# mfkiwl/hyteg

Hardware: AMD Instinct MI355X
Metric: DoF-updates/s, P1 Laplace apply() level 8 (higher is better)
Workload: dtype f64

## Files before the change

hyteg_amd/capi.py:

```python
from __future__ import annotations

import ctypes as C
from pathlib import Path

_PKG = Path(__file__).resolve().parent
_LIB_PATH = _PKG / "lib" / "libhyteg_hip.so"

REPLACE, ADD = 0, 1
MIN_LEVEL, MAX_LEVEL, MAX_SRCS = 2, 11, 4

_vp, _i, _d, _sz, _i64 = C.c_void_p, C.c_int, C.c_double, C.c_size_t, C.c_int64
_dp = C.POINTER(C.c_double)
SIGNATURES = {
    "hyteg_hip_version": (C.c_char_p, []),
    "hyteg_hip_last_error": (C.c_char_p, []),
    "hyteg_hip_device_count": (_i, [C.POINTER(_i)]),
    "hyteg_hip_set_device": (_i, [_i]),
    "hyteg_hip_device_name": (_i, [C.c_char_p, _sz]),
    "hyteg_hip_malloc": (_i, [C.POINTER(_vp), _sz]),
    "hyteg_hip_free": (_i, [_vp]),
    "hyteg_hip_memset_zero": (_i, [_vp, _sz, _vp]),
    "hyteg_hip_upload": (_i, [_vp, _vp, _sz, _vp]),
    "hyteg_hip_download": (_i, [_vp, _vp, _sz, _vp]),
    "hyteg_hip_copy": (_i, [_vp, _vp, _sz, _vp]),
    "hyteg_hip_calib_copy": (_i, [_vp, _vp, _i64, _i, _vp]),
    "hyteg_hip_p2_operator_table_closure_split": (_i, [_vp, _vp, _vp, _vp]),
    "hyteg_hip_p2_operator_table_face_edge_weights": (_i, [_vp, C.POINTER(_i), _vp]),
    "hyteg_hip_p2_sor_face_frames_bytes": (_sz, []),
    "hyteg_hip_p2_sor_face_frames": (_i, [_i, C.POINTER(_i), _vp, _vp]),
    "hyteg_hip_p2_sor_face_edgedofs_cells": (_i, [_i, C.POINTER(_vp), C.POINTER(_vp), _i, _vp, _d, C.POINTER(C.c_uint), _i, _vp]),
    "hyteg_hip_p2_sor_face_edgedofs_cell": (_i, [_vp, _vp, _i, C.POINTER(_i), _vp, _d, C.c_uint, _i, _vp]),
    "hyteg_hip_calib_copy_ring": (_i, [C.POINTER(_vp), C.POINTER(_vp), _i, _i64, _i, _i, _i, _vp, _vp, _vp]),
    "hyteg_hip_stream_create": (_i, [C.POINTER(_vp)]),
    "hyteg_hip_stream_destroy": (_i, [_vp]),
    "hyteg_hip_stream_synchronize": (_i, [_vp]),
    "hyteg_hip_stream_is_capturing": (_i, [_vp, C.POINTER(_i)]),
    "hyteg_hip_event_create": (_i, [C.POINTER(_vp)]),
    "hyteg_hip_event_create_timing": (_i, [C.POINTER(_vp)]),
    "hyteg_hip_event_elapsed_ms": (_i, [_vp, _vp, C.POINTER(C.c_float)]),
    "hyteg_hip_event_destroy": (_i, [_vp]),
    "hyteg_hip_event_record": (_i, [_vp, _vp]),
    "hyteg_hip_stream_wait_event": (_i, [_vp, _vp]),
    "hyteg_hip_comm_available": (_i, [C.c_char_p, _sz]),
    "hyteg_hip_comm_unique_id": (_i, [C.c_char_p]),
    "hyteg_hip_comm_create": (_i, [C.POINTER(_vp), _i, _i, C.c_char_p]),
    "hyteg_hip_comm_destroy": (_i, [_vp]),
    "hyteg_hip_comm_exchange": (_i, [_vp, _i, C.POINTER(_i), _vp, C.POINTER(_i), _vp, C.POINTER(_i), _vp]),
    "hyteg_hip_comm_allreduce_sum": (_i, [_vp, _vp, _i, _vp]),
    "hyteg_hip_p2p_arena_create": (_i, [C.c_size_t, C.POINTER(_vp), C.c_char_p, C.POINTER(_i)]),
    "hyteg_hip_p2p_arena_destroy": (_i, [_vp]),
    "hyteg_hip_p2p_arena_open": (_i, [C.c_char_p, C.POINTER(_vp)]),
    "hyteg_hip_p2p_arena_close": (_i, [_vp]),
    "hyteg_hip_p2p_pack": (_i, [_vp, _i, _vp, _vp, _vp, _i, C.c_ulonglong, _vp, _vp]),
    "hyteg_hip_p2p_wait": (_i, [_vp, _i, _i, C.c_ulonglong, _vp, C.c_uint, _vp]),
    "hyteg_hip_p1_apply_cell_boundary_p2p": (_i, [_vp, _vp, _i, _vp, C.c_uint, _i, _vp, _vp, _vp, _i, C.c_ulonglong, _vp, _vp]),
    "hyteg_hip_reduce_shared_after_p2p": (_i, [_vp, _vp, _vp, _vp, _i, _i, _i, _vp, _i, _i, C.c_ulonglong, _vp, C.c_uint, _vp]),
    "hyteg_hip_graph_begin_capture": (_i, [_vp]),
    "hyteg_hip_graph_end_capture": (_i, [_vp, C.POINTER(_vp)]),
    "hyteg_hip_graph_abort_capture": (_i, [_vp]),
    "hyteg_hip_graph_launch": (_i, [_vp, _vp]),
    "hyteg_hip_graph_destroy": (_i, [_vp]),
    "hyteg_hip_prepare_level": (_i, [_i]),
    "hyteg_hip_cell_width": (_i64, [_i]),
    "hyteg_hip_cell_size": (_i64, [_i]),
    "hyteg_hip_cell_inner_size": (_i64, [_i]),
    "hyteg_hip_cell_index": (_i64, [_i, _i, _i, _i]),
    "hyteg_hip_p1_apply_cell": (_i, [_vp, _vp, _i, _dp, _i, _vp]),
    "hyteg_hip_p1_apply_cell_steps": (_i, [C.POINTER(_vp), C.POINTER(_vp), _i, _i, _dp, _i, _vp]),
    "hyteg_hip_p1_apply_kernel_name": (_i, [_i, _i, C.c_char_p, _sz]),
    "hyteg_hip_p1_residual_jacobi_start_f32": (_i, [_vp, _vp, _vp, _vp, _i, _dp, _d, _vp]),
    "hyteg_hip_p1_jacobi_accumulate_f32": (_i, [_vp, _vp, _vp, _i, _dp, _d, _vp]),
    "hyteg_hip_set_apply_shape": (_i, [_i, _i, _i]),
    "hyteg_hip_p1_apply_cell_f32": (_i, [_vp, _vp, _i, _dp, _i, _vp]),
    "hyteg_hip_p1_jacobi_cell_f32": (_i, [_vp, _vp, _vp, _vp, _i, _dp, _d, _vp]),
    "hyteg_hip_convert_f64_to_f32": (_i, [_vp, _vp, _sz, _vp]),
    "hyteg_hip_convert_f32_to_f64": (_i, [_vp, _vp, _sz, _vp]),
    "hyteg_hip_axpy_f32_into_f64": (_i, [_vp, _vp, _d, _sz, _vp]),
    "hyteg_hip_p1_jacobi_cell": (_i, [_vp, _vp, _vp, _vp, _i, _dp, _d, _vp]),
    "hyteg_hip_p1_chebyshev_start_cell": (_i, [_vp, _vp, _vp, _vp, _i, _dp, _vp]),
    "hyteg_hip_p1_chebyshev_step_cell": (_i, [_vp, _vp, _vp, _vp, _i, _dp, _d, _d, _i, _vp]),
    "hyteg_hip_p1_sor_cell": (_i, [_vp, _vp, _i, _dp, _d, _i, _vp]),
    "hyteg_hip_p1_residual_cell": (_i, [_vp, _vp, _vp, _i, _dp, _vp]),
    "hyteg_hip_p1_sor_cell_sweeps": (_i, [_vp, _vp, _i, _dp, _d, _i, _i, _vp]),
    "hyteg_hip_set_sor_algorithm": (_i, [_i]),
    "hyteg_hip_p1_assign_cell": (_i, [_vp, _i, C.POINTER(_vp), _dp, _i, _vp]),
    "hyteg_hip_p1_add_cell": (_i, [_vp, _i, C.POINTER(_vp), _dp, _i, _vp]),
    "hyteg_hip_p1_mult_cell": (_i, [_vp, _i, C.POINTER(_vp), _i, _vp]),
    "hyteg_hip_dot_workspace_bytes": (_sz, []),
    "hyteg_hip_p1_dot_cell": (_i, [_vp, _vp, _i, _vp, _vp, _vp]),
    "hyteg_hip_p1_restrict_cell": (_i, [_vp, _vp, _i, _dp, _vp]),
    "hyteg_hip_p1_prolongate_cell": (_i, [_vp, _vp, _i, _dp, _i, _vp]),
    "hyteg_hip_p1_apply_cell_boundary": (_i, [_vp, _vp, _i, _dp, C.c_uint, _i, _vp]),
    "hyteg_hip_p1_vector_cell_masked": (_i, [_i, _vp, _i, C.POINTER(_vp), _dp, _i, C.c_uint, _vp]),
    "hyteg_hip_p1_set_cell_masked": (_i, [_vp, _d, _i, C.c_uint, _vp]),
    "hyteg_hip_p1_dot_cell_masked": (_i, [_vp, _vp, _i, C.c_uint, _vp, _vp, _vp]),
    "hyteg_hip_p1_restrict_cell_masked": (_i, [_vp, _vp, _i, _dp, C.c_uint, _vp]),
    "hyteg_hip_p1_prolongate_cell_masked": (_i, [_vp, _vp, _i, _dp, C.c_uint, _vp]),
    "hyteg_hip_p1_prolongate_cell_masked_update": (_i, [_vp, _vp, _i, _dp, C.c_uint, _i, _vp]),
    "hyteg_hip_sum_shared": (_i, [_vp, _vp, _vp, _vp, _i, _i, _vp]),
    "hyteg_hip_copy_shared": (_i, [_vp, _vp, _vp, _vp, _i, _i, _vp]),
    "hyteg_hip_p1_copy_face_to_cell": (_i, [_vp, _vp, _i, _i, _i, _i, _vp]),
    "hyteg_hip_p1_copy_cell_to_face": (_i, [_vp, _vp, _i, _i, _i, _i, _i, _vp]),
    "hyteg_hip_p1_vector_cells": (_i, [_i, _i, C.POINTER(_vp), _i, C.POINTER(_vp), _dp, _i, C.POINTER(C.c_uint), _vp]),
    "hyteg_hip_p1_dot_cells": (_i, [_i, C.POINTER(_vp), C.POINTER(_vp), _i, C.POINTER(C.c_uint), _vp, _vp, _vp]),
    "hyteg_hip_p1_apply_cells": (_i, [_i, C.POINTER(_vp), C.POINTER(_vp), _i, _vp, C.POINTER(C.c_uint), _i, _vp]),
    "hyteg_hip_p1_jacobi_cells": (_i, [_i, C.POINTER(_vp), C.POINTER(_vp), C.POINTER(_vp), C.POINTER(_vp), _i, _vp, _d,
                                        C.POINTER(C.c_uint), _i, _vp]),
    "hyteg_hip_p1_restrict_cells": (_i, [_i, C.POINTER(_vp), C.POINTER(_vp), _i, _vp, C.POINTER(C.c_uint), _vp]),
    "hyteg_hip_p1_prolongate_cells": (_i, [_i, C.POINTER(_vp), C.POINTER(_vp), _i, _vp, C.POINTER(C.c_uint), _i, _vp]),
    "hyteg_hip_p2_edge_array_size": (C.c_size_t, [_i]),
    "hyteg_hip_p2_operator_table_size": (C.c_size_t, []),
    "hyteg_hip_p2_build_operator_table": (_i, [_dp, _dp]),
    "hyteg_hip_p2_prolongate_cell": (_i, [_vp, _vp, _vp, _vp, _i, _i, C.c_uint, _vp]),
    "hyteg_hip_p2_restrict_cell": (_i, [_vp, _vp, _vp, _vp, _i, _dp, C.c_uint, _vp]),
    "hyteg_hip_p2_restrict_cells": (_i, [_i, C.POINTER(_vp), C.POINTER(_vp), C.POINTER(_vp), C.POINTER(_vp), _i, _vp, C.POINTER(C.c_uint), _vp]),
    "hyteg_hip_p2_prolongate_cells": (_i, [_i, C.POINTER(_vp), C.POINTER(_vp), C.POINTER(_vp), C.POINTER(_vp), _i, _i, C.POINTER(C.c_uint), _vp]),
    "hyteg_hip_p2_edge_vector_cell_masked": (_i, [_i, _vp, _i, C.POINTER(_vp), _dp, _i, C.c_uint, _vp]),
    "hyteg_hip_p2_edge_vector_cell_kinds": (_i, [_i, _vp, _i, C.POINTER(_vp), _dp, _i, C.c_uint, C.c_uint, _vp]),
    "hyteg_hip_p2_elementwise_apply_cells_kinds": (_i, [_i, C.POINTER(_vp), C.POINTER(_vp), C.POINTER(_vp), C.POINTER(_vp), _i, C.POINTER(_vp), _d, _i,
                                                   C.POINTER(C.c_uint), C.c_uint, _vp]),
    "hyteg_hip_p2_edge_dot_cells_masked": (_i, [_i, C.POINTER(_vp), C.POINTER(_vp), _i, C.POINTER(C.c_uint), _vp, _vp]),
    "hyteg_hip_p2_edge_vector_cells_kinds": (_i, [_i, _i, C.POINTER(_vp), _i, C.POINTER(_vp), _dp, _i, C.POINTER(C.c_uint), C.c_uint, _vp]),
    "hyteg_hip_p2_edge_dot_cell_masked": (_i, [_vp, _vp, _i, C.c_uint, _vp, _vp, _vp]),
    "hyteg_hip_p2_elementwise_apply_cell": (_i, [_vp, _vp, _vp, _vp, _i, _vp, _d, _i, C.c_uint, _vp]),
    "hyteg_hip_p2_elementwise_apply_cell_kinds": (_i, [_vp, _vp, _vp, _vp, _i, _vp, _d, _i, C.c_uint, C.c_uint, _vp]),
    "hyteg_hip_p2_set_class_rows_min_level": (_i, [_i]),
    "hyteg_hip_p1_vector_cells_dev": (_i, [_i, _i, C.POINTER(_vp), _i, C.POINTER(_vp), C.POINTER(_vp), _i, C.POINTER(C.c_uint), _vp]),
    "hyteg_hip_cg_scalars": (_i, [_vp, _i, _d, _d, _vp]),
    "hyteg_hip_p1_cg_small_max_entries": (_i, []),
    "hyteg_hip_p1_cg_small_cells": (_i, [_i, C.POINTER(_vp), C.POINTER(_vp), _i, _vp, C.POINTER(C.c_uint), C.POINTER(C.c_uint), C.POINTER(_vp),
                                         C.POINTER(_vp), C.POINTER(_vp), C.POINTER(_i), _i, _d, _d, _vp, _vp]),
    "hyteg_hip_p1_dot_cells_cg": (_i, [_i, C.POINTER(_vp), C.POINTER(_vp), _i, C.POINTER(C.c_uint), _vp, _i, _i, _d, _d, _vp, _vp]),
    "hyteg_hip_p1_sor_cells": (_i, [_i, C.POINTER(_vp), C.POINTER(_vp), _i, _vp, _d, _i, C.POINTER(C.c_uint), _vp]),
    "hyteg_hip_p1_sor_shell_cells": (_i, [_i, C.POINTER(_vp), C.POINTER(_vp), C.POINTER(_vp), _i, _vp, _d, C.POINTER(C.c_uint), _i, _vp]),
    "hyteg_hip_p1_sor_shell_cell": (_i, [_vp, _vp, _vp, _i, C.POINTER(_i), _dp, C.POINTER(_i), _dp, _dp, _d, C.c_uint, _i, _vp]),
    "hyteg_hip_p1_apply_face3d": (_i, [_vp, _vp, _i, _i, C.POINTER(_i), _dp, _i, _vp]),
    "hyteg_hip_p1_sor_face3d_workspace": (C.c_size_t, [_i]),
    "hyteg_hip_p1_sor_face3d": (_i, [_vp, _vp, _vp, _i, _i, C.POINTER(_i), _dp, C.c_double, _i, _vp]),
    "hyteg_hip_gather_entries": (_i, [_vp, _vp, _vp, _vp, _i, _vp]),
    "hyteg_hip_p2_constant_stencil_layout": (_i, [C.POINTER(_i), C.POINTER(_i)]),
    "hyteg_hip_p2_build_operator_table_from_stencils": (_i, [_dp, _dp, _dp]),
    "hyteg_hip_p2_apply_cell_edgedof_to_vertexdof": (_i, [_vp] * 7 + [_vp, _dp, _i, _i, _vp]),
    "hyteg_hip_p2_apply_cell_vertexdof_to_edgedof": (_i, [_vp] * 7 + [_vp, _i, _dp, _i, _vp]),
    "hyteg_hip_p2_apply_cell_edgedof_to_edgedof": (_i, [_vp] * 14 + [_dp, _i, _i, _vp]),
    "hyteg_hip_p1_elementwise_diffusion_apply_macro_3d": (_i, [_vp, _vp, _dp, _i64, _d, _vp]),
    "hyteg_hip_p1_elementwise_diffusion_apply_macro_3d_masked": (_i, [_vp, _vp, _dp, _i64, C.c_uint, _i, _vp]),
    "hyteg_hip_p1_elementwise_diffusion_apply_macro_3d_f32": (_i, [_vp, _vp, C.POINTER(C.c_float), _i64, C.c_float, _vp]),
    "hyteg_hip_p1_elementwise_diffusion_diagonal_macro_3d": (_i, [_vp, _dp, _i64, _d, _vp]),
    "hyteg_hip_p1_elementwise_diffusion_stencils": (_i, [_dp, _i64, _dp, _dp]),
    "hyteg_hip_p1_apply_cell_boundary_f32": (_i, [_vp, _vp, _i, _dp, C.c_uint, _i, _vp]),
    "hyteg_hip_p2_elementwise_diffusion_apply_macro_3d": (_i, [_vp, _vp, _vp, _vp, _dp, _i64, _d, _vp]),
    "hyteg_hip_p2_elementwise_diffusion_element_matrices": (_i, [_dp, _i64, _dp]),
}
MASK_INNER, MASK_SHELL, MASK_ALL = 1 << 14, 0x3FFF, 0x7FFF


class HytegHipError(RuntimeError):
    pass


def lib_path() -> Path:
    return _LIB_PATH


_lib = None


def lib() -> C.CDLL:
    global _lib
    if _lib is None:
        if not _LIB_PATH.exists():
            raise HytegHipError(
                f"{_LIB_PATH} not found: build it with `python -c 'import __graft_entry__ as g; g.build()'` "
                "(hipcc --offload-arch=gfx950).  hyteg_amd has no CPU fallback.")
        l = C.CDLL(str(_LIB_PATH))
# ... 95 lines not shown


def event_record(ev, stream=0) -> None:
    check(lib().hyteg_hip_event_record(ev, stream), "event_record")


def stream_wait_event(stream, ev) -> None:
    check(lib().hyteg_hip_stream_wait_event(stream, ev), "stream_wait_event")


def calib_copy(dst, src, n, nontemporal=True, stream=0) -> None:
    check(lib().hyteg_hip_calib_copy(dst, src, n, 1 if nontemporal else 0, stream), "calib_copy")


def calib_copy_ring(pairs, n, nontemporal=True, stream=0):
    m = len(pairs)
    d, s = (_vp * m)(*[p[0] for p in pairs]), (_vp * m)(*[p[1] for p in pairs])
    fn = lib().hyteg_hip_calib_copy_ring

    def call(first, count, ev_start=None, ev_stop=None):
        check(fn(d, s, m, n, 1 if nontemporal else 0, first, count, stream, ev_start, ev_stop), "calib_copy_ring")

    return call


def p1_residual_jacobi_start_f32(r_f32, e_f32, rhs, src, level, w, relax, stream=0):
    check(lib().hyteg_hip_p1_residual_jacobi_start_f32(r_f32, e_f32, rhs, src, level, _w15(w), float(relax), stream), "p1_residual_jacobi_start_f32")


def p1_jacobi_accumulate_f32(x, rhs_f32, e_f32, level, w, relax, stream=0):
    check(lib().hyteg_hip_p1_jacobi_accumulate_f32(x, rhs_f32, e_f32, level, _w15(w), float(relax), stream), "p1_jacobi_accumulate_f32")


def set_apply_shape(ny=0, lz=0, pfd=0) -> None:
    check(lib().hyteg_hip_set_apply_shape(ny, lz, pfd), "set_apply_shape")


def p1_apply_kernel_name(level, update=REPLACE) -> str:
    buf = C.create_string_buffer(256)
    check(lib().hyteg_hip_p1_apply_kernel_name(level, update, buf, 256), "p1_apply_kernel_name")
    return buf.value.decode()


def p2_prolongate_cell(fine_v, fine_e, coarse_v, coarse_e, coarse_level, update=REPLACE, mask=0x7FFF, stream=0):
    check(lib().hyteg_hip_p2_prolongate_cell(fine_v, fine_e, coarse_v, coarse_e, coarse_level, update, mask, stream), "p2_prolongate_cell")


def p2_restrict_cell(coarse_v, coarse_e, fine_v, fine_e, coarse_level, nnc, mask=0x7FFF, stream=0):
    a = (C.c_double * 14)(*[float(x) for x in nnc])
    check(lib().hyteg_hip_p2_restrict_cell(coarse_v, coarse_e, fine_v, fine_e, coarse_level, a, mask, stream), "p2_restrict_cell")


def p1_apply_cell_f32(dst, src, level, w, update=REPLACE, stream=0):
    check(lib().hyteg_hip_p1_apply_cell_f32(dst, src, level, _w15(w), update, stream), "p1_apply_cell_f32")


def p1_jacobi_cell_f32(dst, rhs, src, level, w, relax, invdiag=None, stream=0):
    check(lib().hyteg_hip_p1_jacobi_cell_f32(dst, rhs, src, invdiag, level, _w15(w), relax, stream), "p1_jacobi_cell_f32")


def convert_f64_to_f32(dst, src, n, stream=0):
    check(lib().hyteg_hip_convert_f64_to_f32(dst, src, n, stream), "convert_f64_to_f32")


def convert_f32_to_f64(dst, src, n, stream=0):
    check(lib().hyteg_hip_convert_f32_to_f64(dst, src, n, stream), "convert_f32_to_f64")


def axpy_f32_into_f64(y, x, alpha, n, stream=0):
    check(lib().hyteg_hip_axpy_f32_into_f64(y, x, alpha, n, stream), "axpy_f32_into_f64")


def p1_apply_cell(dst, src, level, w, update=REPLACE, stream=0):
    check(lib().hyteg_hip_p1_apply_cell(dst, src, level, _w15(w), update, stream), "p1_apply_cell")


def p1_apply_cell_steps(dsts, srcs, level, w, update=REPLACE, stream=0):
    if len(srcs) != len(dsts):
        raise ValueError("p1_apply_cell_steps: as many sources as destinations")
    d, s = (_vp * len(dsts))(*[int(p) for p in dsts]), (_vp * len(srcs))(*[int(p) for p in srcs])
    check(lib().hyteg_hip_p1_apply_cell_steps(d, s, len(dsts), level, _w15(w), update, stream), "p1_apply_cell_steps")


def p1_jacobi_cell(dst, rhs, src, level, w, relax, invdiag=None, stream=0):
    check(lib().hyteg_hip_p1_jacobi_cell(dst, rhs, src, invdiag, level, _w15(w), float(relax), stream),
          "p1_jacobi_cell")


def p1_chebyshev_start_cell(t_out, rhs, x, level, w, invdiag=None, stream=0):
    check(lib().hyteg_hip_p1_chebyshev_start_cell(t_out, rhs, x, invdiag, level, _w15(w), stream), "p1_chebyshev_start_cell")


def p1_chebyshev_step_cell(t_out, x, t_in, level, w, c_prev, c_cur, has_prev=True, invdiag=None, stream=0):
    check(lib().hyteg_hip_p1_chebyshev_step_cell(t_out, x, t_in, invdiag, level, _w15(w), float(c_prev), float(c_cur),
                                                 int(bool(has_prev)), stream), "p1_chebyshev_step_cell")


SOR_AUTO, SOR_PLANES, SOR_BLOCKS, SOR_DATAFLOW = 0, 1, 2, 3


def set_sor_algorithm(algorithm: int) -> None:
    check(lib().hyteg_hip_set_sor_algorithm(int(algorithm)), "set_sor_algorithm")


def p1_sor_cell(u, rhs, level, w, relax, backwards=False, stream=0):
    check(lib().hyteg_hip_p1_sor_cell(u, rhs, level, _w15(w), float(relax), int(backwards), stream), "p1_sor_cell")


def p1_residual_cell(dst, rhs, src, level, w, stream=0):
    check(lib().hyteg_hip_p1_residual_cell(dst, rhs, src, level, _w15(w), stream), "p1_residual_cell")


def p1_sor_cell_sweeps(u, rhs, level, w, relax, nsweeps, backwards=False, stream=0):
    check(lib().hyteg_hip_p1_sor_cell_sweeps(u, rhs, level, _w15(w), float(relax), int(backwards), int(nsweeps), stream), "p1_sor_cell_sweeps")


def p1_assign_cell(dst, scalars, srcs, level, stream=0):
    check(lib().hyteg_hip_p1_assign_cell(dst, len(srcs), _ptrs(srcs), _scal(scalars), level, stream),
          "p1_assign_cell")


def p1_add_cell(dst, scalars, srcs, level, stream=0):
    check(lib().hyteg_hip_p1_add_cell(dst, len(srcs), _ptrs(srcs), _scal(scalars), level, stream), "p1_add_cell")


def p1_mult_cell(dst, srcs, level, stream=0):
    check(lib().hyteg_hip_p1_mult_cell(dst, len(srcs), _ptrs(srcs), level, stream), "p1_mult_cell")


def dot_workspace_bytes(): return int(lib().hyteg_hip_dot_workspace_bytes())


def p1_dot_cell(a, b, level, result_dev, workspace_dev, stream=0):
    check(lib().hyteg_hip_p1_dot_cell(a, b, level, result_dev, workspace_dev, stream), "p1_dot_cell")


def p1_restrict_cell(coarse, fine, coarse_level, nnc, stream=0):
    check(lib().hyteg_hip_p1_restrict_cell(coarse, fine, coarse_level, _f14(nnc), stream), "p1_restrict_cell")


def p1_prolongate_cell(coarse, fine, coarse_level, nnc, update=REPLACE, stream=0):
    check(lib().hyteg_hip_p1_prolongate_cell(coarse, fine, coarse_level, _f14(nnc), update, stream),
          "p1_prolongate_cell")


def p1_apply_cell_boundary(dst, src, level, w_slots, mask=MASK_SHELL, update=REPLACE, stream=0):
    flat = [float(v) for row in w_slots for v in row]
    arr = (C.c_double * 210)(*flat)
    check(lib().hyteg_hip_p1_apply_cell_boundary(dst, src, level, arr, mask, update, stream), "p1_apply_cell_boundary")


def p1_vector_cell_masked(op, dst, scalars, srcs, level, mask, stream=0):
    sc = _scal(scalars) if scalars is not None else None
    check(lib().hyteg_hip_p1_vector_cell_masked(op, dst, len(srcs), _ptrs(srcs), sc, level, mask, stream),
          "p1_vector_cell_masked")


def p1_set_cell_masked(dst, value, level, mask, stream=0):
    check(lib().hyteg_hip_p1_set_cell_masked(dst, float(value), level, mask, stream), "p1_set_cell_masked")


def p1_dot_cell_masked(a, b, level, mask, result_dev, workspace_dev, stream=0):
    check(lib().hyteg_hip_p1_dot_cell_masked(a, b, level, mask, result_dev, workspace_dev, stream), "p1_dot_cell_masked")


def p1_restrict_cell_masked(coarse, fine, coarse_level, nnc, mask, stream=0):
    check(lib().hyteg_hip_p1_restrict_cell_masked(coarse, fine, coarse_level, _f14(nnc), mask, stream),
          "p1_restrict_cell_masked")


def p1_prolongate_cell_masked(coarse, fine, coarse_level, nnc, mask, stream=0):
    check(lib().hyteg_hip_p1_prolongate_cell_masked(coarse, fine, coarse_level, _f14(nnc), mask, stream),
          "p1_prolongate_cell_masked")


def p1_prolongate_cell_masked_update(coarse, fine, coarse_level, nnc, mask, update=REPLACE, stream=0):
    check(lib().hyteg_hip_p1_prolongate_cell_masked_update(coarse, fine, coarse_level, _f14(nnc), mask, update, stream),
          "p1_prolongate_cell_masked_update")


def sum_shared(bases, group_ptr, entry_buf, entry_off, ngroups, n_writable, stream=0):
    check(lib().hyteg_hip_sum_shared(bases, group_ptr, entry_buf, entry_off, ngroups, n_writable, stream), "sum_shared")


def gather_entries(out, bases, entry_buf, entry_off, n, stream=0):
    check(lib().hyteg_hip_gather_entries(out, bases, entry_buf, entry_off, n, stream), "gather_entries")


def p1_copy_face_to_cell(cell, face, level, v, stream=0):
    check(lib().hyteg_hip_p1_copy_face_to_cell(cell, face, level, int(v[0]), int(v[1]), int(v[2]), stream), "p1_copy_face_to_cell")


def p1_copy_cell_to_face(face, cell, level, v, neighbor, stream=0):
    check(lib().hyteg_hip_p1_copy_cell_to_face(face, cell, level, int(v[0]), int(v[1]), int(v[2]), int(neighbor), stream),
          "p1_copy_cell_to_face")


def _ptrs(ps):
    return (C.c_void_p * len(ps))(*[int(p) for p in ps])


def _masks(ms):
    return (C.c_uint * len(ms))(*[int(m) for m in ms])


def p1_vector_cells(op, dst, srcs, scalars, level, masks, stream=0):
    n = len(dst)
    flat = [p for f in srcs for p in f]
    sc = (C.c_double * max(1, len(scalars or [])))(*[float(v) for v in (scalars or [0.0])])
    check(lib().hyteg_hip_p1_vector_cells(op, n, _ptrs(dst), len(srcs), _ptrs(flat) if flat else None, sc if scalars is not None else None,
                                          level, _masks(masks), stream), "p1_vector_cells")


def p1_dot_cells(a, b, level, masks, result_dev, workspace_dev, stream=0):
    check(lib().hyteg_hip_p1_dot_cells(len(a), _ptrs(a), _ptrs(b), level, _masks(masks), result_dev, workspace_dev, stream), "p1_dot_cells")


(HYTEG_HIP_CG_PRSOLD, HYTEG_HIP_CG_PAP, HYTEG_HIP_CG_RR, HYTEG_HIP_CG_ALPHA, HYTEG_HIP_CG_NEG_ALPHA, HYTEG_HIP_CG_BETA, HYTEG_HIP_CG_RES_START,
 HYTEG_HIP_CG_DONE, HYTEG_HIP_CG_ITERATIONS, HYTEG_HIP_CG_ONE) = range(10)
HYTEG_HIP_CG_SLOTS = 16
HYTEG_HIP_MAX_BATCH = 80


def p1_vector_cells_dev(op, dst, srcs, scalar_ptrs, level, masks, stream=0):
    flat = [p for f in srcs for p in f]
    sp = (_vp * len(scalar_ptrs))(*[None if p is None else int(p) for p in scalar_ptrs]) if scalar_ptrs is not None else None
    check(lib().hyteg_hip_p1_vector_cells_dev(op, len(dst), _ptrs(dst), len(srcs), _ptrs(flat) if flat else None, sp, level, _masks(masks), stream),
          "p1_vector_cells_dev")


def p1_dot_cells_cg(a, b, level, masks, s_dev, slot, phase, rel_tol, abs_tol, workspace_dev, stream=0):
    check(lib().hyteg_hip_p1_dot_cells_cg(len(a), _ptrs(a), _ptrs(b), level, _masks(masks), s_dev, slot, phase, float(rel_tol), float(abs_tol),
# ... 286 lines not shown
```

hyteg_amd/csrc/exp/apply_trace.hip:

```cpp
#include <algorithm>
#include <cmath>
#include <cstdlib>
#include <cstring>
#include <random>
#include <vector>

#include <hip/hip_runtime.h>

#ifdef ZM_DO_TRACE
__device__ unsigned long long* g_trace;
#define ZM_TRACE( slot )                                                                                              \
   do                                                                                                                 \
   {                                                                                                                  \
      if ( ( slot ) == 3 )                                                                                            \
         asm volatile( "s_waitcnt vmcnt(0)" ::: "memory" );                                                           \
      const unsigned long long _t = __builtin_amdgcn_s_memrealtime();                                                 \
      if ( ( threadIdx.x & 63 ) == 0 )                                                                                \
      {                                                                                                               \
         unsigned long long* _p = g_trace + ( (size_t) blockIdx.x * kZMarchWavesPerBlock + ( threadIdx.x >> 6 ) ) * 8; \
         _p[slot]               = _t;                                                                                 \
         if ( ( slot ) == 0 )                                                                                         \
         {                                                                                                            \
            _p[6] = __builtin_amdgcn_s_getreg( 20 | ( 0 << 6 ) | ( 31 << 11 ) );                          \
            _p[7] = __builtin_amdgcn_s_getreg( 4 | ( 0 << 6 ) | ( 31 << 11 ) );                            \
         }                                                                                                            \
      }                                                                                                               \
   } while ( 0 )
#endif

#include "../kernels_apply_zmarch.hpp"
#include "kernels_apply_zloop.hpp"

using namespace hyteg_hip;

template < int NY, int LZ, int PFD >
__global__ __launch_bounds__( 64 * kZMarchWavesPerBlock ) void zmarch_trace_kernel( const ZMarchArgs A )
{
   zmarch_body< APPLY_REPLACE, NY, LZ, PFD, double >( A, A.tasks, A.ntasks, A.xcd_chunk, A.src, A.dst );
}

#define CK( e )                                                                                \
   do                                                                                          \
   {                                                                                           \
      hipError_t _e = ( e );                                                                   \
      if ( _e != hipSuccess )                                                                  \
      {                                                                                        \
         fprintf( stderr, "%s:%d %s: %s\n", __FILE__, __LINE__, #e, hipGetErrorString( _e ) ); \
         exit( 1 );                                                                            \
      }                                                                                        \
   } while ( 0 )

__global__ __launch_bounds__( 64 ) void apply_rows_naive( double* dst, const double* src, int N, Stencil15 st )
{
   const int z = 1 + blockIdx.y, y = 1 + blockIdx.x;
   const int W = N - z, R = W - y;
   if ( y > W - 3 )
      return;
   const int     S0 = tri( W ), Sm = tri( W + 1 );
   const int     base = slice_start( N, z ) + row_start( W, y );
   const double* w    = st.w;
   for ( int x = 1 + threadIdx.x; x <= R - 2; x += 64 )
   {
      const int i = base + x;
      double    acc;
      acc    = w[6] * src[i - 1];
      acc    = fma( w[3], src[i - Sm + W + 1], acc );
      acc    = fma( w[10], src[i + R], acc );
      acc    = fma( w[5], src[i - R], acc );
      acc    = fma( w[12], src[i + S0 - W + 1], acc );
      acc    = fma( w[1], src[i - Sm + y + 1], acc );
      acc    = fma( w[8], src[i + 1], acc );
      acc    = fma( w[13], src[i + S0 - y - 1], acc );
      acc    = fma( w[2], src[i - Sm + W], acc );
      acc    = fma( w[9], src[i + R - 1], acc );
      acc    = fma( w[4], src[i - R - 1], acc );
      acc    = fma( w[11], src[i + S0 - W], acc );
      acc    = fma( w[0], src[i - Sm + y], acc );
      acc    = fma( w[7], src[i], acc );
      acc    = fma( w[14], src[i + S0 - y], acc );
      dst[i] = acc;
   }
}

template < typename T >
static T pct( std::vector< T > v, double p )
{
   std::sort( v.begin(), v.end() );
   return v[std::min( v.size() - 1, (size_t) ( p * ( v.size() - 1 ) + 0.5 ) )];
}

int main( int argc, char** argv )
{
   const int     level = argc > 1 ? atoi( argv[1] ) : 8;
   const int     reps  = argc > 2 ? atoi( argv[2] ) : 300;
   const int     nbuf  = argc > 3 ? atoi( argv[3] ) : 9;
   const int     N     = ( 1 << level ) + 1;
   const int     total = (int) tet64( N );
   const int64_t inner = hyteg_hip_cell_inner_size( level );
   printf( "level %d  N %d  entries %d  inner %lld  buffers %d pairs (%.1f MB total)\n", level, N, total, (long long) inner,
           nbuf, nbuf * 2.0 * total * 8 / 1e6 );

   std::vector< double >                    h( total );
   std::mt19937_64                          gen( 42 );
   std::uniform_real_distribution< double > U( 0, 1 );
   for ( auto& v : h )
      v = U( gen );
   Stencil15 st;
   for ( int k = 0; k < 15; ++k )
      st.w[k] = U( gen ) - 0.5;
   std::vector< double* > src( nbuf ), dst( nbuf );
   for ( int b = 0; b < nbuf; ++b )
   {
      CK( hipMalloc( &src[b], (size_t) total * 8 + 16 ) );
      CK( hipMalloc( &dst[b], (size_t) total * 8 + 16 ) );
      CK( hipMemcpy( src[b], h.data(), (size_t) total * 8, hipMemcpyHostToDevice ) );
      CK( hipMemset( dst[b], 0, (size_t) total * 8 ) );
   }
   double* refout;
   CK( hipMalloc( &refout, (size_t) total * 8 ) );
   CK( hipMemset( refout, 0, (size_t) total * 8 ) );
   hipLaunchKernelGGL( apply_rows_naive, dim3( N, N ), dim3( 64 ), 0, 0, refout, src[0], N, st );
// ... 142 lines not shown
```

hyteg_amd/csrc/exp/p1_apply_rank.hip:

```cpp
#include <cstdlib>

#include "../kernels_apply_zmarch.hpp"
#include "../p2p_device.hpp"
#include "../shell.hpp"

using namespace hyteg_hip;

namespace {

constexpr int kBrickNY = 4;
inline int   brick_lz( int level ) { return level >= 8 ? 8 : 4; }
constexpr int kRankThreads = 64 * kZMarchWavesPerBlock;

struct RankArgs
{
   shell::Slots14x15           S;
   unsigned                    mask;
   int                         update;
   int                         brickBlocks, shellBlocks;
   const hyteg_hip_p2p_peer_t* peers;
   int                         npeers;
   double* const*              bases;
   const int*                  entry_buf;
   const int*                  entry_off;
   int                         n;
   unsigned long long          seq;
   unsigned*                   counters;
   unsigned*                   status;
   unsigned long long          timeout_ticks;
   int                         dbg;
};

template < int MODE, int LZ >
__global__ __launch_bounds__( kRankThreads ) void p1_apply_rank_kernel( const BrickTask* tasks, int ntasks, int xcd_chunk, const ZMarchArgs A,
                                                                        const RankArgs R )
{
   const int b = blockIdx.x;
   if ( b < R.brickBlocks )
   {
      zmarch_body< MODE, kBrickNY, LZ, 2, double >( A, tasks, ntasks, xcd_chunk, A.src, A.dst );
      return;
   }
   double*       dst = static_cast< double* >( A.dst );
   const double* src = static_cast< const double* >( A.src );
   if ( b < R.brickBlocks + R.shellBlocks )
   {
      const int q = ( b - R.brickBlocks ) * kRankThreads + (int) threadIdx.x;
      int       x, y, z, slot;
      if ( !( R.dbg & 4 ) && shell::shell_point( A.N, q, x, y, z, slot ) && ( ( R.mask >> slot ) & 1u ) )
      {
         const double acc = shell::share( R.S, src, A.N, x, y, z, slot );
         const int    i   = cell_index( A.N, x, y, z );
         if ( R.dbg & 2 )
            dst[i] = acc;
         else
            __hip_atomic_store( dst + i, R.update == HYTEG_HIP_ADD ? acc + dst[i] : acc, __ATOMIC_RELAXED, __HIP_MEMORY_SCOPE_AGENT );
      }
      p2p::stores_acknowledged();
      __syncthreads();
      if ( threadIdx.x == 0 )
         __hip_atomic_fetch_add( R.counters + 1, 1u, __ATOMIC_RELAXED, __HIP_MEMORY_SCOPE_AGENT );
      return;
   }
   if ( threadIdx.x == 0 && !( R.dbg & 1 ) )
   {
      const unsigned long long t0 = wall_clock64();
      while ( __hip_atomic_load( R.counters + 1, __ATOMIC_RELAXED, __HIP_MEMORY_SCOPE_AGENT ) < (unsigned) R.shellBlocks )
      {
         if ( wall_clock64() - t0 > R.timeout_ticks )
         {
            __hip_atomic_store( R.status, 0x40000000u, __ATOMIC_RELAXED, __HIP_MEMORY_SCOPE_SYSTEM );
            break;
         }
         __builtin_amdgcn_s_sleep( 4 );
      }
   }
   __syncthreads();
   const int first = R.brickBlocks + R.shellBlocks;
   const int k     = ( b - first ) * kRankThreads + (int) threadIdx.x;
   if ( k < R.n && !( R.dbg & 8 ) )
      p2p::send_value( R.peers, R.npeers, k, R.seq,
                       __hip_atomic_load( R.bases[R.entry_buf[k]] + R.entry_off[k], __ATOMIC_RELAXED, __HIP_MEMORY_SCOPE_AGENT ) );
   p2p::stores_acknowledged();
   __syncthreads();
   if ( threadIdx.x == 0 )
   {
      const unsigned done = __hip_atomic_fetch_add( R.counters, 1u, __ATOMIC_RELAXED, __HIP_MEMORY_SCOPE_AGENT );
      if ( done == gridDim.x - first - 1 )
      {
         __hip_atomic_store( R.counters, 0u, __ATOMIC_RELAXED, __HIP_MEMORY_SCOPE_AGENT );
         __hip_atomic_store( R.counters + 1, 0u, __ATOMIC_RELAXED, __HIP_MEMORY_SCOPE_AGENT );
         p2p::publish( R.peers, R.npeers, R.seq );
      }
   }
}

template < int MODE, int LZ >
int launch_rank( double* dst, const double* src, int level, const double* w, RankArgs& R, hipStream_t stream )
{
   BrickTable bt;
   int        rc = get_bricks( level, kBrickNY, LZ, &bt );
   if ( rc != HYTEG_HIP_OK )
      return rc;
   ZMarchArgs A{};
   A.dst    = dst;
   A.src    = src;
   A.tasks  = bt.dev;
   A.ntasks = bt.count;
   A.N      = ( 1 << level ) + 1;
   A.bytes  = (unsigned) ( tet64( A.N ) * (int64_t) sizeof( double ) );
   for ( int k = 0; k < 15; ++k )
      A.st.w[k] = w[k];
   int nblocks   = ( bt.count + kZMarchWavesPerBlock - 1 ) / kZMarchWavesPerBlock;
   nblocks       = ( nblocks + 7 ) & ~7;
   if ( R.dbg & 16 )
      nblocks = 0;
   A.xcd_chunk   = nblocks / 8;
   R.brickBlocks = nblocks;
   R.shellBlocks = ( 4 * tri( A.N ) + kRankThreads - 1 ) / kRankThreads;
   const int packBlocks = R.n > 0 ? ( R.n + kRankThreads - 1 ) / kRankThreads : 1;
   hipLaunchKernelGGL( ( p1_apply_rank_kernel< MODE, LZ > ), dim3( nblocks + R.shellBlocks + packBlocks ), dim3( kRankThreads ), 0, stream, A.tasks,
                       A.ntasks, A.xcd_chunk, A, R );
   HH_CHECK_HIP( hipGetLastError() );
// ... 48 lines not shown
```

hyteg_amd/csrc/kernels_apply_zmarch.hpp:

```cpp
#pragma once

#include <algorithm>
#include <utility>
#include <vector>

#include "common.hpp"

namespace hyteg_hip {

constexpr int kBrickMaxSlices = 10;
struct BrickTask
{
   int i0;
   int W0;
   int y0;
   int xb;
   int nz;
   int pad;
   int base[kBrickMaxSlices];
};
static_assert( sizeof( BrickTask ) == 64, "BrickTask must be 64 bytes (one s_load_dwordx16)" );

struct ZMarchArgs
{
// ... 2 lines not shown
   const void*      rhs;
   const void*      invdiag;
   void*            dst2;
   double*          xacc;
   const BrickTask* tasks;
   int              ntasks;
   unsigned         bytes;
   int              xcd_chunk;
   int              N;
   double           relax;
   Stencil15        st;
   double           relax2;
   int              flag;
};

#ifndef HYTEG_ZM_WAVES_PER_BLOCK
#define HYTEG_ZM_WAVES_PER_BLOCK 4
#endif
constexpr int kZMarchWavesPerBlock = HYTEG_ZM_WAVES_PER_BLOCK;

#ifndef ZM_TRACE
#define ZM_TRACE( slot )
#endif

typedef int zm_v2i_t __attribute__( ( ext_vector_type( 2 ) ) );

template < typename T, int AUX = 0 >
__device__ inline T zm_load2( __amdgpu_buffer_rsrc_t r, int voff, int soff )
{
   if constexpr ( sizeof( T ) == 8 )
   {
      zm_v2i_t v = __builtin_amdgcn_raw_buffer_load_b64( r, voff, soff, AUX );
      return *reinterpret_cast< T* >( &v );
   }
   else
   {
      int v = __builtin_amdgcn_raw_buffer_load_b32( r, voff, soff, AUX );
      return *reinterpret_cast< T* >( &v );
   }
}
template < typename T, int AUX = 0 >
__device__ inline void zm_store2( __amdgpu_buffer_rsrc_t r, int voff, int soff, T d )
{
   if constexpr ( sizeof( T ) == 8 )
      __builtin_amdgcn_raw_buffer_store_b64( *reinterpret_cast< zm_v2i_t* >( &d ), r, voff, soff, AUX );
   else
      __builtin_amdgcn_raw_buffer_store_b32( *reinterpret_cast< int* >( &d ), r, voff, soff, AUX );
}
__device__ inline double zm_lane_minus_1( double v )
{
   int lo = __double2loint( v ), hi = __double2hiint( v );
   lo     = __builtin_amdgcn_mov_dpp( lo, 0x138, 0xf, 0xf, true );
   hi     = __builtin_amdgcn_mov_dpp( hi, 0x138, 0xf, 0xf, true );
   return __hiloint2double( hi, lo );
}
__device__ inline double zm_lane_plus_1( double v )
{
   int lo = __double2loint( v ), hi = __double2hiint( v );
   lo     = __builtin_amdgcn_mov_dpp( lo, 0x130, 0xf, 0xf, true );
   hi     = __builtin_amdgcn_mov_dpp( hi, 0x130, 0xf, 0xf, true );
   return __hiloint2double( hi, lo );
}
__device__ inline float zm_lane_minus_1( float v )
{
   return __int_as_float( __builtin_amdgcn_mov_dpp( __float_as_int( v ), 0x138, 0xf, 0xf, true ) );
}
__device__ inline float zm_lane_plus_1( float v )
{
   return __int_as_float( __builtin_amdgcn_mov_dpp( __float_as_int( v ), 0x130, 0xf, 0xf, true ) );
}

__host__ __device__ inline void zm_fill_bases( BrickTask& t, int LZ )
{
   int base = t.i0, Wq = t.W0;
   for ( int q = 0; q < kBrickMaxSlices; ++q )
   {
      t.base[q] = q < LZ + 2 ? base : 0;
      base += tri( Wq ) - ( t.y0 - 1 );
      Wq -= 1;
   }
}

template < int MODE, int NY, int LZ, int PFD, typename T >
__device__ inline void zmarch_body( const ZMarchArgs& A, const BrickTask* tasks, int ntasks, int xcd_chunk, const void* srcp, void* dstp )
{
   static_assert( LZ + 2 <= kBrickMaxSlices, "the table carries the slice bases of bricks of up to kBrickMaxSlices - 2 slices" );
   constexpr int SZ = (int) sizeof( T );
   ZM_TRACE( 0 );
   int b = blockIdx.x;
   if ( xcd_chunk > 0 )
      b = ( blockIdx.x & 7 ) * xcd_chunk + ( blockIdx.x >> 3 );
   const int task = __builtin_amdgcn_readfirstlane( b * kZMarchWavesPerBlock + ( threadIdx.x >> 6 ) );
   if ( task >= ntasks )
      return;
   const BrickTask t = tasks[task];
   const int lane = threadIdx.x & 63;
   ZM_TRACE( 1 );

   constexpr int kStAux = 2;
   const __amdgpu_buffer_rsrc_t rs = __builtin_amdgcn_make_buffer_rsrc( const_cast< void* >( srcp ), 0, A.bytes, 0x00020000 );
   const __amdgpu_buffer_rsrc_t rd = __builtin_amdgcn_make_buffer_rsrc( dstp, 0, MODE == APPLY_RESIDUAL_F32OUT ? A.bytes / 2 : A.bytes, 0x00020000 );
   constexpr bool kHasRhs = MODE == APPLY_JACOBI || MODE == APPLY_RESIDUAL || MODE == APPLY_RESIDUAL_F32OUT || MODE == APPLY_JACOBI_ACCUM ||
                            MODE == APPLY_CHEB_START;
   constexpr bool kHasInv = MODE == APPLY_JACOBI || MODE == APPLY_CHEB_START || MODE == APPLY_CHEB_STEP;
   static_assert( MODE != APPLY_CHEB_STEP || SZ == 8, "the Chebyshev step updates a double iterate" );
   const __amdgpu_buffer_rsrc_t rr = __builtin_amdgcn_make_buffer_rsrc( const_cast< void* >( kHasRhs ? A.rhs : srcp ), 0, A.bytes, 0x00020000 );
   const __amdgpu_buffer_rsrc_t rd2 =
       __builtin_amdgcn_make_buffer_rsrc( MODE == APPLY_RESIDUAL_F32OUT ? A.dst2 : dstp, 0, MODE == APPLY_RESIDUAL_F32OUT ? A.bytes / 2 : A.bytes, 0x00020000 );
   const __amdgpu_buffer_rsrc_t rx = __builtin_amdgcn_make_buffer_rsrc(
       ( MODE == APPLY_JACOBI_ACCUM || MODE == APPLY_CHEB_STEP ) ? (void*) A.xacc : dstp, 0, MODE == APPLY_JACOBI_ACCUM ? A.bytes * 2 : A.bytes, 0x00020000 );
   const __amdgpu_buffer_rsrc_t ri = __builtin_amdgcn_make_buffer_rsrc(
       const_cast< void* >( ( kHasInv && A.invdiag ) ? A.invdiag : srcp ), 0, A.bytes, 0x00020000 );

   const int lane_off = lane * SZ;
   const int ym       = t.y0 - 1;

   T S[LZ + 2][NY + 2];

   auto load_slice = [&]( auto qc, int base_q, int W_q ) {
      constexpr int q  = decltype( qc )::value;
      int           ix = base_q;
#pragma unroll
      for ( int r = 0; r < NY + 2; ++r )
      {
         const bool need = ( q == 0 ) ? ( r >= 1 ) : ( q == LZ + 1 ? ( r <= NY ) : true );
         if ( need )
         {
            const int last8 = ( W_q - ( ym + r ) - 1 - t.xb ) * SZ;
            S[q][r]         = zm_load2< T >( rs, min( lane_off, last8 ), ix * SZ );
         }
         ix += W_q - ( ym + r );
      }
   };

   int baseq[LZ + 2], Wqs[LZ + 2];
#pragma unroll
   for ( int q = 0; q < LZ + 2; ++q )
   {
      baseq[q] = t.base[q];
      Wqs[q]   = t.W0 - q;
   }
   [&]< int... Is >( std::integer_sequence< int, Is... > ) {
      ( load_slice( std::integral_constant< int, Is >{}, baseq[Is], Wqs[Is] ), ... );
   }
   ( std::make_integer_sequence < int, ( 2 + PFD <= LZ + 2 ? 2 + PFD : LZ + 2 ) > {} );
   ZM_TRACE( 2 );

   T w[15];
#pragma unroll
   for ( int i = 0; i < 15; ++i )
      w[i] = (T) A.st.w[i];
   const T invc  = (T) ( 1.0 / A.st.w[7] );
   const T relax = (T) A.relax;

   constexpr int kExAux = MODE == APPLY_ADD ? 2 : 0;
   T          EX0[LZ][NY], EX1[LZ][NY];
   double     EXD[LZ][NY];
   const bool hasInv = kHasInv && A.invdiag != nullptr;
   auto       load_extra = [&]( auto sc ) {
      constexpr int s = decltype( sc )::value;
      constexpr int q = s + 1;
      if constexpr ( MODE != APPLY_REPLACE )
      {
         const int W  = Wqs[q];
         int       ie = baseq[q] + ( W - ym );
#pragma unroll
         for ( int j = 0; j < NY; ++j )
         {
            const int last8 = ( W - ( t.y0 + j ) - 1 - t.xb ) * SZ;
            const int vo    = min( lane_off, last8 );
            if constexpr ( MODE == APPLY_CHEB_STEP )
               EXD[s][j] = zm_load2< double, 0 >( rx, vo, ie * 8 );
            else
               EX0[s][j] = MODE == APPLY_ADD ? zm_load2< T, kExAux >( rd, vo, ie * SZ ) : zm_load2< T, kExAux >( rr, vo, ie * SZ );
            if constexpr ( MODE == APPLY_JACOBI_ACCUM )
               EXD[s][j] = zm_load2< double, 2 >( rx, min( lane * 8, last8 * 2 ), ie * 8 );
            if constexpr ( kHasInv )
            {
               T v = invc;
               if ( hasInv )
                  v = zm_load2< T >( ri, vo, ie * SZ );
               EX1[s][j] = v;
            }
            ie += W - ( t.y0 + j );
         }
      }
   };
   if constexpr ( MODE != APPLY_REPLACE )
   {
      [&]< int... Is >( std::integer_sequence< int, Is... > ) { ( load_extra( std::integral_constant< int, Is >{} ), ... ); }
      ( std::make_integer_sequence < int, ( PFD < LZ ? PFD : LZ ) > {} );
   }

   auto step = [&]( auto sc ) {
      constexpr int s = decltype( sc )::value;
      constexpr int q = s + 1;
      if constexpr ( q + 1 + PFD <= LZ + 1 )
         load_slice( std::integral_constant< int, q + 1 + PFD >{}, baseq[q + 1 + PFD], Wqs[q + 1 + PFD] );
      if constexpr ( s + PFD < LZ )
         load_extra( std::integral_constant< int, s + PFD >{} );

      const int W  = Wqs[q];
      int       io = baseq[q] + ( W - ym );
      if constexpr ( s == 0 )
         ZM_TRACE( 3 );
#pragma unroll
      for ( int j = 0; j < NY; ++j )
      {
         const T am = S[q][j], a0 = S[q][j + 1], ap = S[q][j + 2];
         const T um = S[q + 1][j], u0 = S[q + 1][j + 1];
         const T d0 = S[q - 1][j + 1], dp = S[q - 1][j + 2];
         T pe = w[8] * a0;
         pe        = fma( w[5], am, pe );
         pe        = fma( w[12], um, pe );
         pe        = fma( w[1], d0, pe );
         T pw = w[6] * a0;
         pw        = fma( w[13], u0, pw );
         pw        = fma( w[2], dp, pw );
         pw        = fma( w[9], ap, pw );
         T acc = zm_lane_plus_1( pe ) + zm_lane_minus_1( pw );
         acc        = fma( w[3], dp, acc );
         acc        = fma( w[10], ap, acc );
         acc        = fma( w[4], am, acc );
         acc        = fma( w[11], um, acc );
         acc        = fma( w[0], d0, acc );
         acc        = fma( w[7], a0, acc );
         acc        = fma( w[14], u0, acc );

         const int R = W - ( t.y0 + j );
         T         out;
         if ( MODE == APPLY_REPLACE )
            out = acc;
         else if ( MODE == APPLY_ADD )
            out = acc + EX0[s][j];
         else if ( MODE == APPLY_RESIDUAL || MODE == APPLY_RESIDUAL_F32OUT )
            out = EX0[s][j] - acc;
         else if ( MODE == APPLY_JACOBI_ACCUM )
            out = a0 + relax * ( invc * ( EX0[s][j] - acc ) );
         else if ( MODE == APPLY_CHEB_START )
            out = EX1[s][j] * ( EX0[s][j] - acc );
         else if ( MODE == APPLY_CHEB_STEP )
            out = EX1[s][j] * acc;
         else
            out = a0 + relax * ( EX1[s][j] * ( EX0[s][j] - acc ) );
         const int      cnt = s < t.nz ? min( 62, R - 2 - t.xb ) : 0;
         const unsigned lm1 = (unsigned) ( lane - 1 );
         const bool     on  = lm1 < (unsigned) max( cnt, 0 );
         if constexpr ( MODE == APPLY_RESIDUAL_F32OUT )
         {
            const float rf = (float) out;
            zm_store2< float, 0 >( rd, on ? lane * 4 : -8, io * 4, rf );
            zm_store2< float, 0 >( rd2, on ? lane * 4 : -8, io * 4, (float) relax * ( (float) invc * rf ) );
         }
         else if constexpr ( MODE == APPLY_JACOBI_ACCUM )
            zm_store2< double, kStAux >( rx, on ? lane * 8 : -8, io * 8, EXD[s][j] + (double) out );
         else if constexpr ( MODE == APPLY_CHEB_STEP )
         {
            double xn = EXD[s][j];
            if ( A.flag )
               xn = xn + (double) A.relax2 * (double) a0;
            xn = xn + (double) relax * (double) out;
            zm_store2< T, kStAux >( rd, on ? lane_off : -8, io * SZ, out );
            zm_store2< double, kStAux >( rx, on ? lane * 8 : -8, io * 8, xn );
         }
         else
            zm_store2< T, kStAux >( rd, on ? lane_off : -8, io * SZ, out );
         io += R;
      }
   };

   [&]< int... Is >( std::integer_sequence< int, Is... > ) { ( step( std::integral_constant< int, Is >{} ), ... ); }
   ( std::make_integer_sequence< int, LZ >{} );
   ZM_TRACE( 4 );
}

template < int MODE, int NY, int LZ, int PFD, typename T >
__global__ __launch_bounds__( 64 * kZMarchWavesPerBlock ) void p1_apply_zmarch_preload_kernel( const BrickTask* tasks, int ntasks, int xcd_chunk,
                                                                                              const ZMarchArgs A )
{
   zmarch_body< MODE, NY, LZ, PFD, T >( A, tasks, ntasks, xcd_chunk, A.src, A.dst );
}

constexpr int kZMarchMaxSteps = 16;
struct ZMarchStepPtrs
{
   const void* srcs[kZMarchMaxSteps];
   void*       dsts[kZMarchMaxSteps];
};

template < int MODE, int NY, int LZ, int PFD, typename T >
__global__ __launch_bounds__( 64 * kZMarchWavesPerBlock ) void p1_apply_zmarch_steps_kernel( const BrickTask* tasks, int ntasks, int xcd_chunk,
                                                                                            const ZMarchArgs A, const ZMarchStepPtrs P )
{
   static_assert( MODE == APPLY_REPLACE || MODE == APPLY_ADD, "a steps launch has one source and one destination per step" );
   const unsigned step = blockIdx.y < (unsigned) kZMarchMaxSteps ? blockIdx.y : 0u;
   zmarch_body< MODE, NY, LZ, PFD, T >( A, tasks, ntasks, xcd_chunk, P.srcs[step], P.dsts[step] );
}

inline void build_brick_tasks( int level, int NY, int LZ, std::vector< BrickTask >& out )
{
   const int N = ( 1 << level ) + 1;
   out.clear();
   for ( int z0 = 1; z0 <= N - 4; z0 += LZ )
   {
      const int W = N - z0;
      for ( int y0 = 1; y0 <= W - 3; y0 += NY )
      {
         const int xmax = W - y0 - 2;
         for ( int x0 = 1; x0 <= xmax; x0 += 62 )
         {
            BrickTask t{};
            t.xb = x0 - 1;
            t.y0 = y0;
            t.W0 = W + 1;
            t.i0 = slice_start( N, z0 - 1 ) + row_start( W + 1, y0 - 1 ) + t.xb;
            t.nz = std::min( LZ, N - 4 - z0 + 1 );
            zm_fill_bases( t, LZ );
            out.push_back( t );
         }
      }
   }
}

}
```

hyteg_amd/csrc/p1_apply.hip:

```cpp
#include <cstdlib>
#include <string>
#include <type_traits>

#include "kernels_apply.hpp"
#include "kernels_apply_zmarch.hpp"

using namespace hyteg_hip;

namespace {

constexpr int kTile = 1024;

struct BrickShape
{
   int  ny, lz, pfd;
   bool operator==( const BrickShape& o ) const { return ny == o.ny && lz == o.lz && pfd == o.pfd; }
};
BrickShape g_shape_override{ 0, 0, 0 };

inline BrickShape default_shape( int mode, int level, bool f32 )
{
   if ( level <= 7 )
      return ( mode == APPLY_REPLACE || f32 ) ? BrickShape{ 2, 4, 1 } : BrickShape{ 4, 4, 1 };
   if ( level == 8 )
// ... 39 lines not shown
int zmarch_common_args( ZMarchArgs& A, int& nblocks, int NY, int LZ, int level, const double* w )
{
   nblocks = 0;
   BrickTable bt;
   int        rc = get_bricks( level, NY, LZ, &bt );
   if ( rc != HYTEG_HIP_OK || bt.count == 0 )
      return rc;
   A.tasks  = bt.dev;
   A.ntasks = bt.count;
   A.N      = ( 1 << level ) + 1;
   A.bytes  = (unsigned) ( tet64( A.N ) * (int64_t) sizeof( T ) );
   for ( int k = 0; k < 15; ++k )
      A.st.w[k] = w[k];
   nblocks     = ( bt.count + kZMarchWavesPerBlock - 1 ) / kZMarchWavesPerBlock;
   nblocks     = ( nblocks + 7 ) & ~7;
   A.xcd_chunk = nblocks / 8;
   static const bool xcdSlabs = env_flag( "HYTEG_HIP_APPLY_XCD_SLABS", true );
   if ( !xcdSlabs )
      A.xcd_chunk = 0;
   return HYTEG_HIP_OK;
}

template < int MODE, int NY, int LZ, int PFD, typename T >
int launch_zmarch_shape( void* dst, const T* src, const T* rhs, const T* invdiag, int level, const double* w, double relax, hipStream_t stream,
                         void* extra, double relax2, int flag )
{
   ZMarchArgs A{};
   int        nblocks = 0;
   const int  rc      = zmarch_common_args< T >( A, nblocks, NY, LZ, level, w );
   if ( rc != HYTEG_HIP_OK || nblocks == 0 )
      return rc;
   A.dst     = dst;
   A.src     = src;
   A.rhs     = rhs;
   A.invdiag = invdiag;
   A.dst2    = extra;
   A.xacc    = static_cast< double* >( extra );
   A.relax   = relax;
   A.relax2  = relax2;
   A.flag    = flag;
   hipLaunchKernelGGL( ( p1_apply_zmarch_preload_kernel< MODE, NY, LZ, PFD, T > ), dim3( nblocks ), dim3( 64 * kZMarchWavesPerBlock ), 0, stream, A.tasks,
                       A.ntasks, A.xcd_chunk, A );
   HH_CHECK_HIP( hipGetLastError() );
   return HYTEG_HIP_OK;
}

inline unsigned steps_lds_request( int level )
{
   static const int fromEnv = [] {
      const char* v = getenv( "HYTEG_HIP_APPLY_STEPS_WG_PER_CU" );
      return v ? atoi( v ) : -1;
   }();
   const int m = fromEnv >= 0 ? fromEnv : ( level == 8 ? 2 : 0 );
   return ( m >= 1 && m <= 6 ) ? (unsigned) ( ( 160 * 1024 / m ) & ~4095 ) : 0u;
}

template < int MODE, int NY, int LZ, int PFD >
int launch_zmarch_steps_shape( void* const* dsts, const void* const* srcs, int nsteps, int level, const double* w, hipStream_t stream )
{
   static_assert( MODE == APPLY_REPLACE || MODE == APPLY_ADD, "steps launch: Replace and Add" );
   ZMarchArgs A{};
   int        nblocks = 0;
   const int  rc      = zmarch_common_args< double >( A, nblocks, NY, LZ, level, w );
   if ( rc != HYTEG_HIP_OK || nblocks == 0 )
      return rc;
   ZMarchStepPtrs P{};
   for ( int k = 0; k < kZMarchMaxSteps; ++k )
   {
      P.srcs[k] = srcs[k < nsteps ? k : 0];
      P.dsts[k] = dsts[k < nsteps ? k : 0];
   }
   A.src = P.srcs[0];
   A.dst = P.dsts[0];
   auto           kern = p1_apply_zmarch_steps_kernel< MODE, NY, LZ, PFD, double >;
   const unsigned lds  = steps_lds_request( level );
   if ( lds > 0 )
   {
      static const hipError_t attr = hipFuncSetAttribute( reinterpret_cast< const void* >( kern ), hipFuncAttributeMaxDynamicSharedMemorySize, (int) lds );
      HH_CHECK_HIP( attr );
   }
   hipLaunchKernelGGL( kern, dim3( nblocks, nsteps ), dim3( 64 * kZMarchWavesPerBlock ), lds, stream, A.tasks, A.ntasks, A.xcd_chunk, A, P );
   HH_CHECK_HIP( hipGetLastError() );
   return HYTEG_HIP_OK;
}

template < int MODE, typename T = double >
int launch_zmarch( void* dst, const T* src, const T* rhs, const T* invdiag, int level, const double* w, double relax, hipStream_t stream,
                   void* extra = nullptr, double relax2 = 0.0, int flag = 0 )
{
   const int shapeMode = MODE == APPLY_RESIDUAL_F32OUT ? APPLY_RESIDUAL :
                                                         ( ( MODE == APPLY_JACOBI_ACCUM || MODE == APPLY_CHEB_START || MODE == APPLY_CHEB_STEP ) ? APPLY_JACOBI : MODE );
   int        rc       = HYTEG_HIP_OK;
   const bool compiled = with_compiled_shape( current_shape( shapeMode, level, !std::is_same< T, double >::value ), [&]( auto ny, auto lz, auto pfd ) {
      rc = launch_zmarch_shape< MODE, decltype( ny )::value, decltype( lz )::value, decltype( pfd )::value, T >( dst, src, rhs, invdiag, level, w, relax, stream,
                                                                                                                 extra, relax2, flag );
   } );
   return compiled ? rc : fail( HYTEG_HIP_EINVAL, "apply: brick shape not compiled in" );
}

template < int MODE >
int launch_zmarch_steps( void* const* dsts, const void* const* srcs, int nsteps, int level, const double* w, hipStream_t stream )
{
   int        rc       = HYTEG_HIP_OK;
   const bool compiled = with_compiled_shape( current_shape( MODE, level, false ), [&]( auto ny, auto lz, auto pfd ) {
      rc = launch_zmarch_steps_shape< MODE, decltype( ny )::value, decltype( lz )::value, decltype( pfd )::value >( dsts, srcs, nsteps, level, w, stream );
   } );
   return compiled ? rc : fail( HYTEG_HIP_EINVAL, "apply steps: brick shape not compiled in" );
}

inline bool level_runs_zmarch( int level )
{
   static const bool forceTiled = env_flag( "HYTEG_HIP_APPLY_LDS_TILED", false );
   return !forceTiled && tet64( ( 1 << level ) + 1 ) * 8 < ( (int64_t) 1 << 31 );
}

template < int MODE >
int launch_apply( double* dst, const double* src, const double* rhs, const double* invdiag, int level, const double* w,
                  double relax, hipStream_t stream )
{
   if ( level_runs_zmarch( level ) )
      return launch_zmarch< MODE >( dst, src, rhs, invdiag, level, w, relax, stream );

   TileTable tt;
   int       rc = get_tiles( level, TILES_INNER, kTile, &tt );
   if ( rc != HYTEG_HIP_OK )
      return rc;
   if ( tt.count == 0 )
      return HYTEG_HIP_OK;

   ApplyArgs A;
   A.dst     = dst;
   A.src     = src;
   A.rhs     = rhs;
   A.invdiag = invdiag;
   A.tiles   = tt.dev;
   A.ntiles  = tt.count;
   A.N       = ( 1 << level ) + 1;
   A.total   = (int) tet64( A.N );
   A.relax   = relax;
   for ( int k = 0; k < 15; ++k )
      A.st.w[k] = w[k];
   const int nblocks = ( tt.count + 7 ) & ~7;
   A.xcd_chunk       = nblocks / 8;

   const size_t lds_bytes = (size_t) apply_lds_doubles( kTile, A.N ) * sizeof( double );
   const bool   vec       = ( reinterpret_cast< uintptr_t >( src ) & 15 ) == 0;
   auto         kern      = vec ? p1_apply_tiled_kernel< MODE, true > : p1_apply_tiled_kernel< MODE, false >;
   if ( lds_bytes > 48 * 1024 )
      HH_CHECK_HIP( hipFuncSetAttribute( reinterpret_cast< const void* >( kern ),
                                         hipFuncAttributeMaxDynamicSharedMemorySize,
                                         (int) lds_bytes ) );
   hipLaunchKernelGGL( kern, dim3( nblocks ), dim3( kApplyThreads ), lds_bytes, stream, A );
   HH_CHECK_HIP( hipGetLastError() );
   return HYTEG_HIP_OK;
}

}

extern "C" {

HYTEG_HIP_API int hyteg_hip_p1_apply_cell( double*            dst,
                                           const double*      src,
                                           int                level,
                                           const double*      w,
                                           int                update,
                                           hyteg_hip_stream_t stream )
{
   HH_REQUIRE( dst && src && w, "p1_apply_cell: null pointer" );
   HH_REQUIRE( level_ok( level ), "p1_apply_cell: level out of range [2,11]" );
   HH_REQUIRE( dst != src, "p1_apply_cell: src and dst must not alias" );
   HH_REQUIRE( update == HYTEG_HIP_REPLACE || update == HYTEG_HIP_ADD, "p1_apply_cell: bad update type" );
   if ( update == HYTEG_HIP_REPLACE )
      return launch_apply< APPLY_REPLACE >( dst, src, nullptr, nullptr, level, w, 0.0, as_stream( stream ) );
   return launch_apply< APPLY_ADD >( dst, src, nullptr, nullptr, level, w, 0.0, as_stream( stream ) );
}

HYTEG_HIP_API int hyteg_hip_p1_apply_cell_steps( void* const*       dsts,
                                                 const void* const* srcs,
                                                 int                nsteps,
                                                 int                level,
                                                 const double*      w,
                                                 int                update,
                                                 hyteg_hip_stream_t stream )
{
   HH_REQUIRE( dsts && srcs && w, "p1_apply_cell_steps: null pointer" );
   HH_REQUIRE( nsteps >= 1 && nsteps <= kZMarchMaxSteps, "p1_apply_cell_steps: nsteps out of range [1,16]" );
   HH_REQUIRE( level_ok( level ), "p1_apply_cell_steps: level out of range [2,11]" );
   HH_REQUIRE( update == HYTEG_HIP_REPLACE || update == HYTEG_HIP_ADD, "p1_apply_cell_steps: bad update type" );
   for ( int i = 0; i < nsteps; ++i )
   {
      HH_REQUIRE( dsts[i] && srcs[i], "p1_apply_cell_steps: null array" );
      for ( int j = 0; j < nsteps; ++j )
         HH_REQUIRE( dsts[i] != srcs[j] && ( i == j || dsts[i] != dsts[j] ),
                     "p1_apply_cell_steps: an array written by one step must not be read or written by another (nor be the step's own source)" );
   }
   if ( nsteps == 1 )
      return hyteg_hip_p1_apply_cell( static_cast< double* >( dsts[0] ), static_cast< const double* >( srcs[0] ), level, w, update, stream );
   if ( !level_runs_zmarch( level ) )
      return fail( HYTEG_HIP_ENOTSUP, "p1_apply_cell_steps: this level does not run the z-march kernel" );
   if ( update == HYTEG_HIP_REPLACE )
      return launch_zmarch_steps< APPLY_REPLACE >( dsts, srcs, nsteps, level, w, as_stream( stream ) );
   return launch_zmarch_steps< APPLY_ADD >( dsts, srcs, nsteps, level, w, as_stream( stream ) );
}

HYTEG_HIP_API int hyteg_hip_p1_apply_cell_f32( float* dst, const float* src, int level, const double* w, int update, hyteg_hip_stream_t stream )
{
   HH_REQUIRE( dst && src && w, "p1_apply_cell_f32: null pointer" );
   HH_REQUIRE( level >= HYTEG_HIP_MIN_LEVEL && level <= 10, "p1_apply_cell_f32: level out of range [2,10]" );
   HH_REQUIRE( dst != src, "p1_apply_cell_f32: src and dst must not alias" );
   HH_REQUIRE( update == HYTEG_HIP_REPLACE || update == HYTEG_HIP_ADD, "p1_apply_cell_f32: bad update type" );
   if ( update == HYTEG_HIP_REPLACE )
      return launch_zmarch< APPLY_REPLACE, float >( dst, src, nullptr, nullptr, level, w, 0.0, as_stream( stream ) );
   return launch_zmarch< APPLY_ADD, float >( dst, src, nullptr, nullptr, level, w, 0.0, as_stream( stream ) );
}

HYTEG_HIP_API int hyteg_hip_p1_jacobi_cell_f32( float*             dst,
                                                const float*       rhs,
                                                const float*       src,
                                                const float*       invdiag,
                                                int                level,
                                                const double*      w,
                                                double             relax,
                                                hyteg_hip_stream_t stream )
{
   HH_REQUIRE( dst && rhs && src && w, "p1_jacobi_cell_f32: null pointer" );
   HH_REQUIRE( level >= HYTEG_HIP_MIN_LEVEL && level <= 10, "p1_jacobi_cell_f32: level out of range [2,10]" );
   HH_REQUIRE( dst != src, "p1_jacobi_cell_f32: src and dst must not alias" );
   HH_REQUIRE( w[7] != 0.0, "p1_jacobi_cell_f32: zero centre weight" );
   return launch_zmarch< APPLY_JACOBI, float >( dst, src, rhs, invdiag, level, w, relax, as_stream( stream ) );
}

HYTEG_HIP_API int hyteg_hip_p1_residual_cell( double*            dst,
                                              const double*      rhs,
                                              const double*      src,
                                              int                level,
                                              const double*      w,
                                              hyteg_hip_stream_t stream )
{
   HH_REQUIRE( dst && rhs && src && w, "p1_residual_cell: null pointer" );
   HH_REQUIRE( level >= HYTEG_HIP_MIN_LEVEL && level <= 10, "p1_residual_cell: level out of range [2,10]" );
   HH_REQUIRE( dst != src, "p1_residual_cell: src and dst must not alias" );
   return launch_zmarch< APPLY_RESIDUAL >( dst, src, rhs, (const double*) nullptr, level, w, 0.0, as_stream( stream ) );
}

HYTEG_HIP_API int hyteg_hip_p1_residual_jacobi_start_f32( float*             r_f32,
                                                          float*             e_f32,
                                                          const double*      rhs,
                                                          const double*      src,
                                                          int                level,
                                                          const double*      w,
                                                          double             relax,
                                                          hyteg_hip_stream_t stream )
{
   HH_REQUIRE( r_f32 && e_f32 && rhs && src && w, "p1_residual_jacobi_start_f32: null pointer" );
   HH_REQUIRE( level >= HYTEG_HIP_MIN_LEVEL && level <= 10, "p1_residual_jacobi_start_f32: level out of range [2,10]" );
   HH_REQUIRE( r_f32 != e_f32, "p1_residual_jacobi_start_f32: the two outputs must differ" );
   HH_REQUIRE( w[7] != 0.0, "p1_residual_jacobi_start_f32: zero centre weight" );
   return launch_zmarch< APPLY_RESIDUAL_F32OUT >( r_f32, src, rhs, (const double*) nullptr, level, w, relax, as_stream( stream ), e_f32 );
}

HYTEG_HIP_API int hyteg_hip_p1_jacobi_accumulate_f32( double*            x,
                                                      const float*       rhs_f32,
                                                      const float*       e_f32,
                                                      int                level,
                                                      const double*      w,
                                                      double             relax,
                                                      hyteg_hip_stream_t stream )
{
   HH_REQUIRE( x && rhs_f32 && e_f32 && w, "p1_jacobi_accumulate_f32: null pointer" );
   HH_REQUIRE( level >= HYTEG_HIP_MIN_LEVEL && level <= 10, "p1_jacobi_accumulate_f32: level out of range [2,10]" );
   HH_REQUIRE( w[7] != 0.0, "p1_jacobi_accumulate_f32: zero centre weight" );
   return launch_zmarch< APPLY_JACOBI_ACCUM, float >( nullptr, e_f32, rhs_f32, (const float*) nullptr, level, w, relax, as_stream( stream ), x );
}

HYTEG_HIP_API int hyteg_hip_p1_chebyshev_start_cell( double*            t_out,
                                                     const double*      rhs,
                                                     const double*      x,
                                                     const double*      invdiag,
                                                     int                level,
                                                     const double*      w,
                                                     hyteg_hip_stream_t stream )
{
   HH_REQUIRE( t_out && rhs && x && w, "p1_chebyshev_start_cell: null pointer" );
   HH_REQUIRE( level_ok( level ), "p1_chebyshev_start_cell: level out of range [2,11]" );
   HH_REQUIRE( t_out != x && t_out != rhs && t_out != invdiag, "p1_chebyshev_start_cell: t_out must not alias x, rhs or invdiag" );
   HH_REQUIRE( w[7] != 0.0, "p1_chebyshev_start_cell: zero centre weight" );
   if ( level_runs_zmarch( level ) )
// ... 110 lines not shown
```

hyteg_amd/csrc/p1_boundary.hip:

```cpp
#include "p2p_device.hpp"
#include "shell.hpp"

using namespace hyteg_hip;

namespace {

constexpr int kThreads = 256;

using namespace hyteg_hip::shell;

template < typename T >
__global__ __launch_bounds__( kThreads ) void p1_apply_shell_kernel( T* __restrict__ dst,
                                                                      const T* __restrict__ src,
                                                                      int              N,
                                                                      unsigned         mask,
                                                                      int              update,
                                                                      const Slots14x15 S )
{
   const int q = blockIdx.x * kThreads + threadIdx.x;
   int       x, y, z, slot;
   if ( !shell_point( N, q, x, y, z, slot ) || !( ( mask >> slot ) & 1u ) )
      return;
   const T   acc = share< T >( S, src, N, x, y, z, slot );
   const int i   = cell_index( N, x, y, z );
   dst[i]        = update == HYTEG_HIP_ADD ? acc + dst[i] : acc;
}

__global__ __launch_bounds__( kThreads ) void p1_apply_shell_send_kernel( double* __restrict__ dst,
                                                                           const double* __restrict__ src,
                                                                           int              N,
                                                                           unsigned         mask,
                                                                           int              update,
                                                                           const Slots14x15 S,
                                                                           const int* __restrict__ send_first,
                                                                           const int* __restrict__ send_list,
                                                                           const hyteg_hip_p2p_peer_t* __restrict__ peers,
                                                                           int                npeers,
                                                                           unsigned long long seq,
                                                                           unsigned*          counter )
{
   const int q = blockIdx.x * kThreads + threadIdx.x;
   int       x, y, z, slot;
   if ( shell_point( N, q, x, y, z, slot ) && ( ( mask >> slot ) & 1u ) )
   {
      const double acc = share( S, src, N, x, y, z, slot );
      const int    i   = cell_index( N, x, y, z );
      const double val = update == HYTEG_HIP_ADD ? acc + dst[i] : acc;
      dst[i]           = val;
      for ( int j = send_first[q]; j < send_first[q + 1]; ++j )
         p2p::send_value( peers, npeers, send_list[j], seq, val );
   }
   p2p::stores_acknowledged();
   __syncthreads();
   if ( threadIdx.x == 0 )
   {
      const unsigned done = __hip_atomic_fetch_add( counter, 1u, __ATOMIC_RELAXED, __HIP_MEMORY_SCOPE_AGENT );
      if ( done == gridDim.x - 1 )
      {
         __hip_atomic_store( counter, 0u, __ATOMIC_RELAXED, __HIP_MEMORY_SCOPE_AGENT );
         p2p::publish( peers, npeers, seq );
      }
   }
}

struct VecArgsM
{
   double*       dst;
   const double* src[HYTEG_HIP_MAX_SRCS];
   double        c[HYTEG_HIP_MAX_SRCS];
   int           N;
   int           nsrc;
   unsigned      mask;
   int           op;
};

__global__ __launch_bounds__( kThreads ) void p1_vector_shell_kernel( const VecArgsM A )
{
   const int q = blockIdx.x * kThreads + threadIdx.x;
   int       x, y, z, slot;
   if ( !shell_point( A.N, q, x, y, z, slot ) || !( ( A.mask >> slot ) & 1u ) )
      return;
   const int i = cell_index( A.N, x, y, z );
   double    tmp;
   if ( A.op == 3 )
      tmp = A.c[0];
   else if ( A.op == 2 )
   {
      tmp = A.src[0][i];
      for ( int k = 1; k < A.nsrc; ++k )
         tmp *= A.src[k][i];
   }
   else
   {
      tmp = A.c[0] * A.src[0][i];
      for ( int k = 1; k < A.nsrc; ++k )
         tmp += A.c[k] * A.src[k][i];
      if ( A.op == 1 )
         tmp = A.dst[i] + tmp;
   }
   A.dst[i] = tmp;
}

constexpr int kFlatPerThread = 4;
__global__ __launch_bounds__( kThreads ) void p1_vector_flat_kernel( const VecArgsM A, int n )
{
   const int base = blockIdx.x * ( kThreads * kFlatPerThread ) + threadIdx.x;
   double    v[kFlatPerThread][HYTEG_HIP_MAX_SRCS + 1];
#pragma unroll
// ... 234 lines not shown
   const int Wf = dir == 0 ? N : N - 1;
   const int r  = blockIdx.x * kThreads + threadIdx.x;
   if ( r >= tri( Wf ) )
      return;
   const int y = row_of( Wf, r ), x = r - row_start( Wf, y );
   int       cx, cy, cz;
   face_to_cell( N - 1, m, x, y, dir, cx, cy, cz );
   const int ci = cell_index( N, cx, cy, cz );
   if ( dir == 0 )
      dst[ci] = src[r];
   else
      dst[ghost_offset + r] = src[ci];
}

__global__ __launch_bounds__( kThreads ) void p1_apply_face3d_kernel( const FaceApplyArgs A )
{
   const int N = A.N, n = N - 1;
   const int r = blockIdx.x * kThreads + threadIdx.x;
   if ( r >= tri( N ) )
      return;
   const int y = row_of( N, r ), x = r - row_start( N, y );
   if ( x < 1 || y < 1 || x + y > n - 1 )
      return;
   double tmp = 0.0;
   for ( int k = 0; k < A.ncells; ++k )
   {
      const FaceMap& m = A.map[k];
      int            cx, cy, cz;
      face_to_cell( n, m, x, y, 0, cx, cy, cz );
#pragma unroll
      for ( int s = 0; s < 15; ++s )
      {
         const int lx = cx + kStencilOffs[s][0], ly = cy + kStencilOffs[s][1], lz = cz + kStencilOffs[s][2];
         if ( lx < 0 || ly < 0 || lz < 0 || lx + ly + lz > n )
            continue;
         const int bary[4] = { n - lx - ly - lz, lx, ly, lz };
         const int fx = bary[m.v[1]], fy = bary[m.v[2]], fz = bary[m.v3];
         if ( fz > 1 )
            continue;
         const int idx = fz == 0 ? row_start( N, fy ) + fx : tri( N ) + k * tri( N - 1 ) + row_start( N - 1, fy ) + fx;
         tmp           = fma( A.w[k][s], A.src[idx], tmp );
      }
   }
   A.dst[r] = A.update == HYTEG_HIP_ADD ? A.dst[r] + tmp : tmp;
}

inline bool vmap_ok( int v0, int v1, int v2 )
{
   return v0 >= 0 && v0 < 4 && v1 >= 0 && v1 < 4 && v2 >= 0 && v2 < 4 && v0 != v1 && v0 != v2 && v1 != v2;
}

inline int  shell_blocks( int N ) { return ( 4 * tri( N ) + kThreads - 1 ) / kThreads; }

}

namespace hyteg_hip {
int launch_vec_inner( int op, double* dst, int nsrc, const double* const* srcs, const double* scalars, int level, hipStream_t stream );
int launch_dot_inner_partial( const double* a, const double* b, int level, double* partial, int* nblocks, hipStream_t stream );
}

extern "C" {

HYTEG_HIP_API int hyteg_hip_p1_apply_cell_boundary( double*            dst,
                                                    const double*      src,
                                                    int                level,
                                                    const double*      w_slots,
                                                    unsigned           mask,
                                                    int                update,
                                                    hyteg_hip_stream_t stream )
{
   HH_REQUIRE( dst && src && w_slots, "p1_apply_cell_boundary: null pointer" );
   HH_REQUIRE( any_level_ok( level ), "p1_apply_cell_boundary: level out of range [0,11]" );
   HH_REQUIRE( dst != src, "p1_apply_cell_boundary: src and dst must not alias" );
   HH_REQUIRE( update == HYTEG_HIP_REPLACE || update == HYTEG_HIP_ADD, "p1_apply_cell_boundary: bad update type" );
   if ( ( mask & HYTEG_HIP_MASK_SHELL ) == 0 )
      return HYTEG_HIP_OK;
   Slots14x15 S;
   for ( int s = 0; s < 14; ++s )
      for ( int k = 0; k < 15; ++k )
         S.w[s][k] = w_slots[15 * s + k];
   const int N = ( 1 << level ) + 1;
   hipLaunchKernelGGL( p1_apply_shell_kernel< double >, dim3( shell_blocks( N ) ), dim3( kThreads ), 0, as_stream( stream ), dst, src, N,
                       mask & HYTEG_HIP_MASK_SHELL, update, S );
   HH_CHECK_HIP( hipGetLastError() );
   return HYTEG_HIP_OK;
}

HYTEG_HIP_API int hyteg_hip_p1_apply_cell_boundary_f32( float*             dst,
                                                        const float*       src,
                                                        int                level,
                                                        const double*      w_slots,
                                                        unsigned           mask,
                                                        int                update,
                                                        hyteg_hip_stream_t stream )
{
   HH_REQUIRE( dst && src && w_slots, "p1_apply_cell_boundary_f32: null pointer" );
   HH_REQUIRE( any_level_ok( level ), "p1_apply_cell_boundary_f32: level out of range [0,11]" );
   HH_REQUIRE( dst != src, "p1_apply_cell_boundary_f32: src and dst must not alias" );
   HH_REQUIRE( update == HYTEG_HIP_REPLACE || update == HYTEG_HIP_ADD, "p1_apply_cell_boundary_f32: bad update type" );
   if ( ( mask & HYTEG_HIP_MASK_SHELL ) == 0 )
      return HYTEG_HIP_OK;
   Slots14x15 S;
   for ( int s = 0; s < 14; ++s )
      for ( int k = 0; k < 15; ++k )
         S.w[s][k] = w_slots[15 * s + k];
   const int N = ( 1 << level ) + 1;
   hipLaunchKernelGGL( p1_apply_shell_kernel< float >, dim3( shell_blocks( N ) ), dim3( kThreads ), 0, as_stream( stream ), dst, src, N,
                       mask & HYTEG_HIP_MASK_SHELL, update, S );
   HH_CHECK_HIP( hipGetLastError() );
   return HYTEG_HIP_OK;
}

HYTEG_HIP_API int hyteg_hip_p1_apply_cell_boundary_p2p( double*                     dst,
                                                        const double*               src,
                                                        int                         level,
                                                        const double*               w_slots,
                                                        unsigned                    mask,
                                                        int                         update,
                                                        const int*                  send_first,
                                                        const int*                  send_list,
                                                        const hyteg_hip_p2p_peer_t* peers,
                                                        int                         npeers,
                                                        unsigned long long          seq,
                                                        unsigned*                   counter,
                                                        hyteg_hip_stream_t          stream )
{
   HH_REQUIRE( dst && src && w_slots, "p1_apply_cell_boundary_p2p: null pointer" );
   HH_REQUIRE( any_level_ok( level ), "p1_apply_cell_boundary_p2p: level out of range [0,11]" );
   HH_REQUIRE( dst != src, "p1_apply_cell_boundary_p2p: src and dst must not alias" );
   HH_REQUIRE( update == HYTEG_HIP_REPLACE || update == HYTEG_HIP_ADD, "p1_apply_cell_boundary_p2p: bad update type" );
   HH_REQUIRE( send_first && send_list && peers && npeers > 0 && counter && seq > 0, "p1_apply_cell_boundary_p2p: bad exchange arguments" );
   Slots14x15 S;
   for ( int s = 0; s < 14; ++s )
      for ( int k = 0; k < 15; ++k )
         S.w[s][k] = w_slots[15 * s + k];
   const int N = ( 1 << level ) + 1;
   hipLaunchKernelGGL( p1_apply_shell_send_kernel, dim3( shell_blocks( N ) ), dim3( kThreads ), 0, as_stream( stream ), dst, src, N,
                       mask & HYTEG_HIP_MASK_SHELL, update, S, send_first, send_list, peers, npeers, seq, counter );
   HH_CHECK_HIP( hipGetLastError() );
   return HYTEG_HIP_OK;
}

HYTEG_HIP_API int hyteg_hip_p1_vector_cell_masked( int                  op,
                                                   double*              dst,
                                                   int                  nsrc,
                                                   const double* const* srcs,
                                                   const double*        scalars,
                                                   int                  level,
                                                   unsigned             mask,
                                                   hyteg_hip_stream_t   stream )
{
   HH_REQUIRE( dst && srcs, "p1_vector_cell_masked: null pointer" );
   HH_REQUIRE( op >= 0 && op <= 2, "p1_vector_cell_masked: op must be 0 (assign), 1 (add) or 2 (mult)" );
   HH_REQUIRE( any_level_ok( level ), "p1_vector_cell_masked: level out of range [0,11]" );
   HH_REQUIRE( nsrc >= 1 && nsrc <= HYTEG_HIP_MAX_SRCS, "p1_vector_cell_masked: nsrc must be 1..HYTEG_HIP_MAX_SRCS" );
   HH_REQUIRE( op == 2 || scalars != nullptr, "p1_vector_cell_masked: null scalars" );
   for ( int k = 0; k < nsrc; ++k )
      HH_REQUIRE( srcs[k] != nullptr, "p1_vector_cell_masked: null source pointer" );
   if ( ( mask & HYTEG_HIP_MASK_ALL ) == HYTEG_HIP_MASK_ALL && level <= 10 )
   {
      VecArgsM A{};
      A.dst = dst;
      for ( int k = 0; k < nsrc; ++k )
      {
         A.src[k] = srcs[k];
         A.c[k]   = scalars ? scalars[k] : 1.0;
// ... 266 lines not shown
```

hyteg_amd/host.py:

```python
from __future__ import annotations

import ctypes as C
from pathlib import Path

import numpy as np

_PKG = Path(__file__).resolve().parent
_LIB_PATH = _PKG / "lib" / "libhyteg_host.so"

Inner, DirichletBoundary, NeumannBoundary, FreeslipBoundary, All, Boundary = 1, 2, 4, 8, 15, 14
Replace, Add = 0, 1
JACOBI, GAUSS_SEIDEL, SOR, JACOBI_FP32 = 0, 1, 2, 3
CHEBYSHEV = 4

_vp, _i, _d, _u = C.c_void_p, C.c_int, C.c_double, C.c_uint
_ip, _dp = C.POINTER(C.c_int), C.POINTER(C.c_double)
EXCHANGE_CB = C.CFUNCTYPE(_i, _vp, _i, _i)
ALLREDUCE_CB = C.CFUNCTYPE(_i, _vp, _dp, _i)

SIGNATURES = {
    "hyteg_host_last_error": (C.c_char_p, []),
    "hyteg_host_storage_from_gmsh": (_i, [C.c_char_p, _i, _i, C.POINTER(_vp)]),
    "hyteg_host_storage_from_arrays": (_i, [_i, _dp, _i, _ip, _i, _i, C.POINTER(_vp)]),
    "hyteg_host_storage_destroy": (_i, [_vp]),
    "hyteg_host_storage_counts": (_i, [_vp, _ip]),
    "hyteg_host_storage_local_cell": (_i, [_vp, _i, _ip, _dp, _dp]),
    "hyteg_host_storage_mask": (_i, [_vp, _i, _i, _i, C.POINTER(_u)]),
    "hyteg_host_storage_set_boundary_type": (_i, [_vp, _i]),
    "hyteg_host_storage_set_stream": (_i, [_vp, _vp]),
    "hyteg_host_storage_set_batch_max_level": (_i, [_vp, _i]),
    "hyteg_host_storage_set_apply_lanes": (_i, [_vp, _i]),
    "hyteg_host_storage_set_apply_cell_lanes_min": (_i, [_vp, _i]),
    "hyteg_host_storage_lanes_seen": (_i, [_vp, C.POINTER(C.c_uint)]),
    "hyteg_host_storage_set_apply_steps": (_i, [_vp, _i]),
    "hyteg_host_storage_steps_launches": (_i, [_vp, C.POINTER(_u)]),
    "hyteg_host_apply_steps_plan": (_i, [_i, C.POINTER(C.c_ulonglong), C.POINTER(C.c_ulonglong), _i, _i, _i, _i, _ip, _ip]),
    "hyteg_host_lane_plan": (_i, [_i, _i, _ip, C.POINTER(C.c_ulonglong), _ip, C.POINTER(C.c_ulonglong), _ip, C.POINTER(_u)]),
    "hyteg_host_storage_set_hooks": (_i, [_vp, EXCHANGE_CB, EXCHANGE_CB, ALLREDUCE_CB, _vp]),
    "hyteg_host_storage_use_rccl": (_i, [_vp, C.c_char_p]),
    "hyteg_host_storage_use_p2p": (_i, [_vp, C.c_size_t, C.c_char_p, C.POINTER(C.c_int)]),
    "hyteg_host_storage_p2p_open": (_i, [_vp, C.c_char_p]),
    "hyteg_host_storage_p2p_layout": (_i, [_vp, _i, _i, C.POINTER(C.c_longlong)]),
    "hyteg_host_storage_p2p_connect": (_i, [_vp, _i, _i, C.POINTER(C.c_longlong)]),
    "hyteg_host_storage_drop_p2p": (_i, [_vp]),
    "hyteg_host_storage_check_transport": (_i, [_vp]),
    "hyteg_host_storage_transport_name": (_i, [_vp, C.c_char_p, _i]),
    "hyteg_host_storage_allreduce_sum": (_i, [_vp, _dp, _i]),
    "hyteg_host_storage_enable_timing": (_i, [_vp, _i, _i]),
    "hyteg_host_storage_timing_json": (_i, [_vp, C.c_char_p, C.c_size_t, C.POINTER(C.c_size_t)]),
    "hyteg_host_storage_timing_reset": (_i, [_vp]),
    "hyteg_host_plan_sizes": (_i, [_vp, _i, _i, _ip]),
    "hyteg_host_plan_export": (_i, [_vp, _i, _i, _ip, _ip, _ip, _ip, _ip, _ip, _ip, _ip]),
    "hyteg_host_plan_register_buffers": (_i, [_vp, _i, _i, _vp, _vp]),
    "hyteg_host_function_create": (_i, [_vp, C.c_char_p, _i, _i, C.POINTER(_vp)]),
    "hyteg_host_function_destroy": (_i, [_vp]),
    "hyteg_host_function_cell_pointer": (_i, [_vp, _i, _i, C.POINTER(_vp)]),
    "hyteg_host_function_upload_cell": (_i, [_vp, _i, _i, _dp]),
    "hyteg_host_function_download_cell": (_i, [_vp, _i, _i, _dp]),
    "hyteg_host_function_interpolate_constant": (_i, [_vp, _d, _i, _i]),
    "hyteg_host_function_assign": (_i, [_vp, _i, _dp, C.POINTER(_vp), _i, _i]),
    "hyteg_host_function_add": (_i, [_vp, _i, _dp, C.POINTER(_vp), _i, _i]),
    "hyteg_host_function_mult_elementwise": (_i, [_vp, _i, C.POINTER(_vp), _i, _i]),
    "hyteg_host_function_dot": (_i, [_vp, _vp, _i, _i, _i, _dp]),
    "hyteg_host_function_sum_shared": (_i, [_vp, _i, _i]),
    "hyteg_host_function_sync_shared": (_i, [_vp, _i, _i]),
    "hyteg_host_function_set_all_inner": (_i, [_vp, _i]),
    "hyteg_host_th_function_create": (_i, [_vp, C.c_char_p, _i, _i, C.POINTER(_vp)]),
    "hyteg_host_th_function_destroy": (_i, [_vp]),
    "hyteg_host_th_function_velocity": (_i, [_vp, _i, C.POINTER(_vp)]),
    "hyteg_host_th_function_pressure": (_i, [_vp, C.POINTER(_vp)]),
    "hyteg_host_th_function_assign": (_i, [_vp, _i, _dp, C.POINTER(_vp), _i, _i]),
    "hyteg_host_th_function_interpolate_constant": (_i, [_vp, _d, _i, _i]),
    "hyteg_host_th_function_dot": (_i, [_vp, _vp, _i, _i, C.POINTER(_d)]),
    "hyteg_host_th_operator_create": (_i, [_vp, _i, _i, C.POINTER(_vp)]),
    "hyteg_host_th_operator_destroy": (_i, [_vp]),
    "hyteg_host_th_operator_apply": (_i, [_vp, _vp, _vp, _i, _i]),
    "hyteg_host_th_operator_apply_block": (_i, [_vp, _i, _vp, _vp, _i, _i]),
    "hyteg_host_th_gmg_create": (_i, [_vp, _i, _i, _d, _i, _i, _i, _i, _d, C.POINTER(_vp)]),
    "hyteg_host_th_minres_create": (_i, [_vp, _i, _i, _i, _d, C.POINTER(_vp)]),
    "hyteg_host_th_solver_solve": (_i, [_vp, _vp, _vp, _vp, _i]),
    "hyteg_host_th_solver_destroy": (_i, [_vp]),
    "hyteg_host_th_project_pressure_mean": (_i, [_vp, _i]),
    "hyteg_host_th_form_element_matrix": (_i, [_i, _i, _dp, _dp]),
    "hyteg_host_stokes_function_create": (_i, [_vp, C.c_char_p, _i, _i, C.POINTER(_vp)]),
    "hyteg_host_stokes_function_destroy": (_i, [_vp]),
    "hyteg_host_stokes_function_component": (_i, [_vp, _i, C.POINTER(_vp)]),
    "hyteg_host_stokes_function_assign": (_i, [_vp, _i, _dp, C.POINTER(_vp), _i, _i]),
    "hyteg_host_stokes_function_dot": (_i, [_vp, _vp, _i, _i, _dp]),
    "hyteg_host_project_mean": (_i, [_vp, _i]),
    "hyteg_host_stokes_operator_create": (_i, [_vp, _i, _i, C.POINTER(_vp)]),
    "hyteg_host_stokes_operator_destroy": (_i, [_vp]),
    "hyteg_host_stokes_operator_apply": (_i, [_vp, _vp, _vp, _i, _i]),
    "hyteg_host_stokes_uzawa_create": (_i, [_vp, _i, _i, _d, _i, _i, _d, C.POINTER(_vp)]),
    "hyteg_host_stokes_gmg_create": (_i, [_vp, _vp, _i, _i, _i, _i, _i, _i, C.POINTER(_vp)]),
    "hyteg_host_stokes_gmg_create_with_coarse": (_i, [_vp, _vp, _i, _i, _i, _i, _i, _i, _i, _i, _d, C.POINTER(_vp)]),
    "hyteg_host_stokes_minres_create": (_i, [_vp, _i, _i, _i, _d, _i, _i, C.POINTER(_vp)]),
    "hyteg_host_stokes_minres_iterations": (_i, [_vp, C.POINTER(_i)]),
    "hyteg_host_solver_create_minres": (_i, [_vp, _i, _i, _i, _d, _i, C.POINTER(_vp)]),
    "hyteg_host_stokes_solver_solve": (_i, [_vp, _vp, _vp, _vp, _i]),
    "hyteg_host_stokes_solver_destroy": (_i, [_vp]),
    "hyteg_host_operator_create": (_i, [_vp, _i, _i, _i, C.POINTER(_vp)]),
    "hyteg_host_operator_destroy": (_i, [_vp]),
    "hyteg_host_operator_stencils": (_i, [_vp, _i, _i, _dp, _dp]),
    "hyteg_host_operator_apply": (_i, [_vp, _vp, _vp, _i, _i, _i]),
    "hyteg_host_operator_apply_cycle": (_i, [_vp, _i, C.POINTER(_vp), C.POINTER(_vp), _i, _i, _i, _i, _i]),
    "hyteg_host_operator_apply_cycle_timed": (_i, [_vp, _i, C.POINTER(_vp), C.POINTER(_vp), _i, _i, _i, _i, _i, _vp, _vp]),
    "hyteg_host_operator_smooth_jac": (_i, [_vp, _vp, _vp, _vp, _d, _i, _i]),
    "hyteg_host_operator_smooth_sor": (_i, [_vp, _vp, _vp, _d, _i, _i, _i]),
    "hyteg_host_operator_smooth_sor_many": (_i, [_vp, _i, C.POINTER(_vp), C.POINTER(_vp), _d, _i, _i, _i]),
    "hyteg_host_operator_compute_inverse_diagonal": (_i, [_vp]),
    "hyteg_host_operator_inverse_diagonal": (_i, [_vp, C.POINTER(_vp)]),
    "hyteg_host_elementwise_create": (_i, [_vp, _i, _i, C.POINTER(_vp)]),
    "hyteg_host_elementwise_destroy": (_i, [_vp]),
    "hyteg_host_elementwise_apply": (_i, [_vp, _vp, _vp, _i, _i, _i]),
    "hyteg_host_elementwise_compute_inverse_diagonal": (_i, [_vp]),
    "hyteg_host_elementwise_inverse_diagonal": (_i, [_vp, C.POINTER(_vp)]),
    "hyteg_host_elementwise_smooth_jac": (_i, [_vp, _vp, _vp, _vp, _d, _i, _i]),
    "hyteg_host_restrict": (_i, [_vp, _i, _i]),
# ... 93 lines not shown
    _ck(lib().hyteg_host_chebyshev_coefficients(int(order), float(lower), float(upper), out.ctypes.data_as(_dp)), "chebyshev_coefficients")
    return out


def estimate_radius(op, level: int, max_iter: int, x, tmp) -> float:
    r = _d()
    fn = lib().hyteg_host_p2_chebyshev_estimate_radius if isinstance(op, P2ElementwiseLaplaceOperator) else lib().hyteg_host_chebyshev_estimate_radius
    _ck(fn(op.h, int(level), int(max_iter), x.h, tmp.h, C.byref(r)), "chebyshev_estimate_radius")
    return r.value


def cell_size(level: int) -> int:
    n = (1 << level) + 1
    return n * (n + 1) * (n + 2) // 6


class Storage:

    def __init__(self, handle):
        self.h = handle
        self._hooks = None
        self.stream = 0
        c = (C.c_int * 6)()
        _ck(lib().hyteg_host_storage_counts(self.h, c), "storage_counts")
        self.n_cells, self.n_faces, self.n_edges, self.n_vertices, self.n_local_cells, self.n_ranks = list(c)

    @classmethod
    def from_gmsh(cls, path, rank=0, nranks=1):
        h = _vp()
        _ck(lib().hyteg_host_storage_from_gmsh(str(path).encode(), rank, nranks, C.byref(h)), "storage_from_gmsh")
        return cls(h)

    @classmethod
    def from_arrays(cls, vertices, cells, rank=0, nranks=1):
        v = np.ascontiguousarray(vertices, dtype=np.float64).reshape(-1, 3)
        c = np.ascontiguousarray(cells, dtype=np.int32).reshape(-1, 4)
        h = _vp()
        _ck(lib().hyteg_host_storage_from_arrays(len(v), v.ctypes.data_as(_dp), len(c), c.ctypes.data_as(_ip), rank, nranks,
                                                 C.byref(h)), "storage_from_arrays")
        return cls(h)

    @classmethod
    def single_tet(cls, coords):
        return cls.from_arrays(coords, [[0, 1, 2, 3]])

    def local_cell(self, i):
        gid = C.c_int()
        co = np.empty(12)
        nnc = np.empty(14)
        _ck(lib().hyteg_host_storage_local_cell(self.h, i, C.byref(gid), co.ctypes.data_as(_dp), nnc.ctypes.data_as(_dp)),
            "storage_local_cell")
        return gid.value, co.reshape(4, 3), nnc

    def mask(self, i, flag, owned=False):
        m = _u()
        _ck(lib().hyteg_host_storage_mask(self.h, i, flag, int(owned), C.byref(m)), "storage_mask")
        return m.value

    def set_boundary_type(self, t):
        _ck(lib().hyteg_host_storage_set_boundary_type(self.h, t), "set_boundary_type")

    def set_batch_max_level(self, level):
        _ck(lib().hyteg_host_storage_set_batch_max_level(self.h, level), "set_batch_max_level")

    def set_apply_steps(self, steps):
        _ck(lib().hyteg_host_storage_set_apply_steps(self.h, steps), "set_apply_steps")

    def set_apply_lanes(self, lanes):
        _ck(lib().hyteg_host_storage_set_apply_lanes(self.h, lanes), "set_apply_lanes")

    def set_apply_cell_lanes_min(self, cells):
        _ck(lib().hyteg_host_storage_set_apply_cell_lanes_min(self.h, cells), "set_apply_cell_lanes_min")

    def lanes_seen(self):
        m = C.c_uint()
        _ck(lib().hyteg_host_storage_lanes_seen(self.h, C.byref(m)), "lanes_seen")
        return m.value

    def steps_launches(self):
        n = C.c_uint()
        _ck(lib().hyteg_host_storage_steps_launches(self.h, C.byref(n)), "steps_launches")
        return n.value

    def set_stream(self, stream):
        _ck(lib().hyteg_host_storage_set_stream(self.h, stream), "set_stream")
        self.stream = int(stream) if stream else 0

    def set_hooks(self, exchange_begin, exchange_end, allreduce_sum):

        def guard(fn):
            def call(user, *args):
                global _hook_exception
                try:
                    fn(*args)
                    return 0
                except BaseException as e:
                    _hook_exception = e
                    return 1
            return call

        exb, exe, ar = EXCHANGE_CB(guard(exchange_begin)), EXCHANGE_CB(guard(exchange_end)), ALLREDUCE_CB(guard(allreduce_sum))
        self._hooks = (exb, exe, ar)
        _ck(lib().hyteg_host_storage_set_hooks(self.h, exb, exe, ar, None), "set_hooks")

    def use_rccl(self, unique_id: bytes):
        if len(unique_id) != 128:
            raise ValueError("use_rccl: the unique id has 128 bytes")
        _ck(lib().hyteg_host_storage_use_rccl(self.h, bytes(unique_id)), "storage_use_rccl")

    def use_p2p(self, arena_bytes: int):
        buf = C.create_string_buffer(64)
        kind = C.c_int(0)
        _ck(lib().hyteg_host_storage_use_p2p(self.h, int(arena_bytes), buf, C.byref(kind)), "storage_use_p2p")
        return buf.raw, kind.value

    def p2p_open(self, handles):
        blob = b"".join(bytes(h) for h in handles)
        _ck(lib().hyteg_host_storage_p2p_open(self.h, blob), "storage_p2p_open")

    def p2p_layout(self, level: int, key: int, npeers: int):
        o = np.zeros((max(npeers, 1), 3), dtype=np.int64)
        _ck(lib().hyteg_host_storage_p2p_layout(self.h, level, key, o.ctypes.data_as(C.POINTER(C.c_longlong))), "storage_p2p_layout")
        return o[:npeers]

    def p2p_connect(self, level: int, key: int, offsets):
        o = np.ascontiguousarray(offsets, dtype=np.int64).reshape(-1, 3)
        o = o if len(o) else np.zeros((1, 3), dtype=np.int64)
        _ck(lib().hyteg_host_storage_p2p_connect(self.h, level, key, o.ctypes.data_as(C.POINTER(C.c_longlong))), "storage_p2p_connect")

    def drop_p2p(self):
        _ck(lib().hyteg_host_storage_drop_p2p(self.h), "storage_drop_p2p")

    def check_transport(self):
        _ck(lib().hyteg_host_storage_check_transport(self.h), "storage_check_transport")

    def allreduce_sum(self, values):
        a = np.ascontiguousarray(values, dtype=np.float64).copy()
        _ck(lib().hyteg_host_storage_allreduce_sum(self.h, a.ctypes.data_as(_dp), len(a)), "storage_allreduce_sum")
        return a

    def enable_timing(self, on=True, synchronize=False):
        _ck(lib().hyteg_host_storage_enable_timing(self.h, int(on), int(synchronize)), "storage_enable_timing")

    def timing_json(self) -> str:
        need = C.c_size_t()
        _ck(lib().hyteg_host_storage_timing_json(self.h, None, 0, C.byref(need)), "storage_timing_json")
        buf = C.create_string_buffer(need.value)
        _ck(lib().hyteg_host_storage_timing_json(self.h, buf, need.value, None), "storage_timing_json")
        return buf.value.decode()

    def timing_reset(self):
        _ck(lib().hyteg_host_storage_timing_reset(self.h), "storage_timing_reset")

    @property
    def transport(self) -> str:
        buf = C.create_string_buffer(32)
        _ck(lib().hyteg_host_storage_transport_name(self.h, buf, 32), "storage_transport_name")
        return buf.value.decode()

    def plan(self, level, key):
        cls = key
        s = (C.c_int * 5)()
        _ck(lib().hyteg_host_plan_sizes(self.h, level, cls, s), "plan_sizes")
        ng, ne, npeer, ts, tr = list(s)
        a = lambda n: np.zeros(max(n, 1), dtype=np.int32)
        gp, eb, eo, peers, sc, rc, sb, so = a(ng + 1), a(ne), a(ne), a(npeer), a(npeer), a(npeer), a(ts), a(ts)
# ... 611 lines not shown
```

hyteg_amd/host/hyteg_host_capi.cpp:

```cpp
#include "hyteg_host.hpp"

#include <variant>

#include "../../include/hyteg_host.h"

using namespace hyteg;

namespace {
thread_local std::string g_err;

struct StorageH
{
   std::shared_ptr< PrimitiveStorage > p;
};
struct FunctionH
{
   std::shared_ptr< P1Function< double > > p;
};
struct OperatorH
{
   std::variant< std::shared_ptr< P1ConstantLaplaceOperator >, std::shared_ptr< P1ConstantMassOperator >, std::shared_ptr< P1DivxOperator >,
                 std::shared_ptr< P1DivyOperator >, std::shared_ptr< P1DivzOperator >, std::shared_ptr< P1DivTxOperator >,
                 std::shared_ptr< P1DivTyOperator >, std::shared_ptr< P1DivTzOperator >, std::shared_ptr< P1PSPGOperator > >
             op;
// ... 198 lines not shown
   if ( nRadii == 1 )
      sm->setupCoefficients( (uint_t) order, radii[0], upper, lower );
   else
      sm->setupCoefficients( (uint_t) order, std::vector< double >( radii, radii + nRadii ), upper, lower );
   return sm;
}
}

extern "C" {

HYTEG_HOST_API const char* hyteg_host_last_error( void ) { return g_err.c_str(); }

HYTEG_HOST_API int hyteg_host_storage_from_gmsh( const char* path, int rank, int nranks, hh_storage_t* out )
{
   return guarded( [&] { *out = new StorageH{ std::make_shared< PrimitiveStorage >( MeshInfo::fromGmshFile( path ), rank, nranks ) }; } );
}
HYTEG_HOST_API int hyteg_host_storage_from_arrays( int nv, const double* xyz, int nc, const int* cells, int rank, int nranks, hh_storage_t* out )
{
   return guarded( [&] { *out = new StorageH{ std::make_shared< PrimitiveStorage >( MeshInfo::fromArrays( nv, xyz, nc, cells ), rank, nranks ) }; } );
}
HYTEG_HOST_API int hyteg_host_storage_destroy( hh_storage_t s )
{
   return guarded( [&] { delete static_cast< StorageH* >( s ); } );
}
HYTEG_HOST_API int hyteg_host_storage_counts( hh_storage_t s, int* c )
{
   return guarded( [&] {
      auto& st = S( s );
      c[0]     = (int) st.getCells().size();
      c[1]     = (int) st.getFaces().size();
      c[2]     = (int) st.getEdges().size();
      c[3]     = (int) st.getVertices().size();
      c[4]     = (int) st.getNumberOfLocalCells();
      c[5]     = st.numRanks();
   } );
}
HYTEG_HOST_API int hyteg_host_storage_local_cell( hh_storage_t s, int li, int* gid, double* coords12, double* nnc14 )
{
   return guarded( [&] {
      const MacroCell& c = S( s ).getLocalCell( (uint_t) li );
      if ( gid )
         *gid = c.id;
      if ( coords12 )
         for ( int v = 0; v < 4; ++v )
            for ( int r = 0; r < 3; ++r )
               coords12[3 * v + r] = c.coords[v][r];
      if ( nnc14 )
      {
         auto n = S( s ).numNeighborCells( c );
         std::copy( n.begin(), n.end(), nnc14 );
      }
   } );
}
HYTEG_HOST_API int hyteg_host_storage_mask( hh_storage_t s, int li, int flag, int owned, unsigned* mask )
{
   return guarded( [&] {
      const MacroCell& c = S( s ).getLocalCell( (uint_t) li );
      *mask              = owned ? S( s ).ownedMaskFor( c, DoFType( flag ) ) : S( s ).maskFor( c, DoFType( flag ) );
   } );
}
HYTEG_HOST_API int hyteg_host_storage_set_boundary_type( hh_storage_t s, int t )
{
   return guarded( [&] { S( s ).setBoundaryType( DoFType( t ) ); } );
}
HYTEG_HOST_API int hyteg_host_storage_set_stream( hh_storage_t s, void* stream )
{
   return guarded( [&] { S( s ).setStream( stream ); } );
}
HYTEG_HOST_API int hyteg_host_storage_set_batch_max_level( hh_storage_t s, int level )
{
   return guarded( [&] { S( s ).setBatchMaxLevel( level ); } );
}
HYTEG_HOST_API int hyteg_host_storage_set_apply_lanes( hh_storage_t s, int lanes )
{
   return guarded( [&] { S( s ).setApplyLanes( lanes ); } );
}
HYTEG_HOST_API int hyteg_host_storage_set_apply_steps( hh_storage_t s, int steps )
{
   return guarded( [&] { S( s ).setApplySteps( steps ); } );
}
HYTEG_HOST_API int hyteg_host_storage_steps_launches( hh_storage_t s, unsigned* count )
{
   return guarded( [&] { *count = S( s ).stepsLaunchesSeen(); } );
}
HYTEG_HOST_API int hyteg_host_storage_set_apply_cell_lanes_min( hh_storage_t s, int cells )
{
   return guarded( [&] { S( s ).setApplyCellLanesMin( cells ); } );
}
HYTEG_HOST_API int hyteg_host_storage_lanes_seen( hh_storage_t s, unsigned* mask )
{
   return guarded( [&] { *mask = S( s ).lanesSeen(); } );
}
HYTEG_HOST_API int hyteg_host_lane_plan( int lanes, int nsteps, const int* read_ptr, const unsigned long long* read_ids, const int* write_ptr,
                                         const unsigned long long* write_ids, int* lane_out, unsigned* waits_out )
{
   return guarded( [&] {
      if ( nsteps < 0 || ( nsteps > 0 && ( !read_ptr || !write_ptr || !lane_out || !waits_out ) ) )
         throw std::runtime_error( "lane_plan: null argument" );
      LanePlanner                 planner( lanes );
      std::vector< const void* > r, w;
      for ( int k = 0; k < nsteps; ++k )
      {
         r.clear(), w.clear();
         for ( int i = read_ptr[k]; i < read_ptr[k + 1]; ++i )
            r.push_back( reinterpret_cast< const void* >( (uintptr_t) read_ids[i] ) );
         for ( int i = write_ptr[k]; i < write_ptr[k + 1]; ++i )
            w.push_back( reinterpret_cast< const void* >( (uintptr_t) write_ids[i] ) );
         const auto p = planner.place( r.data(), (int) r.size(), w.data(), (int) w.size() );
         lane_out[k] = p.lane, waits_out[k] = p.waits;
      }
   } );
}
HYTEG_HOST_API int hyteg_host_apply_steps_plan( int npairs, const unsigned long long* src_ids, const unsigned long long* dst_ids, int first, int steps,
                                                int max_group, int lanes, int* sizes_out, int* ngroups_out )
{
   return guarded( [&] {
      if ( npairs < 1 || steps < 0 || first < 0 || !src_ids || !dst_ids || !ngroups_out || ( steps > 0 && !sizes_out ) )
         throw std::runtime_error( "apply_steps_plan: bad argument" );
      std::vector< const void* > u( (size_t) steps ), d( (size_t) steps );
      for ( int k = 0; k < steps; ++k )
      {
         const int j   = (int) ( ( (long long) first + k ) % npairs );
         u[(size_t) k] = reinterpret_cast< const void* >( (uintptr_t) src_ids[j] );
         d[(size_t) k] = reinterpret_cast< const void* >( (uintptr_t) dst_ids[j] );
      }
      const std::vector< int > sizes = planApplySteps( u.data(), d.data(), steps, max_group, lanes );
      std::copy( sizes.begin(), sizes.end(), sizes_out );
      *ngroups_out = (int) sizes.size();
   } );
}
HYTEG_HOST_API int hyteg_host_storage_use_rccl( hh_storage_t s, const unsigned char* unique_id )
{
   return guarded( [&] {
      if ( !unique_id )
         throw std::runtime_error( "storage_use_rccl: null unique id" );
      S( s ).useRccl( unique_id );
   } );
}
HYTEG_HOST_API int hyteg_host_storage_use_p2p( hh_storage_t s, size_t arena_bytes, unsigned char* handle, int* arena_kind )
{
   return guarded( [&] {
      if ( !handle )
         throw std::runtime_error( "storage_use_p2p: null handle buffer" );
      P2PTransport& T = S( s ).useP2P( arena_bytes );
      std::copy( T.handle().begin(), T.handle().end(), handle );
      if ( arena_kind )
         *arena_kind = T.arenaKind();
   } );
}
HYTEG_HOST_API int hyteg_host_storage_p2p_open( hh_storage_t s, const unsigned char* handles )
{
   return guarded( [&] {
      if ( !handles )
         throw std::runtime_error( "storage_p2p_open: null handles" );
      S( s ).p2p().openPeers( handles );
   } );
}
HYTEG_HOST_API int hyteg_host_storage_p2p_layout( hh_storage_t s, int level, int key, long long* offsets )
{
   return guarded( [&] {
      const auto& plan = S( s ).devicePlan( level, key & 1, key >> 1 );
      const auto  o    = S( s ).p2p().layoutPlan( plan, level, key );
      if ( !o.empty() && !offsets )
         throw std::runtime_error( "storage_p2p_layout: null offsets" );
      std::copy( o.begin(), o.end(), offsets );
   } );
// ... 821 lines not shown
```

hyteg_amd/host/p1operator.hpp:

```cpp
#pragma once

#include "forms.hpp"
#include "p1function.hpp"

namespace hyteg {

template < class Form >
class P1ConstantOperator
{
 public:
   using srcType = P1Function< double >;
   using dstType = P1Function< double >;
   using FunctionList = std::vector< std::reference_wrapper< const P1Function< double > > >;

   P1ConstantOperator( const std::shared_ptr< PrimitiveStorage >& storage, uint_t minLevel, uint_t maxLevel )
   : storage_( storage )
   , minLevel_( minLevel )
   , maxLevel_( maxLevel )
   {
      for ( uint_t l = minLevel; l <= maxLevel; ++l )
      {
         std::vector< stencil::CellStencils > perCell;
         for ( const auto& cell : storage->getCells() )
            perCell.push_back( stencil::assemble< Form >( cell, l ) );
         stencils_[l] = perCell;
         sorTables_[l] = buildSorTables( perCell );
         if ( l >= HYTEG_HIP_MIN_LEVEL )
            hipCheck( hyteg_hip_prepare_level( (int) l ), "P1ConstantOperator: prepare_level" );
      }
   }

   std::shared_ptr< PrimitiveStorage > getStorage() const { return storage_; }
   uint64_t                            uid() const { return uid_; }
   uint_t                              getMinLevel() const { return minLevel_; }
   uint_t                              getMaxLevel() const { return maxLevel_; }
   const stencil::CellStencils&        getCellStencils( int globalCellID, uint_t level ) const { return stencils_.at( level ).at( globalCellID ); }

   void apply( const P1Function< double >& src, const P1Function< double >& dst, uint_t level, DoFType flagIn, UpdateType updateType = Replace ) const
   {
      ScopedTimer timerOp( storage_->getTimingTree(), "Operator P1Function to P1Function" ), timerApply( storage_->getTimingTree(), "Apply" );
      const DoFType flag = dst.effectiveFlag( flagIn );
      if ( &src == &dst )
         throw std::runtime_error( "P1ConstantOperator::apply: src and dst must differ (P1Operator.hpp:198)" );
      if ( storage_->lanesOpen() )
      {
         if ( pureInterior( level, flag ) )
         {
            storage_->forLocalCells( [&]( uint_t c, const MacroCell& cell ) {
               if ( !( storage_->maskFor( cell, flag ) & HYTEG_HIP_MASK_INNER ) )
                  return;
               double*            d    = dst.getCellPointer( c, level );
               const double*      u    = src.getCellPointer( c, level );
               const void*        r[1] = { u };
               const void*        w[1] = { d };
               hyteg_hip_stream_t lane = storage_->laneFor( r, 1, w, 1 );
               hipCheck( hyteg_hip_p1_apply_cell( d, u, (int) level, getCellStencils( cell.id, level ).inner, hipUpdate( updateType ), lane ),
                         "apply: cell" );
            } );
            return;
         }
         storage_->joinLanes();
      }
      if ( storage_->useBatch( level ) )
      {
         applyBatched( src, dst, level, flag, updateType );
         return;
      }
      std::unique_ptr< P1Function< double > > tmp;
      if ( updateType == Add && hasSharedPoints( level, flag ) )
         tmp = P1Function< double >::zeroedScratch( "apply_tmp", storage_, level );
      const P1Function< double >& shellDst    = tmp ? *tmp : dst;
      const int                   shellUpdate = hipUpdate( tmp ? Replace : updateType );
      const bool                  sideChain = storage_->sideChainUsable( (int) level, flag, 0 );
      PrimitiveStorage::SideChain chain( *storage_, sideChain );
      PrimitiveStorage::LaneScope cellLanes( *storage_, !sideChain && storage_->applyCellLanesMin() > 0 && storage_->getNumberOfLocalCells() >= storage_->applyCellLanesMin() &&
                                                            level >= HYTEG_HIP_MIN_LEVEL );
      PrimitiveStorage::ShareSend send;
      const bool bySharesKernel = shellDst.beginSumSharedCopiesByShares( level, flag, send );
      storage_->forLocalCells( [&]( uint_t c, const MacroCell& cell ) {
         const auto& S = getCellStencils( cell.id, level );
         if ( bySharesKernel )
         {
            hipCheck( hyteg_hip_p1_apply_cell_boundary_p2p( shellDst.getCellPointer( c, level ), src.getCellPointer( c, level ), (int) level,
                                                            &S.slots[0][0], storage_->maskFor( cell, flag ), shellUpdate, send.first, send.list,
                                                            send.a.peers, send.a.npeers, send.a.seq, send.a.counter, storage_->stream() ),
                      "apply: boundary + send" );
            return;
         }
         hipCheck( hyteg_hip_p1_apply_cell_boundary( shellDst.getCellPointer( c, level ), src.getCellPointer( c, level ), (int) level,
                                                     &S.slots[0][0], storage_->maskFor( cell, flag ), shellUpdate, storage_->stream() ),
                   "apply: boundary" );
      } );
      if ( !bySharesKernel )
         shellDst.beginSumSharedCopies( level, flag );
      chain.toMain();
      storage_->forLocalCells( [&]( uint_t c, const MacroCell& cell ) {
         const unsigned mask = storage_->maskFor( cell, flag );
         if ( ( mask & HYTEG_HIP_MASK_INNER ) && level >= HYTEG_HIP_MIN_LEVEL )
            hipCheck( hyteg_hip_p1_apply_cell( dst.getCellPointer( c, level ), src.getCellPointer( c, level ), (int) level,
                                               getCellStencils( cell.id, level ).inner, hipUpdate( updateType ),
                                               cellLanes.active() ? storage_->laneStream( (int) c + 1 ) : storage_->stream() ),
                      "apply: cell" );
      } );
      cellLanes.join();
      chain.toSide();
      shellDst.endSumSharedCopies( level, flag );
      chain.join();
      if ( tmp )
         dst.addOnShell( *tmp, level, flag );
   }

   void applyRun( const std::vector< const P1Function< double >* >& srcs, const std::vector< const P1Function< double >* >& dsts, uint_t level,
                  DoFType flagIn, UpdateType updateType = Replace ) const
   {
      const int n       = (int) srcs.size();
      const int G       = storage_->applySteps();
      storage_->resetStepsLaunches();
      bool      grouped = G > 1 && n > 1 && level <= 8 && storage_->getNumberOfLocalCells() == 1 && storage_->applyStepsUsable();
      for ( int k = 0; k < n && grouped; ++k )
      {
         const DoFType flag = dsts[k]->effectiveFlag( flagIn );
         grouped            = srcs[k] != dsts[k] && pureInterior( level, flag );
         storage_->forLocalCells( [&]( uint_t, const MacroCell& cell ) { grouped = grouped && ( storage_->maskFor( cell, flag ) & HYTEG_HIP_MASK_INNER ); } );
      }
      if ( !grouped )
      {
         for ( int k = 0; k < n; ++k )
            apply( *srcs[k], *dsts[k], level, flagIn, updateType );
         return;
      }
      std::vector< const void* > u( (size_t) n );
      std::vector< void* >       d( (size_t) n );
      const double*              stencil = nullptr;
      storage_->forLocalCells( [&]( uint_t c, const MacroCell& cell ) {
         stencil = getCellStencils( cell.id, level ).inner;
         for ( int k = 0; k < n; ++k )
         {
            u[(size_t) k] = srcs[k]->getCellPointer( c, level );
            d[(size_t) k] = dsts[k]->getCellPointer( c, level );
         }
      } );
      const int upd = hipUpdate( updateType );
      int       k   = 0;
      for ( const int g : planApplySteps( u.data(), d.data(), n, G, storage_->lanesOpen() ? storage_->applyLanes() : 1 ) )
      {
         const void* const* r = u.data() + k;
         void* const*       w = d.data() + k;
         hyteg_hip_stream_t s = storage_->lanesOpen() ? storage_->laneFor( r, g, w, g ) : storage_->stream();
         int                rc = g > 1 ? hyteg_hip_p1_apply_cell_steps( w, r, g, (int) level, stencil, upd, s ) : HYTEG_HIP_ENOTSUP;
         if ( g > 1 && rc == HYTEG_HIP_OK )
            storage_->countStepsLaunch();
         if ( rc == HYTEG_HIP_ENOTSUP )
         {
            rc = HYTEG_HIP_OK;
            for ( int i = 0; i < g && rc == HYTEG_HIP_OK; ++i )
               rc = hyteg_hip_p1_apply_cell( static_cast< double* >( w[i] ), static_cast< const double* >( r[i] ), (int) level, stencil, upd, s );
         }
         hipCheck( rc, "applyRun: cell" );
         k += g;
      }
   }

   void residual( const P1Function< double >& x, const P1Function< double >& b, const P1Function< double >& r, uint_t level, DoFType flagIn ) const
   {
      const DoFType flag = r.effectiveFlag( flagIn );
      if ( !pureInterior( level, flag ) || level > 10 || &x == &r )
      {
         apply( x, r, level, flagIn );
         r.assign( { 1.0, -1.0 }, { b, r }, level, flagIn );
         return;
      }
      ScopedTimer timerOp( storage_->getTimingTree(), "Operator P1Function to P1Function" ), timerApply( storage_->getTimingTree(), "Apply" );
      storage_->forLocalCells( [&]( uint_t c, const MacroCell& cell ) {
         if ( storage_->maskFor( cell, flag ) & HYTEG_HIP_MASK_INNER )
            hipCheck( hyteg_hip_p1_residual_cell( r.getCellPointer( c, level ), b.getCellPointer( c, level ), x.getCellPointer( c, level ),
                                                  (int) level, getCellStencils( cell.id, level ).inner, storage_->stream() ),
                      "residual: cell" );
      } );
   }

   void smooth_jac( const P1Function< double >& dst, const P1Function< double >& rhs, const P1Function< double >& src, double relax,
                    uint_t level, DoFType flagIn ) const
   {
      ScopedTimer timerOp( storage_->getTimingTree(), "Operator P1Function to P1Function" ), timerJac( storage_->getTimingTree(), "smooth_jac" );
      const DoFType flag = dst.effectiveFlag( flagIn );
      if ( &src == &dst )
// ... 346 lines not shown
            if ( c.v[q] == g )
               return q;
         throw std::runtime_error( "slotOf: primitive is not part of the cell" );
      };
      if ( p.v.size() == 1 )
         return 10 + local( p.v[0] );
      if ( p.v.size() == 2 )
      {
         int a = local( p.v[0] ), b = local( p.v[1] );
         if ( a > b )
            std::swap( a, b );
         for ( int e = 0; e < 6; ++e )
            if ( kCellEdgeVerts[e][0] == a && kCellEdgeVerts[e][1] == b )
               return e;
      }
      int l[3] = { local( p.v[0] ), local( p.v[1] ), local( p.v[2] ) };
      std::sort( l, l + 3 );
      for ( int f = 0; f < 4; ++f )
         if ( kCellFaceVerts[f][0] == l[0] && kCellFaceVerts[f][1] == l[1] && kCellFaceVerts[f][2] == l[2] )
            return 6 + f;
      throw std::runtime_error( "slotOf: not found" );
   }

 private:
   void applyBatched( const P1Function< double >& src, const P1Function< double >& dst, uint_t level, DoFType flag, UpdateType updateType ) const
   {
      const bool sharedAdd = updateType == Add && hasSharedPoints( level, flag );
      auto       run       = [&]( const P1Function< double >& out, unsigned keep, int update ) {
         const auto masks = storage_->masksFor( flag, false, keep );
         storage_->forCellChunks( [&]( int first, int count ) {
            const auto d = out.cellPointers( level, first, count ), u = src.cellPointers( level, first, count );
            hipCheck( hyteg_hip_p1_apply_cells( count, d.data(), u.data(), (int) level, stencilTable( level ) + (size_t) first * 225,
                                                masks.data() + first, update, storage_->stream() ),
                      "apply (batched)" );
         } );
      };
      if ( !sharedAdd )
      {
         run( dst, HYTEG_HIP_MASK_ALL, hipUpdate( updateType ) );
         dst.sumSharedCopies( level, flag );
         return;
      }
      const auto tmp = P1Function< double >::zeroedScratch( "apply_tmp", storage_, level );
      run( dst, HYTEG_HIP_MASK_INNER, HYTEG_HIP_ADD );
      run( *tmp, HYTEG_HIP_MASK_SHELL, HYTEG_HIP_REPLACE );
      tmp->sumSharedCopies( level, flag );
      const auto masks = storage_->masksFor( flag, false, HYTEG_HIP_MASK_SHELL );
      storage_->forCellChunks( [&]( int first, int count ) {
         const auto   d = dst.cellPointers( level, first, count ), t = tmp->cellPointers( level, first, count );
         const double one = 1.0;
         hipCheck( hyteg_hip_p1_vector_cells( 1, count, d.data(), 1, t.data(), &one, (int) level, masks.data() + first, storage_->stream() ),
                   "apply: add shell (batched)" );
      } );
   }
 public:
   bool canCgSolveSmall( uint_t level ) const
   {
      const size_t n = storage_->getNumberOfLocalCells();
      return storage_->numRanks() == 1 && n >= 1 && n <= HYTEG_HIP_MAX_BATCH &&
             (int64_t) n * layout::cellSize( (int) level ) <= hyteg_hip_p1_cg_small_max_entries();
   }
   void cgSolveSmall( const P1Function< double >& x, const P1Function< double >& b, uint_t level, DoFType flagIn, uint_t maxIter, double relTol,
                      double absTol, double* infoDev ) const
   {
      const DoFType flag = x.effectiveFlag( flagIn );
      const int  count = (int) storage_->getNumberOfLocalCells();
      const auto masks = storage_->masksFor( flag ), owned = storage_->masksFor( flag, true );
      const auto xs = x.cellPointers( level, 0, count ), bs = b.cellPointers( level, 0, count );
      const int* gp[2] = { nullptr, nullptr }, *ec[2] = { nullptr, nullptr }, *eo[2] = { nullptr, nullptr };
      int        ng[2] = { 0, 0 };
      for ( int cls = 0; cls < 2; ++cls )
      {
         if ( !testFlag( storage_->boundaryTypeOf( cls == 1 ), flag ) || storage_->exchangePlan( (int) level, cls ).ngroups() == 0 )
            continue;
         const auto& plan = storage_->devicePlan( (int) level, cls );
         gp[cls] = plan.dGroupPtr, ec[cls] = plan.dEntryBuf, eo[cls] = plan.dEntryOff, ng[cls] = plan.ngroups();
      }
      hipCheck( hyteg_hip_p1_cg_small_cells( count, xs.data(), bs.data(), (int) level, stencilTable( level ), masks.data(), owned.data(), gp, ec,
                                             eo, ng, (int) maxIter, relTol, absTol, infoDev, storage_->stream() ),
                "cgSolveSmall" );
   }

 private:
   template < typename T, typename Build >
   const T* deviceTable( std::map< std::pair< uint_t, uint_t >, const T* >& cache, uint_t level, uint_t nf, Build&& hostTable ) const
   {
      const auto key = std::make_pair( level, nf );
      const auto it  = cache.find( key );
      if ( it != cache.end() )
         return it->second;
      const std::vector< T > once = hostTable();
      std::vector< T >       h;
      for ( uint_t k = 0; k < nf; ++k )
         h.insert( h.end(), once.begin(), once.end() );
      return cache[key] = static_cast< const T* >( storage_->uploadBytes( h.data(), h.size() * sizeof( T ) ) );
   }
   const double* stencilTable( uint_t level, uint_t nf = 1 ) const
   {
      return deviceTable( stencilTables_, level, nf, [&] { return stencilTableHost( level ); } );
   }
   const double* restTable( uint_t level, uint_t nf = 1 ) const
   {
      return deviceTable( restTables_, level, nf, [&] { return restTableHost( level ); } );
   }
   const hyteg_hip_sor_shell_tables* shellTable( uint_t level, uint_t nf = 1 ) const
   {
      return deviceTable( shellTables_, level, nf, [&] { return shellTableHost( level ); } );
   }
   std::vector< double > stencilTableHost( uint_t level ) const
   {
      std::vector< double > h;
      for ( int id : storage_->getLocalCellIDs() )
      {
         const auto& S = getCellStencils( id, level );
         h.insert( h.end(), &S.slots[0][0], &S.slots[0][0] + 14 * 15 );
         h.insert( h.end(), S.inner, S.inner + 15 );
      }
      return h;
   }
   std::vector< double > restTableHost( uint_t level ) const
   {
      std::vector< double > h;
      for ( int id : storage_->getLocalCellIDs() )
      {
         const auto& T = sorTables_.at( level ).at( id );
         h.insert( h.end(), &T.rest[0][0], &T.rest[0][0] + 14 * 15 );
         h.insert( h.end(), 15, 0.0 );
      }
      return h;
   }
   std::vector< hyteg_hip_sor_shell_tables > shellTableHost( uint_t level ) const
   {
      std::vector< hyteg_hip_sor_shell_tables > h;
      for ( int id : storage_->getLocalCellIDs() )
      {
         const auto&                T = sorTables_.at( level ).at( id );
         hyteg_hip_sor_shell_tables r{};
         std::memcpy( r.edge_verts, T.edgeVerts, sizeof( r.edge_verts ) );
         std::memcpy( r.face_verts, T.faceVerts, sizeof( r.face_verts ) );
         std::memcpy( r.edge_w, T.edgeW, sizeof( r.edge_w ) );
         std::memcpy( r.face_w, T.faceW, sizeof( r.face_w ) );
         std::memcpy( r.vertex_w, T.vertexW, sizeof( r.vertex_w ) );
         h.push_back( r );
      }
      return h;
   }
   std::vector< stencil::CellSorTables > buildSorTables( const std::vector< stencil::CellStencils >& S ) const
   {
      using namespace stencil;
      const auto&                   cells = storage_->getCells();
      std::vector< CellSorTables >  T( cells.size() );
      std::vector< std::array< double, 3 > > edgeTot( storage_->getEdges().size(), std::array< double, 3 >{} );
      std::vector< std::array< double, 7 > > faceTot( storage_->getFaces().size(), std::array< double, 7 >{} );
      std::vector< double >                  vertTot( storage_->getVertices().size(), 0.0 );
      for ( const auto& c : cells )
      {
         CellSorTables& t = T[c.id];
         for ( int s = 0; s < 14; ++s )
            for ( int k = 0; k < 15; ++k )
               t.rest[s][k] = k == C ? 0.0 : S[c.id].slots[s][k];
         for ( int k = 0; k < 4; ++k )
            vertTot[c.v[k]] += S[c.id].slots[10 + k][C];
         for ( int e = 0; e < 6; ++e )
         {
            int lo = kCellEdgeVerts[e][0], hi = kCellEdgeVerts[e][1];
            if ( c.v[lo] > c.v[hi] )
               std::swap( lo, hi );
            const int kp = offsetIndex( kUnit[hi][0] - kUnit[lo][0], kUnit[hi][1] - kUnit[lo][1], kUnit[hi][2] - kUnit[lo][2] );
            const int km = offsetIndex( kUnit[lo][0] - kUnit[hi][0], kUnit[lo][1] - kUnit[hi][1], kUnit[lo][2] - kUnit[hi][2] );
            t.edgeVerts[e][0] = lo, t.edgeVerts[e][1] = hi;
            auto& tot = edgeTot[c.edges[e]];
            tot[0] += S[c.id].slots[e][C], tot[1] += S[c.id].slots[e][km], tot[2] += S[c.id].slots[e][kp];
            t.rest[e][km] = t.rest[e][kp] = 0.0;
         }
         for ( int f = 0; f < 4; ++f )
         {
            int l[3] = { kCellFaceVerts[f][0], kCellFaceVerts[f][1], kCellFaceVerts[f][2] };
            std::sort( l, l + 3, [&]( int a, int b ) { return c.v[a] < c.v[b]; } );
            auto& tot = faceTot[c.faces[f]];
            tot[0] += S[c.id].slots[6 + f][C];
            for ( int d = 0; d < 6; ++d )
            {
               int o[3];
               for ( int r = 0; r < 3; ++r )
                  o[r] = kFaceDirs[d][0] * ( kUnit[l[1]][r] - kUnit[l[0]][r] ) + kFaceDirs[d][1] * ( kUnit[l[2]][r] - kUnit[l[0]][r] );
               const int k = offsetIndex( o[0], o[1], o[2] );
               tot[1 + d] += S[c.id].slots[6 + f][k];
               t.rest[6 + f][k] = 0.0;
            }
            for ( int r = 0; r < 3; ++r )
               t.faceVerts[f][r] = l[r];
         }
      }
      for ( const auto& c : cells )
      {
         CellSorTables& t = T[c.id];
         for ( int k = 0; k < 4; ++k )
            t.vertexW[k] = vertTot[c.v[k]];
         for ( int e = 0; e < 6; ++e )
            for ( int k = 0; k < 3; ++k )
               t.edgeW[e][k] = edgeTot[c.edges[e]][k];
         for ( int f = 0; f < 4; ++f )
            for ( int k = 0; k < 7; ++k )
               t.faceW[f][k] = faceTot[c.faces[f]][k];
      }
      return T;
   }
   bool pureInterior( uint_t level, DoFType flag ) const
   {
      return storage_->numRanks() == 1 && !storage_->useBatch( level ) && level >= HYTEG_HIP_MIN_LEVEL && !storage_->anyShellSelected( flag );
   }
   bool hasSharedPoints( uint_t level, DoFType flag ) const
   {
      for ( int cls = 0; cls < 2; ++cls )
         if ( testFlag( storage_->boundaryTypeOf( cls == 1 ), flag ) && storage_->exchangePlan( (int) level, cls ).ngroups() > 0 )
            return true;
      return false;
   }

   std::shared_ptr< PrimitiveStorage >                        storage_;
   uint_t                                                     minLevel_, maxLevel_;
   uint64_t                                                   uid_ = nextUid();
   std::map< uint_t, std::vector< stencil::CellStencils > >   stencils_;
   std::map< uint_t, std::vector< stencil::CellSorTables > >  sorTables_;
   mutable std::map< std::pair< uint_t, uint_t >, std::unique_ptr< P1Function< double > > > sorRest_;
   mutable std::map< std::pair< uint_t, uint_t >, const double* >                         stencilTables_, restTables_;
   mutable std::map< std::pair< uint_t, uint_t >, const hyteg_hip_sor_shell_tables* >     shellTables_;
   std::shared_ptr< P1Function< double > >                    inverseDiagonalValues_;
};

using P1ConstantLaplaceOperator = P1ConstantOperator< forms::P1LaplaceForm >;
using P1ConstantMassOperator    = P1ConstantOperator< forms::P1MassForm >;

}
```

hyteg_amd/host/storage.hpp:

```cpp
#pragma once

#include "comm.hpp"
#include "lanes.hpp"
#include "mesh.hpp"
#include "timing.hpp"

namespace hyteg {

struct MacroCell
{
   int                      id;
   std::array< int, 4 >     v;
   std::array< Point3D, 4 > coords;
   std::array< int, 6 >     edges;
   std::array< int, 4 >     faces;
   int                      rank;
   int                      localIndex;
};
struct MacroPrimitive
{
   std::vector< int > v;
   std::vector< int > cells;
   bool               onBoundary = false;
   uint_t             getNumNeighborCells() const { return cells.size(); }
// ... 233 lines not shown
   }
   double* uploadTable( const std::vector< double >& h ) const
   {
      return static_cast< double* >( uploadBytes( h.data(), h.size() * sizeof( double ) ) );
   }
   template < typename F >
   void forCellChunks( F&& fn ) const
   {
      const int n = (int) localCells_.size();
      for ( int first = 0; first < n; first += HYTEG_HIP_MAX_BATCH )
         fn( first, std::min( HYTEG_HIP_MAX_BATCH, n - first ) );
   }

   void              setStream( hyteg_hip_stream_t s )
   {
      joinLanes();
      stream_ = s;
      if ( timingTree_ )
         timingTree_->setStream( s );
   }
   void enableTiming( bool on, bool synchronize = false )
   {
      if ( !on )
      {
         timingTree_.reset();
         return;
      }
      if ( !timingTree_ )
         timingTree_ = std::make_shared< TimingTree >();
      timingTree_->setSynchronize( synchronize, stream_ );
   }
   TimingTree* getTimingTree() const { return timingTree_.get(); }
   hyteg_hip_stream_t stream() const
   {
      if ( laneUsed_ )
         joinLanes();
      return stream_;
   }

   void setApplyLanes( int lanes )
   {
      if ( lanes < 0 || lanes > LanePlanner::kMaxLanes )
         throw std::runtime_error( "setApplyLanes: 0 (default) to " + std::to_string( LanePlanner::kMaxLanes ) + " lanes" );
      if ( laneDepth_ > 0 )
         throw std::runtime_error( "setApplyLanes: a lane scope is open" );
      laneCount_ = lanes == 0 ? -1 : lanes;
   }
   int applyLanes() const
   {
      if ( laneCount_ < 0 )
      {
         static const int fromEnv = [] {
            const char* e = std::getenv( "HYTEG_AMD_APPLY_LANES" );
            const int   n = e ? std::atoi( e ) : 2;
            return std::min( std::max( n, 1 ), (int) LanePlanner::kMaxLanes );
         }();
         laneCount_ = fromEnv;
      }
      return laneCount_;
   }
   static constexpr int kMaxApplySteps = 16, kDefaultApplySteps = 16;
   void                 setApplySteps( int steps )
   {
      if ( steps < 0 || steps > kMaxApplySteps )
         throw std::runtime_error( "setApplySteps: 0 (default) to " + std::to_string( kMaxApplySteps ) + " steps per launch" );
      applySteps_ = steps == 0 ? -1 : steps;
   }
   int applySteps() const
   {
      if ( applySteps_ < 0 )
      {
         static const int fromEnv = [] {
            const char* e = std::getenv( "HYTEG_AMD_APPLY_STEPS" );
            const int   n = e ? std::atoi( e ) : kDefaultApplySteps;
            return std::min( std::max( n, 1 ), kMaxApplySteps );
         }();
         applySteps_ = fromEnv;
      }
      return applySteps_;
   }
   unsigned stepsLaunchesSeen() const { return stepsLaunches_; }
   void     resetStepsLaunches() const { stepsLaunches_ = 0; }
   void     countStepsLaunch() const { ++stepsLaunches_; }
   bool applyStepsUsable() const
   {
      if ( nranks_ != 1 || mainStream_ || timingTree_ )
         return false;
      if ( lanesOpen() )
         return true;
      int capturing = 0;
      return hyteg_hip_stream_is_capturing( stream_, &capturing ) == HYTEG_HIP_OK && !capturing;
   }
   void   setApplyCellLanesMin( int cells ) { cellLanesMin_ = cells < 0 ? -1 : cells; }
   uint_t applyCellLanesMin() const
   {
      if ( cellLanesMin_ < 0 )
      {
         static const int fromEnv = [] {
            const char* e = std::getenv( "HYTEG_AMD_APPLY_CELL_LANES_MIN" );
            return e ? std::max( 0, std::atoi( e ) ) : 24;
         }();
         cellLanesMin_ = fromEnv;
      }
      return (uint_t) cellLanesMin_;
   }
   unsigned lanesSeen() const { return lanesSeen_; }
   bool lanesOpen() const { return laneDepth_ > 0 && lanesOn_; }
   hyteg_hip_stream_t laneFor( const void* const* reads, int nReads, const void* const* writes, int nWrites ) const
   {
      if ( laneManual_ )
         joinLanes();
      const LanePlanner::Placement p = planner_.place( reads, nReads, writes, nWrites );
      hyteg_hip_stream_t           s = useLane( p.lane );
      lanesSeen_ |= 1u << p.lane;
      for ( int j = 0; j < planner_.lanes(); ++j )
         if ( p.waits & ( 1u << j ) )
         {
            hipCheck( hyteg_hip_event_record( laneEvents_[j], j == 0 ? stream_ : laneStreams_[j] ), "lanes: record" );
            hipCheck( hyteg_hip_stream_wait_event( s, laneEvents_[j] ), "lanes: wait" );
         }
      return s;
   }
   hyteg_hip_stream_t laneStream( int lane ) const
   {
      laneManual_ = true;
      lane %= planner_.lanes();
      lanesSeen_ |= 1u << lane;
      return useLane( lane );
   }
   void joinLanes() const
   {
      const unsigned used = laneUsed_;
      laneUsed_ = 0, laneManual_ = false;
      planner_.reset();
      for ( int l = 1; l < LanePlanner::kMaxLanes; ++l )
         if ( used & ( 1u << l ) )
         {
            hipCheck( hyteg_hip_event_record( laneEvents_[l], laneStreams_[l] ), "lanes: record" );
            hipCheck( hyteg_hip_stream_wait_event( stream_, laneEvents_[l] ), "lanes: wait" );
         }
   }
   class LaneScope
   {
    public:
      explicit LaneScope( const PrimitiveStorage& st, bool want = true )
      : st_( st )
      {
         if ( st_.laneDepth_ == 0 )
         {
            st_.lanesSeen_ = 0;
            st_.lanesOn_   = want && st_.nranks_ == 1 && st_.applyLanes() > 1 && !st_.mainStream_ && !st_.timingTree_;
            if ( st_.lanesOn_ )
            {
               int capturing = 0;
               if ( hyteg_hip_stream_is_capturing( st_.stream_, &capturing ) != HYTEG_HIP_OK || capturing )
                  st_.lanesOn_ = false;
            }
            if ( st_.lanesOn_ && st_.planner_.lanes() != st_.applyLanes() )
               st_.planner_.setLanes( st_.applyLanes() );
            st_.planner_.reset();
         }
         ++st_.laneDepth_;
         use_ = want && st_.lanesOn_;
      }
      bool active() const { return use_; }
      int  lanes() const { return use_ ? st_.planner_.lanes() : 1; }
// ... 549 lines not shown

      std::vector< int > recvCursor( P.peers.size(), 0 );
      P.groupPtr.push_back( 0 );
      forAllPrimitives( [&]( const MacroPrimitive& p ) {
         bool local;
         if ( !involves( p, local ) || !local )
            return;
         pointsOf( p, [&]( const int* w, const int* wb ) {
            for ( int c : p.cells )
            {
               const MacroCell& cell = cells_[c];
               if ( cell.rank == rank_ )
               {
                  const int off = dofKind == 1 ? (int) edgeIndexInCell( cell, p, w, wb, level ) : (int) indexInCell( cell, p, w, N );
                  P.entryBuf.push_back( cell.localIndex );
                  P.entryOff.push_back( off );
                  std::set< int > dests;
                  for ( int c2 : p.cells )
                     if ( cells_[c2].rank != rank_ )
                        dests.insert( cells_[c2].rank );
                  for ( int d : dests )
                  {
                     sendBufPer[peerSlot[d]].push_back( cell.localIndex );
                     sendOffPer[peerSlot[d]].push_back( off );
                  }
               }
               else
               {
                  const int s = peerSlot[cell.rank];
                  P.entryBuf.push_back( nLocal + s );
                  P.entryOff.push_back( recvCursor[s]++ );
               }
            }
            P.groupPtr.push_back( (int) P.entryBuf.size() );
         } );
      } );
      for ( uint_t s = 0; s < P.peers.size(); ++s )
      {
         P.recvCount[s] = recvCursor[s];
         P.sendCount[s] = (int) sendBufPer[s].size();
         P.sendBuf.insert( P.sendBuf.end(), sendBufPer[s].begin(), sendBufPer[s].end() );
         P.sendOff.insert( P.sendOff.end(), sendOffPer[s].begin(), sendOffPer[s].end() );
      }
      return P;
   }

   int                                                     rank_, nranks_;
   std::vector< MacroCell >                                cells_;
   std::vector< MacroPrimitive >                           faces_, edges_, vertices_;
   std::vector< int >                                      localCells_;
   DoFType                                                 boundaryType_ = DirichletBoundary;
   mutable hyteg_hip_stream_t                              stream_       = nullptr;
   mutable hyteg_hip_stream_t                              sideStream_ = nullptr, mainStream_ = nullptr;
   mutable hyteg_hip_event_t                               forked_ = nullptr, joined_ = nullptr;
   mutable int                                             sideEnabled_ = -1;
   hyteg_hip_stream_t useLane( int lane ) const
   {
      if ( lane == 0 )
         return stream_;
      if ( !laneStreams_[lane] )
      {
         hipCheck( hyteg_hip_stream_create( &laneStreams_[lane] ), "lanes: stream_create" );
         hipCheck( hyteg_hip_event_create( &laneEvents_[lane] ), "lanes: event_create" );
      }
      if ( !laneEvents_[0] )
      {
         hipCheck( hyteg_hip_event_create( &laneEvents_[0] ), "lanes: event_create" );
         hipCheck( hyteg_hip_event_create( &laneFork_ ), "lanes: event_create" );
      }
      if ( !( laneUsed_ & ( 1u << lane ) ) )
      {
         if ( !laneUsed_ )
            hipCheck( hyteg_hip_event_record( laneFork_, stream_ ), "lanes: fork" );
         hipCheck( hyteg_hip_stream_wait_event( laneStreams_[lane], laneFork_ ), "lanes: fork wait" );
         laneUsed_ |= 1u << lane;
      }
      return laneStreams_[lane];
   }
   mutable LanePlanner                                     planner_;
   mutable hyteg_hip_stream_t                              laneStreams_[LanePlanner::kMaxLanes] = {};
   mutable hyteg_hip_event_t                               laneEvents_[LanePlanner::kMaxLanes]  = {}, laneFork_ = nullptr;
   mutable int                                             laneCount_ = -1, laneDepth_ = 0, applySteps_ = -1;
   mutable int                                             cellLanesMin_ = -1;
   mutable unsigned                                        laneUsed_  = 0, lanesSeen_ = 0, stepsLaunches_ = 0;
   mutable bool                                            lanesOn_ = false, laneManual_ = false;
   std::shared_ptr< Transport >                            transport_;
   std::shared_ptr< TimingTree >                           timingTree_;
   mutable void *                                          dotResult_ = nullptr, *dotWorkspace_ = nullptr;
   mutable std::map< size_t, std::vector< double* > >      scratchFree_;
   mutable std::vector< void* >                            scratchAll_;
   mutable std::map< std::vector< double* >, double** >    pointerTables_;
   mutable std::map< std::pair< int, int >, ShareSendTable > shareSendTables_;
   mutable double*                                         nncInv_        = nullptr;
   mutable int                                             batchMaxLevel_ = -2;
   static constexpr int                                    kBatchSingleMaxLevelDefault = -1;
   mutable int                                             batchSingleMaxLevel_        = kBatchSingleMaxLevelDefault;
   mutable std::map< std::pair< int, int >, ExchangePlan > plans_;
};

}
```

include/hyteg_hip.h:

```cpp
#ifndef HYTEG_HIP_H
#define HYTEG_HIP_H

#include <stddef.h>
#include <stdint.h>

#ifdef __cplusplus
extern "C" {
#endif

#if defined( HYTEG_HIP_BUILDING )
#define HYTEG_HIP_API __attribute__( ( visibility( "default" ) ) )
#else
#define HYTEG_HIP_API
#endif

enum
{
   HYTEG_HIP_OK      = 0,
   HYTEG_HIP_EINVAL  = 1,
   HYTEG_HIP_ELAUNCH = 2,
   HYTEG_HIP_ENOMEM  = 3,
   HYTEG_HIP_ENODEV  = 4,
   HYTEG_HIP_ENOTSUP = 5
};

enum
{
   HYTEG_HIP_REPLACE = 0,
   HYTEG_HIP_ADD     = 1
};

#define HYTEG_HIP_MIN_LEVEL 2
#define HYTEG_HIP_MAX_LEVEL 11
#define HYTEG_HIP_MAX_SRCS 4

typedef void* hyteg_hip_stream_t;

HYTEG_HIP_API const char* hyteg_hip_version( void );
HYTEG_HIP_API const char* hyteg_hip_last_error( void );
HYTEG_HIP_API int         hyteg_hip_device_count( int* count );
HYTEG_HIP_API int         hyteg_hip_set_device( int device );
HYTEG_HIP_API int hyteg_hip_device_name( char* buf, size_t buflen );

HYTEG_HIP_API int hyteg_hip_malloc( void** dev_ptr, size_t bytes );
HYTEG_HIP_API int hyteg_hip_free( void* dev_ptr );
HYTEG_HIP_API int hyteg_hip_memset_zero( void* dev_ptr, size_t bytes, hyteg_hip_stream_t stream );
HYTEG_HIP_API int hyteg_hip_upload( void* dev_dst, const void* host_src, size_t bytes, hyteg_hip_stream_t stream );
HYTEG_HIP_API int hyteg_hip_download( void* host_dst, const void* dev_src, size_t bytes, hyteg_hip_stream_t stream );
HYTEG_HIP_API int hyteg_hip_copy( void* dev_dst, const void* dev_src, size_t bytes, hyteg_hip_stream_t stream );
HYTEG_HIP_API int hyteg_hip_calib_copy( double* dst, const double* src, int64_t n, int nontemporal, hyteg_hip_stream_t stream );
typedef void* hyteg_hip_event_t;
HYTEG_HIP_API int hyteg_hip_calib_copy_ring( double* const* dsts, const double* const* srcs, int npairs, int64_t n, int nontemporal, int first,
                                             int count, hyteg_hip_stream_t stream, hyteg_hip_event_t start, hyteg_hip_event_t stop );
HYTEG_HIP_API int hyteg_hip_stream_create( hyteg_hip_stream_t* stream );
HYTEG_HIP_API int hyteg_hip_stream_destroy( hyteg_hip_stream_t stream );
HYTEG_HIP_API int hyteg_hip_stream_synchronize( hyteg_hip_stream_t stream );

typedef void* hyteg_hip_graph_t;
HYTEG_HIP_API int hyteg_hip_graph_begin_capture( hyteg_hip_stream_t stream );
HYTEG_HIP_API int hyteg_hip_graph_end_capture( hyteg_hip_stream_t stream, hyteg_hip_graph_t* graph );
HYTEG_HIP_API int hyteg_hip_graph_abort_capture( hyteg_hip_stream_t stream );
HYTEG_HIP_API int hyteg_hip_stream_is_capturing( hyteg_hip_stream_t stream, int* capturing );
HYTEG_HIP_API int hyteg_hip_graph_launch( hyteg_hip_graph_t graph, hyteg_hip_stream_t stream );
HYTEG_HIP_API int hyteg_hip_graph_destroy( hyteg_hip_graph_t graph );

HYTEG_HIP_API int hyteg_hip_prepare_level( int level );

HYTEG_HIP_API int64_t hyteg_hip_cell_width( int level );
HYTEG_HIP_API int64_t hyteg_hip_cell_size( int level );
HYTEG_HIP_API int64_t hyteg_hip_cell_inner_size( int level );
HYTEG_HIP_API int64_t hyteg_hip_cell_index( int level, int x, int y, int z );

HYTEG_HIP_API int hyteg_hip_p1_apply_cell( double*            dst,
                                           const double*      src,
                                           int                level,
                                           const double*      w ,
                                           int                update,
                                           hyteg_hip_stream_t stream );
HYTEG_HIP_API int hyteg_hip_p1_apply_cell_steps( void* const*       dsts ,
                                                 const void* const* srcs ,
                                                 int                nsteps,
                                                 int                level,
                                                 const double*      w ,
                                                 int                update,
                                                 hyteg_hip_stream_t stream );

HYTEG_HIP_API int hyteg_hip_p1_apply_cell_f32( float* dst, const float* src, int level, const double* w , int update, hyteg_hip_stream_t stream );
HYTEG_HIP_API int hyteg_hip_p1_jacobi_cell_f32( float*             dst,
                                                const float*       rhs,
                                                const float*       src,
                                                const float*       invdiag ,
                                                int                level,
                                                const double*      w ,
                                                double             relax,
                                                hyteg_hip_stream_t stream );
HYTEG_HIP_API int hyteg_hip_convert_f64_to_f32( float* dst, const double* src, size_t n, hyteg_hip_stream_t stream );
HYTEG_HIP_API int hyteg_hip_convert_f32_to_f64( double* dst, const float* src, size_t n, hyteg_hip_stream_t stream );
HYTEG_HIP_API int hyteg_hip_axpy_f32_into_f64( double* y, const float* x, double alpha, size_t n, hyteg_hip_stream_t stream );

HYTEG_HIP_API int hyteg_hip_p1_residual_jacobi_start_f32( float* r_f32, float* e_f32, const double* rhs, const double* src, int level, const double* w,
                                                          double relax, hyteg_hip_stream_t stream );
HYTEG_HIP_API int hyteg_hip_p1_jacobi_accumulate_f32( double* x, const float* rhs_f32, const float* e_f32, int level, const double* w, double relax,
                                                      hyteg_hip_stream_t stream );

HYTEG_HIP_API int hyteg_hip_p1_apply_kernel_name( int level, int update, char* buf, size_t buflen );
HYTEG_HIP_API int hyteg_hip_set_apply_shape( int ny, int lz, int pfd );

HYTEG_HIP_API int hyteg_hip_p1_jacobi_cell( double*            dst,
                                            const double*      rhs,
                                            const double*      src,
                                            const double*      invdiag ,
                                            int                level,
                                            const double*      w ,
                                            double             relax,
                                            hyteg_hip_stream_t stream );

HYTEG_HIP_API int hyteg_hip_p1_chebyshev_start_cell( double*            t_out,
                                                     const double*      rhs,
                                                     const double*      x,
                                                     const double*      invdiag ,
                                                     int                level,
                                                     const double*      w ,
                                                     hyteg_hip_stream_t stream );
HYTEG_HIP_API int hyteg_hip_p1_chebyshev_step_cell( double*            t_out,
                                                    double*            x,
                                                    const double*      t_in,
                                                    const double*      invdiag ,
                                                    int                level,
                                                    const double*      w ,
                                                    double             c_prev,
                                                    double             c_cur,
                                                    int                has_prev,
                                                    hyteg_hip_stream_t stream );

enum hyteg_hip_sor_algorithm
{
   HYTEG_HIP_SOR_AUTO     = 0,
   HYTEG_HIP_SOR_PLANES   = 1,
   HYTEG_HIP_SOR_BLOCKS   = 2,
   HYTEG_HIP_SOR_DATAFLOW = 3
};
HYTEG_HIP_API int hyteg_hip_set_sor_algorithm( int algorithm );

HYTEG_HIP_API int hyteg_hip_p1_sor_cell( double*            u,
                                         const double*      rhs,
                                         int                level,
                                         const double*      w ,
                                         double             relax,
                                         int                backwards,
                                         hyteg_hip_stream_t stream );
HYTEG_HIP_API int hyteg_hip_p1_sor_cell_sweeps( double*            u,
                                                const double*      rhs,
                                                int                level,
                                                const double*      w ,
                                                double             relax,
                                                int                backwards,
                                                int                nsweeps,
                                                hyteg_hip_stream_t stream );

HYTEG_HIP_API int hyteg_hip_p1_residual_cell( double*            dst,
                                              const double*      rhs,
                                              const double*      src,
                                              int                level,
                                              const double*      w ,
                                              hyteg_hip_stream_t stream );

HYTEG_HIP_API int hyteg_hip_p1_assign_cell( double*              dst,
                                            int                  nsrc,
                                            const double* const* srcs,
                                            const double*        scalars ,
                                            int                  level,
                                            hyteg_hip_stream_t   stream );
HYTEG_HIP_API int hyteg_hip_p1_add_cell( double*              dst,
                                         int                  nsrc,
                                         const double* const* srcs,
                                         const double*        scalars ,
                                         int                  level,
                                         hyteg_hip_stream_t   stream );
HYTEG_HIP_API int
    hyteg_hip_p1_mult_cell( double* dst, int nsrc, const double* const* srcs, int level, hyteg_hip_stream_t stream );

HYTEG_HIP_API size_t hyteg_hip_dot_workspace_bytes( void );
HYTEG_HIP_API int    hyteg_hip_p1_dot_cell( const double*      a,
                                            const double*      b,
                                            int                level,
                                            double*            result_dev,
                                            void*              workspace_dev,
                                            hyteg_hip_stream_t stream );

HYTEG_HIP_API int hyteg_hip_p1_restrict_cell( double*            coarse,
                                              const double*      fine,
                                              int                coarse_level,
                                              const double*      nnc ,
                                              hyteg_hip_stream_t stream );
HYTEG_HIP_API int hyteg_hip_p1_prolongate_cell( const double*      coarse,
                                                double*            fine,
                                                int                coarse_level,
                                                const double*      nnc ,
                                                int                update,
                                                hyteg_hip_stream_t stream );

#define HYTEG_HIP_SLOT_INNER 14
#define HYTEG_HIP_MASK_INNER ( 1u << 14 )
#define HYTEG_HIP_MASK_SHELL 0x3FFFu
#define HYTEG_HIP_MASK_ALL 0x7FFFu

HYTEG_HIP_API int hyteg_hip_p1_apply_cell_boundary( double*            dst,
                                                    const double*      src,
                                                    int                level,
                                                    const double*      w_slots ,
                                                    unsigned           mask,
                                                    int                update,
                                                    hyteg_hip_stream_t stream );

HYTEG_HIP_API int hyteg_hip_p1_vector_cell_masked( int                  op,
                                                   double*              dst,
                                                   int                  nsrc,
                                                   const double* const* srcs,
                                                   const double*        scalars ,
                                                   int                  level,
                                                   unsigned             mask,
                                                   hyteg_hip_stream_t   stream );
HYTEG_HIP_API int
    hyteg_hip_p1_set_cell_masked( double* dst, double value, int level, unsigned mask, hyteg_hip_stream_t stream );
HYTEG_HIP_API int hyteg_hip_p1_dot_cell_masked( const double*      a,
                                                const double*      b,
                                                int                level,
                                                unsigned           mask,
                                                double*            result_dev,
                                                void*              workspace_dev,
                                                hyteg_hip_stream_t stream );
HYTEG_HIP_API int hyteg_hip_p1_restrict_cell_masked( double*            coarse,
                                                     const double*      fine,
                                                     int                coarse_level,
                                                     const double*      nnc ,
                                                     unsigned           mask,
                                                     hyteg_hip_stream_t stream );
HYTEG_HIP_API int hyteg_hip_p1_prolongate_cell_masked( const double*      coarse,
                                                       double*            fine,
                                                       int                coarse_level,
                                                       const double*      nnc ,
                                                       unsigned           mask,
                                                       hyteg_hip_stream_t stream );
HYTEG_HIP_API int hyteg_hip_p1_prolongate_cell_masked_update( const double*      coarse,
                                                              double*            fine,
                                                              int                coarse_level,
                                                              const double*      nnc ,
                                                              unsigned           mask,
                                                              int                update,
                                                              hyteg_hip_stream_t stream );

HYTEG_HIP_API int hyteg_hip_p1_sor_shell_cell( double*            dst,
                                               const double*      rhs,
                                               double*            rest,
                                               int                level,
                                               const int*         edge_verts,
                                               const double*      edge_w,
                                               const int*         face_verts,
                                               const double*      face_w,
                                               const double*      vertex_w,
                                               double             relax,
                                               unsigned           mask,
                                               int                backwards,
                                               hyteg_hip_stream_t stream );

#define HYTEG_HIP_MAX_BATCH 80
HYTEG_HIP_API int hyteg_hip_p1_vector_cells( int                  op,
                                             int                  ncells,
                                             double* const*       dst,
                                             int                  nsrc,
                                             const double* const* srcs,
                                             const double*        scalars,
                                             int                  level,
                                             const unsigned*      masks,
                                             hyteg_hip_stream_t   stream );
HYTEG_HIP_API int hyteg_hip_p1_vector_cells_dev( int                  op,
                                                 int                  ncells,
                                                 double* const*       dst,
                                                 int                  nsrc,
                                                 const double* const* srcs,
                                                 const double* const* scalar_ptrs,
                                                 int                  level,
                                                 const unsigned*      masks,
                                                 hyteg_hip_stream_t   stream );
enum hyteg_hip_cg_slot
{
   HYTEG_HIP_CG_PRSOLD     = 0,
   HYTEG_HIP_CG_PAP        = 1,
   HYTEG_HIP_CG_RR         = 2,
   HYTEG_HIP_CG_ALPHA      = 3,
   HYTEG_HIP_CG_NEG_ALPHA  = 4,
   HYTEG_HIP_CG_BETA       = 5,
   HYTEG_HIP_CG_RES_START  = 6,
   HYTEG_HIP_CG_DONE       = 7,
   HYTEG_HIP_CG_ITERATIONS = 8,
   HYTEG_HIP_CG_ONE        = 9,
// ... 399 lines not shown
```

include/hyteg_host.h:

```cpp
#ifndef HYTEG_HOST_H
#define HYTEG_HOST_H
#include <stddef.h>
#include <stdint.h>
#ifdef __cplusplus
extern "C" {
#endif
#if defined( HYTEG_HOST_BUILDING )
#define HYTEG_HOST_API __attribute__( ( visibility( "default" ) ) )
#else
#define HYTEG_HOST_API
#endif

typedef void* hh_storage_t;
typedef void* hh_function_t;
typedef void* hh_operator_t;
typedef void* hh_solver_t;
typedef void* hh_p2function_t;
typedef void* hh_p2operator_t;
typedef void* hh_elementwise_t;
typedef void* hh_stokes_function_t;
typedef void* hh_stokes_operator_t;
typedef void* hh_stokes_solver_t;

HYTEG_HOST_API const char* hyteg_host_last_error( void );

HYTEG_HOST_API int hyteg_host_storage_from_gmsh( const char* path, int rank, int nranks, hh_storage_t* out );
HYTEG_HOST_API int hyteg_host_storage_from_arrays( int nvertices, const double* xyz, int ncells, const int* cells, int rank, int nranks, hh_storage_t* out );
HYTEG_HOST_API int hyteg_host_storage_destroy( hh_storage_t s );
HYTEG_HOST_API int hyteg_host_storage_counts( hh_storage_t s, int* counts );
HYTEG_HOST_API int hyteg_host_storage_local_cell( hh_storage_t s, int local_index, int* global_id, double* coords12, double* nnc14 );
HYTEG_HOST_API int hyteg_host_storage_mask( hh_storage_t s, int local_index, int flag, int owned, unsigned* mask );
HYTEG_HOST_API int hyteg_host_storage_set_boundary_type( hh_storage_t s, int dof_type );
HYTEG_HOST_API int hyteg_host_storage_set_stream( hh_storage_t s, void* stream );
HYTEG_HOST_API int hyteg_host_storage_set_batch_max_level( hh_storage_t s, int level );
HYTEG_HOST_API int hyteg_host_storage_set_apply_lanes( hh_storage_t s, int lanes );
HYTEG_HOST_API int hyteg_host_storage_set_apply_cell_lanes_min( hh_storage_t s, int cells );
HYTEG_HOST_API int hyteg_host_storage_lanes_seen( hh_storage_t s, unsigned* mask );
HYTEG_HOST_API int hyteg_host_lane_plan( int lanes, int nsteps, const int* read_ptr, const unsigned long long* read_ids, const int* write_ptr,
                                         const unsigned long long* write_ids, int* lane_out, unsigned* waits_out );
HYTEG_HOST_API int hyteg_host_storage_set_apply_steps( hh_storage_t s, int steps );
HYTEG_HOST_API int hyteg_host_storage_steps_launches( hh_storage_t s, unsigned* count );
HYTEG_HOST_API int hyteg_host_apply_steps_plan( int npairs, const unsigned long long* src_ids, const unsigned long long* dst_ids, int first, int steps,
                                                int max_group, int lanes, int* sizes_out, int* ngroups_out );
HYTEG_HOST_API int hyteg_host_storage_enable_timing( hh_storage_t s, int on, int synchronize );
HYTEG_HOST_API int hyteg_host_storage_timing_json( hh_storage_t s, char* buf, size_t buflen, size_t* needed );
HYTEG_HOST_API int hyteg_host_storage_timing_reset( hh_storage_t s );
HYTEG_HOST_API int hyteg_host_storage_use_rccl( hh_storage_t s, const unsigned char* unique_id );
HYTEG_HOST_API int hyteg_host_storage_transport_name( hh_storage_t s, char* buf, int buflen );
HYTEG_HOST_API int hyteg_host_storage_use_p2p( hh_storage_t s, size_t arena_bytes, unsigned char* handle, int* arena_kind );
HYTEG_HOST_API int hyteg_host_storage_p2p_open( hh_storage_t s, const unsigned char* handles );
HYTEG_HOST_API int hyteg_host_storage_p2p_layout( hh_storage_t s, int level, int key, long long* offsets );
HYTEG_HOST_API int hyteg_host_storage_p2p_connect( hh_storage_t s, int level, int key, const long long* offsets );
HYTEG_HOST_API int hyteg_host_storage_drop_p2p( hh_storage_t s );
HYTEG_HOST_API int hyteg_host_storage_check_transport( hh_storage_t s );
HYTEG_HOST_API int hyteg_host_storage_allreduce_sum( hh_storage_t s, double* values, int n );
HYTEG_HOST_API int hyteg_host_storage_set_hooks( hh_storage_t s, int ( *exchange_begin )( void*, int, int ),
                                                 int ( *exchange_end )( void*, int, int ),
                                                 int ( *allreduce_sum )( void*, double*, int ), void* user );
HYTEG_HOST_API int hyteg_host_plan_sizes( hh_storage_t s, int level, int key, int* sizes );
HYTEG_HOST_API int hyteg_host_plan_export( hh_storage_t s, int level, int key, int* group_ptr, int* entry_buf, int* entry_off,
                                           int* peers, int* send_count, int* recv_count, int* send_buf, int* send_off );
HYTEG_HOST_API int hyteg_host_plan_register_buffers( hh_storage_t s, int level, int key, double* send_dev, double* recv_dev );

HYTEG_HOST_API int hyteg_host_function_create( hh_storage_t s, const char* name, int min_level, int max_level, hh_function_t* out );
HYTEG_HOST_API int hyteg_host_function_destroy( hh_function_t f );
HYTEG_HOST_API int hyteg_host_function_cell_pointer( hh_function_t f, int local_cell, int level, double** dev_ptr );
HYTEG_HOST_API int hyteg_host_function_upload_cell( hh_function_t f, int local_cell, int level, const double* host );
HYTEG_HOST_API int hyteg_host_function_download_cell( hh_function_t f, int local_cell, int level, double* host );
HYTEG_HOST_API int hyteg_host_function_interpolate_constant( hh_function_t f, double value, int level, int flag );
HYTEG_HOST_API int hyteg_host_function_assign( hh_function_t dst, int n, const double* scalars, const hh_function_t* srcs, int level, int flag );
HYTEG_HOST_API int hyteg_host_function_add( hh_function_t dst, int n, const double* scalars, const hh_function_t* srcs, int level, int flag );
HYTEG_HOST_API int hyteg_host_function_mult_elementwise( hh_function_t dst, int n, const hh_function_t* srcs, int level, int flag );
HYTEG_HOST_API int hyteg_host_function_dot( hh_function_t a, hh_function_t b, int level, int flag, int global, double* result );
HYTEG_HOST_API int hyteg_host_function_sum_shared( hh_function_t f, int level, int flag );
HYTEG_HOST_API int hyteg_host_function_sync_shared( hh_function_t f, int level, int flag );
HYTEG_HOST_API int hyteg_host_function_set_all_inner( hh_function_t f, int on );

HYTEG_HOST_API int hyteg_host_operator_create( hh_storage_t s, int min_level, int max_level, int form, hh_operator_t* out );
HYTEG_HOST_API int hyteg_host_operator_destroy( hh_operator_t op );
HYTEG_HOST_API int hyteg_host_operator_stencils( hh_operator_t op, int global_cell, int level, double* inner15, double* slots210 );
HYTEG_HOST_API int hyteg_host_operator_apply( hh_operator_t op, hh_function_t src, hh_function_t dst, int level, int flag, int update );
HYTEG_HOST_API int hyteg_host_operator_apply_cycle( hh_operator_t op, int npairs, const hh_function_t* srcs, const hh_function_t* dsts,
                                                    int level, int flag, int update, int first, int steps );
HYTEG_HOST_API int hyteg_host_operator_apply_cycle_timed( hh_operator_t op, int npairs, const hh_function_t* srcs, const hh_function_t* dsts,
                                                          int level, int flag, int update, int first, int steps, void* ev_start, void* ev_stop );
HYTEG_HOST_API int hyteg_host_operator_smooth_jac( hh_operator_t op, hh_function_t dst, hh_function_t rhs, hh_function_t src, double relax, int level, int flag );
HYTEG_HOST_API int hyteg_host_operator_smooth_sor( hh_operator_t op, hh_function_t dst, hh_function_t rhs, double relax, int level, int flag, int backwards );
HYTEG_HOST_API int hyteg_host_operator_smooth_sor_many( hh_operator_t op, int n, const hh_function_t* dsts, const hh_function_t* rhss, double relax,
                                                        int level, int flag, int backwards );
HYTEG_HOST_API int hyteg_host_operator_compute_inverse_diagonal( hh_operator_t op );
HYTEG_HOST_API int hyteg_host_operator_inverse_diagonal( hh_operator_t op, hh_function_t* out  );

HYTEG_HOST_API int hyteg_host_elementwise_create( hh_storage_t s, int min_level, int max_level, hh_elementwise_t* out );
HYTEG_HOST_API int hyteg_host_elementwise_destroy( hh_elementwise_t op );
HYTEG_HOST_API int hyteg_host_elementwise_apply( hh_elementwise_t op, hh_function_t src, hh_function_t dst, int level, int flag, int update );
HYTEG_HOST_API int hyteg_host_elementwise_compute_inverse_diagonal( hh_elementwise_t op );
HYTEG_HOST_API int hyteg_host_elementwise_inverse_diagonal( hh_elementwise_t op, hh_function_t* out  );
HYTEG_HOST_API int hyteg_host_elementwise_smooth_jac( hh_elementwise_t op, hh_function_t dst, hh_function_t rhs, hh_function_t src, double relax,
                                                      int level, int flag );

HYTEG_HOST_API int hyteg_host_restrict( hh_function_t f, int source_level, int flag );
HYTEG_HOST_API int hyteg_host_prolongate( hh_function_t f, int source_level, int flag );
HYTEG_HOST_API int hyteg_host_prolongate_and_add( hh_function_t f, int source_level, int flag );

HYTEG_HOST_API int hyteg_host_gmg_create( hh_storage_t s, int min_level, int max_level, int smoother, double relax, int pre, int post,
                                          int wcycle, int cg_max_iter, double cg_tol, hh_solver_t* out );
HYTEG_HOST_API int hyteg_host_chebyshev_coefficients( int order, double lower, double upper, double* out  );
HYTEG_HOST_API int hyteg_host_chebyshev_estimate_radius( hh_operator_t op, int level, int max_iter, hh_function_t x, hh_function_t tmp,
                                                         double* radius );
HYTEG_HOST_API int hyteg_host_chebyshev_create( hh_storage_t s, int min_level, int max_level, int order, const double* radii, int n_radii,
                                                double upper, double lower, hh_solver_t* out );
HYTEG_HOST_API int hyteg_host_chebyshev_set_fused( hh_solver_t solver, int on );
HYTEG_HOST_API int hyteg_host_gmg_create_chebyshev( hh_storage_t s, int min_level, int max_level, int order, const double* radii, int n_radii,
                                                    double upper, double lower, int pre, int post, int wcycle, int cg_max_iter, double cg_tol,
                                                    hh_solver_t* out );
HYTEG_HOST_API int hyteg_host_gmg_set_use_graphs( hh_solver_t solver, int on );
HYTEG_HOST_API int hyteg_host_gmg_replayed_cycles( hh_solver_t solver, int* count );
HYTEG_HOST_API int hyteg_host_cg_set_use_device_scalars( hh_solver_t solver, int on );
HYTEG_HOST_API int hyteg_host_cg_iterations( hh_solver_t solver, int* iterations );
HYTEG_HOST_API int hyteg_host_cg_create( hh_storage_t s, int min_level, int max_level, int max_iter, double tol, hh_solver_t* out );
HYTEG_HOST_API int hyteg_host_solver_solve( hh_solver_t solver, hh_operator_t laplace, hh_function_t x, hh_function_t b, int level );
HYTEG_HOST_API int hyteg_host_solver_destroy( hh_solver_t solver );

HYTEG_HOST_API int hyteg_host_stokes_function_create( hh_storage_t s, const char* name, int min_level, int max_level, hh_stokes_function_t* out );
// ... 89 lines not shown
```

Before: 257.1 billion.

## Batch per-cell P1 apply into multi-cell inner and boundary launches

```diff
diff --git a/hyteg_amd/capi.py b/hyteg_amd/capi.py
--- a/hyteg_amd/capi.py
+++ b/hyteg_amd/capi.py
@@ -67,6 +67,7 @@
     "hyteg_hip_cell_index": (_i64, [_i, _i, _i, _i]),
     "hyteg_hip_p1_apply_cell": (_i, [_vp, _vp, _i, _dp, _i, _vp]),
     "hyteg_hip_p1_apply_cell_steps": (_i, [C.POINTER(_vp), C.POINTER(_vp), _i, _i, _dp, _i, _vp]),
+    "hyteg_hip_p1_apply_cells_inner": (_i, [C.POINTER(_vp), C.POINTER(_vp), _dp, _i, _i, _i, _vp]),
     "hyteg_hip_p1_apply_kernel_name": (_i, [_i, _i, C.c_char_p, _sz]),
     "hyteg_hip_p1_residual_jacobi_start_f32": (_i, [_vp, _vp, _vp, _vp, _i, _dp, _d, _vp]),
     "hyteg_hip_p1_jacobi_accumulate_f32": (_i, [_vp, _vp, _vp, _i, _dp, _d, _vp]),
@@ -91,6 +92,7 @@
     "hyteg_hip_p1_restrict_cell": (_i, [_vp, _vp, _i, _dp, _vp]),
     "hyteg_hip_p1_prolongate_cell": (_i, [_vp, _vp, _i, _dp, _i, _vp]),
     "hyteg_hip_p1_apply_cell_boundary": (_i, [_vp, _vp, _i, _dp, C.c_uint, _i, _vp]),
+    "hyteg_hip_p1_apply_cells_boundary": (_i, [C.POINTER(_vp), C.POINTER(_vp), _vp, C.POINTER(C.c_uint), _i, _i, _i, _vp]),
     "hyteg_hip_p1_vector_cell_masked": (_i, [_i, _vp, _i, C.POINTER(_vp), _dp, _i, C.c_uint, _vp]),
     "hyteg_hip_p1_set_cell_masked": (_i, [_vp, _d, _i, C.c_uint, _vp]),
     "hyteg_hip_p1_dot_cell_masked": (_i, [_vp, _vp, _i, C.c_uint, _vp, _vp, _vp]),
@@ -352,6 +354,17 @@
     check(lib().hyteg_hip_p1_apply_cell_steps(d, s, len(dsts), level, _w15(w), update, stream), "p1_apply_cell_steps")
 
 
+def p1_apply_cells_inner(dsts, srcs, level, stencils, update=REPLACE, stream=0):
+    if len(srcs) != len(dsts) or len(stencils) != len(dsts):
+        raise ValueError("p1_apply_cells_inner: as many sources and stencils as destinations")
+    d, s = (_vp * len(dsts))(*[int(p) for p in dsts]), (_vp * len(srcs))(*[int(p) for p in srcs])
+    flat = [float(v) for w in stencils for v in w]
+    if len(flat) != 15 * len(dsts):
+        raise ValueError("p1_apply_cells_inner: 15 weights per cell")
+    arr = (C.c_double * max(1, len(flat)))(*flat)
+    check(lib().hyteg_hip_p1_apply_cells_inner(d, s, arr, len(dsts), level, update, stream), "p1_apply_cells_inner")
+
+
 def p1_jacobi_cell(dst, rhs, src, level, w, relax, invdiag=None, stream=0):
     check(lib().hyteg_hip_p1_jacobi_cell(dst, rhs, src, invdiag, level, _w15(w), float(relax), stream),
           "p1_jacobi_cell")
@@ -418,6 +431,14 @@
     flat = [float(v) for row in w_slots for v in row]
     arr = (C.c_double * 210)(*flat)
     check(lib().hyteg_hip_p1_apply_cell_boundary(dst, src, level, arr, mask, update, stream), "p1_apply_cell_boundary")
+
+
+def p1_apply_cells_boundary(dsts, srcs, level, w_slots_dev, masks, update=REPLACE, stream=0):
+    if len(srcs) != len(dsts) or len(masks) != len(dsts):
+        raise ValueError("p1_apply_cells_boundary: as many sources and masks as destinations")
+    d, s = (_vp * len(dsts))(*[int(p) for p in dsts]), (_vp * len(srcs))(*[int(p) for p in srcs])
+    m = (C.c_uint * max(1, len(masks)))(*[int(x) for x in masks])
+    check(lib().hyteg_hip_p1_apply_cells_boundary(d, s, w_slots_dev, m, len(dsts), level, update, stream), "p1_apply_cells_boundary")
 
 
 def p1_vector_cell_masked(op, dst, scalars, srcs, level, mask, stream=0):
diff --git a/hyteg_amd/csrc/exp/apply_trace.hip b/hyteg_amd/csrc/exp/apply_trace.hip
--- a/hyteg_amd/csrc/exp/apply_trace.hip
+++ b/hyteg_amd/csrc/exp/apply_trace.hip
@@ -36,7 +36,7 @@
 template < int NY, int LZ, int PFD >
 __global__ __launch_bounds__( 64 * kZMarchWavesPerBlock ) void zmarch_trace_kernel( const ZMarchArgs A )
 {
-   zmarch_body< APPLY_REPLACE, NY, LZ, PFD, double >( A, A.tasks, A.ntasks, A.xcd_chunk, A.src, A.dst );
+   zmarch_body< APPLY_REPLACE, NY, LZ, PFD, double >( A, A.tasks, A.ntasks, A.xcd_chunk, A.src, A.dst, A.st );
 }
 
 #define CK( e )                                                                                \
diff --git a/hyteg_amd/csrc/exp/p1_apply_rank.hip b/hyteg_amd/csrc/exp/p1_apply_rank.hip
--- a/hyteg_amd/csrc/exp/p1_apply_rank.hip
+++ b/hyteg_amd/csrc/exp/p1_apply_rank.hip
@@ -38,7 +38,7 @@
    const int b = blockIdx.x;
    if ( b < R.brickBlocks )
    {
-      zmarch_body< MODE, kBrickNY, LZ, 2, double >( A, tasks, ntasks, xcd_chunk, A.src, A.dst );
+      zmarch_body< MODE, kBrickNY, LZ, 2, double >( A, tasks, ntasks, xcd_chunk, A.src, A.dst, A.st );
       return;
    }
    double*       dst = static_cast< double* >( A.dst );
diff --git a/hyteg_amd/csrc/kernels_apply_zmarch.hpp b/hyteg_amd/csrc/kernels_apply_zmarch.hpp
--- a/hyteg_amd/csrc/kernels_apply_zmarch.hpp
+++ b/hyteg_amd/csrc/kernels_apply_zmarch.hpp
@@ -108,7 +108,8 @@
 }
 
 template < int MODE, int NY, int LZ, int PFD, typename T >
-__device__ inline void zmarch_body( const ZMarchArgs& A, const BrickTask* tasks, int ntasks, int xcd_chunk, const void* srcp, void* dstp )
+__device__ inline void zmarch_body( const ZMarchArgs& A, const BrickTask* tasks, int ntasks, int xcd_chunk, const void* srcp, void* dstp,
+                                    const Stencil15& st )
 {
    static_assert( LZ + 2 <= kBrickMaxSlices, "the table carries the slice bases of bricks of up to kBrickMaxSlices - 2 slices" );
    constexpr int SZ = (int) sizeof( T );
@@ -175,8 +176,8 @@
    T w[15];
 #pragma unroll
    for ( int i = 0; i < 15; ++i )
-      w[i] = (T) A.st.w[i];
-   const T invc  = (T) ( 1.0 / A.st.w[7] );
+      w[i] = (T) st.w[i];
+   const T invc  = (T) ( 1.0 / st.w[7] );
    const T relax = (T) A.relax;
 
    constexpr int kExAux = MODE == APPLY_ADD ? 2 : 0;
@@ -304,7 +305,7 @@
 __global__ __launch_bounds__( 64 * kZMarchWavesPerBlock ) void p1_apply_zmarch_preload_kernel( const BrickTask* tasks, int ntasks, int xcd_chunk,
                                                                                               const ZMarchArgs A )
 {
-   zmarch_body< MODE, NY, LZ, PFD, T >( A, tasks, ntasks, xcd_chunk, A.src, A.dst );
+   zmarch_body< MODE, NY, LZ, PFD, T >( A, tasks, ntasks, xcd_chunk, A.src, A.dst, A.st );
 }
 
 constexpr int kZMarchMaxSteps = 16;
@@ -320,7 +321,22 @@
 {
    static_assert( MODE == APPLY_REPLACE || MODE == APPLY_ADD, "a steps launch has one source and one destination per step" );
    const unsigned step = blockIdx.y < (unsigned) kZMarchMaxSteps ? blockIdx.y : 0u;
-   zmarch_body< MODE, NY, LZ, PFD, T >( A, tasks, ntasks, xcd_chunk, P.srcs[step], P.dsts[step] );
+   zmarch_body< MODE, NY, LZ, PFD, T >( A, tasks, ntasks, xcd_chunk, P.srcs[step], P.dsts[step], A.st );
+}
+
+struct ZMarchCellStencils
+{
+   Stencil15 st[kZMarchMaxSteps];
+};
+
+template < int MODE, int NY, int LZ, int PFD, typename T >
+__global__ __launch_bounds__( 64 * kZMarchWavesPerBlock ) void p1_apply_zmarch_cells_kernel( const BrickTask* tasks, int ntasks, int xcd_chunk,
+                                                                                            const ZMarchArgs A, const ZMarchStepPtrs P,
+                                                                                            const ZMarchCellStencils C )
+{
+   static_assert( MODE == APPLY_REPLACE || MODE == APPLY_ADD, "a cells launch has one source and one destination per cell" );
+   const unsigned cell = blockIdx.y < (unsigned) kZMarchMaxSteps ? blockIdx.y : 0u;
+   zmarch_body< MODE, NY, LZ, PFD, T >( A, tasks, ntasks, xcd_chunk, P.srcs[cell], P.dsts[cell], C.st[cell] );
 }
 
 inline void build_brick_tasks( int level, int NY, int LZ, std::vector< BrickTask >& out )
diff --git a/hyteg_amd/csrc/p1_apply.hip b/hyteg_amd/csrc/p1_apply.hip
--- a/hyteg_amd/csrc/p1_apply.hip
+++ b/hyteg_amd/csrc/p1_apply.hip
@@ -145,6 +145,50 @@
    hipLaunchKernelGGL( kern, dim3( nblocks, nsteps ), dim3( 64 * kZMarchWavesPerBlock ), lds, stream, A.tasks, A.ntasks, A.xcd_chunk, A, P );
    HH_CHECK_HIP( hipGetLastError() );
    return HYTEG_HIP_OK;
+}
+
+template < int MODE, int NY, int LZ, int PFD >
+int launch_zmarch_cells_shape( void* const* dsts, const void* const* srcs, const double* stencils, int ncells, int level, hipStream_t stream )
+{
+   static_assert( MODE == APPLY_REPLACE || MODE == APPLY_ADD, "cells launch: Replace and Add" );
+   ZMarchArgs A{};
+   int        nblocks = 0;
+   const int  rc      = zmarch_common_args< double >( A, nblocks, NY, LZ, level, stencils );
+   if ( rc != HYTEG_HIP_OK || nblocks == 0 )
+      return rc;
+   ZMarchStepPtrs     P{};
+   ZMarchCellStencils C{};
+   for ( int k = 0; k < kZMarchMaxSteps; ++k )
+   {
+      const int c = k < ncells ? k : 0;
+      P.srcs[k]   = srcs[c];
+      P.dsts[k]   = dsts[c];
+      for ( int i = 0; i < 15; ++i )
+         C.st[k].w[i] = stencils[15 * c + i];
+   }
+   A.src = P.srcs[0];
+   A.dst = P.dsts[0];
+   auto           kern = p1_apply_zmarch_cells_kernel< MODE, NY, LZ, PFD, double >;
+   const unsigned lds  = steps_lds_request( level );
+   if ( lds > 0 )
+   {
+      static const hipError_t attr = hipFuncSetAttribute( reinterpret_cast< const void* >( kern ), hipFuncAttributeMaxDynamicSharedMemorySize, (int) lds );
+      HH_CHECK_HIP( attr );
+   }
+   hipLaunchKernelGGL( kern, dim3( nblocks, ncells ), dim3( 64 * kZMarchWavesPerBlock ), lds, stream, A.tasks, A.ntasks, A.xcd_chunk, A, P, C );
+   HH_CHECK_HIP( hipGetLastError() );
+   return HYTEG_HIP_OK;
+}
+
+template < int MODE >
+int launch_zmarch_cells( void* const* dsts, const void* const* srcs, const double* stencils, int ncells, int level, hipStream_t stream )
+{
+   int        rc       = HYTEG_HIP_OK;
+   const bool compiled = with_compiled_shape( current_shape( MODE, level, false ), [&]( auto ny, auto lz, auto pfd ) {
+      rc = launch_zmarch_cells_shape< MODE, decltype( ny )::value, decltype( lz )::value, decltype( pfd )::value >( dsts, srcs, stencils, ncells, level,
+                                                                                                                    stream );
+   } );
+   return compiled ? rc : fail( HYTEG_HIP_EINVAL, "apply cells: brick shape not compiled in" );
 }
 
 template < int MODE, typename T = double >
@@ -266,6 +310,32 @@
    return launch_zmarch_steps< APPLY_ADD >( dsts, srcs, nsteps, level, w, as_stream( stream ) );
 }
 
+HYTEG_HIP_API int hyteg_hip_p1_apply_cells_inner( void* const*       dsts,
+                                                  const void* const* srcs,
+                                                  const double*      stencils,
+                                                  int                ncells,
+                                                  int                level,
+                                                  int                update,
+                                                  hyteg_hip_stream_t stream )
+{
+   HH_REQUIRE( dsts && srcs && stencils, "p1_apply_cells_inner: null pointer" );
+   HH_REQUIRE( ncells >= 1 && ncells <= kZMarchMaxSteps, "p1_apply_cells_inner: ncells out of range [1,16]" );
+   HH_REQUIRE( level_ok( level ), "p1_apply_cells_inner: level out of range [2,11]" );
+   HH_REQUIRE( update == HYTEG_HIP_REPLACE || update == HYTEG_HIP_ADD, "p1_apply_cells_inner: bad update type" );
+   for ( int i = 0; i < ncells; ++i )
+   {
+      HH_REQUIRE( dsts[i] && srcs[i], "p1_apply_cells_inner: null array" );
+      for ( int j = 0; j < ncells; ++j )
+         HH_REQUIRE( dsts[i] != srcs[j] && ( i == j || dsts[i] != dsts[j] ),
+                     "p1_apply_cells_inner: an array written for one cell must not be read or written for another (nor be the cell's own source)" );
+   }
+   if ( !level_runs_zmarch( level ) )
+      return fail( HYTEG_HIP_ENOTSUP, "p1_apply_cells_inner: this level does not run the z-march kernel" );
+   if ( update == HYTEG_HIP_REPLACE )
+      return launch_zmarch_cells< APPLY_REPLACE >( dsts, srcs, stencils, ncells, level, as_stream( stream ) );
+   return launch_zmarch_cells< APPLY_ADD >( dsts, srcs, stencils, ncells, level, as_stream( stream ) );
+}
+
 HYTEG_HIP_API int hyteg_hip_p1_apply_cell_f32( float* dst, const float* src, int level, const double* w, int update, hyteg_hip_stream_t stream )
 {
    HH_REQUIRE( dst && src && w, "p1_apply_cell_f32: null pointer" );
diff --git a/hyteg_amd/csrc/p1_boundary.hip b/hyteg_amd/csrc/p1_boundary.hip
--- a/hyteg_amd/csrc/p1_boundary.hip
+++ b/hyteg_amd/csrc/p1_boundary.hip
@@ -24,6 +24,31 @@
    const T   acc = share< T >( S, src, N, x, y, z, slot );
    const int i   = cell_index( N, x, y, z );
    dst[i]        = update == HYTEG_HIP_ADD ? acc + dst[i] : acc;
+}
+
+constexpr int kShellMaxCells = 16;
+struct ShellCells
+{
+   double*       dst[kShellMaxCells];
+   const double* src[kShellMaxCells];
+   unsigned      mask[kShellMaxCells];
+};
+
+__global__ __launch_bounds__( kThreads ) void p1_apply_shell_cells_kernel( const ShellCells A, const Slots14x15* __restrict__ slots, int N, int update )
+{
+   const unsigned cell = blockIdx.y < (unsigned) kShellMaxCells ? blockIdx.y : 0u;
+   const unsigned mask = A.mask[cell];
+   if ( mask == 0u )
+      return;
+   const int q = blockIdx.x * kThreads + threadIdx.x;
+   int       x, y, z, slot;
+   if ( !shell_point( N, q, x, y, z, slot ) || !( ( mask >> slot ) & 1u ) )
+      return;
+   const double* __restrict__ src = A.src[cell];
+   double* __restrict__ dst       = A.dst[cell];
+   const double acc               = share< double >( slots[cell], src, N, x, y, z, slot );
+   const int    i                 = cell_index( N, x, y, z );
+   dst[i]                         = update == HYTEG_HIP_ADD ? acc + dst[i] : acc;
 }
 
 __global__ __launch_bounds__( kThreads ) void p1_apply_shell_send_kernel( double* __restrict__ dst,
@@ -424,6 +449,41 @@
    const int N = ( 1 << level ) + 1;
    hipLaunchKernelGGL( p1_apply_shell_kernel< double >, dim3( shell_blocks( N ) ), dim3( kThreads ), 0, as_stream( stream ), dst, src, N,
                        mask & HYTEG_HIP_MASK_SHELL, update, S );
+   HH_CHECK_HIP( hipGetLastError() );
+   return HYTEG_HIP_OK;
+}
+
+HYTEG_HIP_API int hyteg_hip_p1_apply_cells_boundary( double* const*       dsts,
+                                                     const double* const* srcs,
+                                                     const double*        w_slots_dev,
+                                                     const unsigned*      masks,
+                                                     int                  ncells,
+                                                     int                  level,
+                                                     int                  update,
+                                                     hyteg_hip_stream_t   stream )
+{
+   HH_REQUIRE( dsts && srcs && w_slots_dev && masks, "p1_apply_cells_boundary: null pointer" );
+   HH_REQUIRE( ncells >= 1 && ncells <= kShellMaxCells, "p1_apply_cells_boundary: ncells out of range [1,16]" );
+   HH_REQUIRE( any_level_ok( level ), "p1_apply_cells_boundary: level out of range [0,11]" );
+   HH_REQUIRE( update == HYTEG_HIP_REPLACE || update == HYTEG_HIP_ADD, "p1_apply_cells_boundary: bad update type" );
+   ShellCells A{};
+   bool       any = false;
+   for ( int i = 0; i < ncells; ++i )
+   {
+      HH_REQUIRE( dsts[i] && srcs[i], "p1_apply_cells_boundary: null array" );
+      for ( int j = 0; j < ncells; ++j )
+         HH_REQUIRE( dsts[i] != srcs[j] && ( i == j || dsts[i] != dsts[j] ),
+                     "p1_apply_cells_boundary: an array written for one cell must not be read or written for another (nor be the cell's own source)" );
+      A.dst[i]  = dsts[i];
+      A.src[i]  = srcs[i];
+      A.mask[i] = masks[i] & HYTEG_HIP_MASK_SHELL;
+      any       = any || A.mask[i] != 0u;
+   }
+   if ( !any )
+      return HYTEG_HIP_OK;
+   const int N = ( 1 << level ) + 1;
+   hipLaunchKernelGGL( p1_apply_shell_cells_kernel, dim3( shell_blocks( N ), ncells ), dim3( kThreads ), 0, as_stream( stream ), A,
+                       reinterpret_cast< const Slots14x15* >( w_slots_dev ), N, update );
    HH_CHECK_HIP( hipGetLastError() );
    return HYTEG_HIP_OK;
 }
diff --git a/hyteg_amd/host.py b/hyteg_amd/host.py
--- a/hyteg_amd/host.py
+++ b/hyteg_amd/host.py
@@ -34,6 +34,8 @@
     "hyteg_host_storage_lanes_seen": (_i, [_vp, C.POINTER(C.c_uint)]),
     "hyteg_host_storage_set_apply_steps": (_i, [_vp, _i]),
     "hyteg_host_storage_steps_launches": (_i, [_vp, C.POINTER(_u)]),
+    "hyteg_host_storage_set_apply_cells": (_i, [_vp, _i]),
+    "hyteg_host_storage_cells_launches": (_i, [_vp, C.POINTER(_u)]),
     "hyteg_host_apply_steps_plan": (_i, [_i, C.POINTER(C.c_ulonglong), C.POINTER(C.c_ulonglong), _i, _i, _i, _i, _ip, _ip]),
     "hyteg_host_lane_plan": (_i, [_i, _i, _ip, C.POINTER(C.c_ulonglong), _ip, C.POINTER(C.c_ulonglong), _ip, C.POINTER(_u)]),
     "hyteg_host_storage_set_hooks": (_i, [_vp, EXCHANGE_CB, EXCHANGE_CB, ALLREDUCE_CB, _vp]),
@@ -293,6 +295,14 @@
         _ck(lib().hyteg_host_storage_steps_launches(self.h, C.byref(n)), "steps_launches")
         return n.value
 
+    def set_apply_cells(self, on):
+        _ck(lib().hyteg_host_storage_set_apply_cells(self.h, on), "set_apply_cells")
+
+    def cells_launches(self):
+        n = C.c_uint()
+        _ck(lib().hyteg_host_storage_cells_launches(self.h, C.byref(n)), "cells_launches")
+        return n.value
+
     def set_stream(self, stream):
         _ck(lib().hyteg_host_storage_set_stream(self.h, stream), "set_stream")
         self.stream = int(stream) if stream else 0
diff --git a/hyteg_amd/host/hyteg_host_capi.cpp b/hyteg_amd/host/hyteg_host_capi.cpp
--- a/hyteg_amd/host/hyteg_host_capi.cpp
+++ b/hyteg_amd/host/hyteg_host_capi.cpp
@@ -304,6 +304,14 @@
 HYTEG_HOST_API int hyteg_host_storage_steps_launches( hh_storage_t s, unsigned* count )
 {
    return guarded( [&] { *count = S( s ).stepsLaunchesSeen(); } );
+}
+HYTEG_HOST_API int hyteg_host_storage_set_apply_cells( hh_storage_t s, int on )
+{
+   return guarded( [&] { S( s ).setApplyCells( on ); } );
+}
+HYTEG_HOST_API int hyteg_host_storage_cells_launches( hh_storage_t s, unsigned* count )
+{
+   return guarded( [&] { *count = S( s ).cellsLaunchesSeen(); } );
 }
 HYTEG_HOST_API int hyteg_host_storage_set_apply_cell_lanes_min( hh_storage_t s, int cells )
 {
diff --git a/hyteg_amd/host/p1operator.hpp b/hyteg_amd/host/p1operator.hpp
--- a/hyteg_amd/host/p1operator.hpp
+++ b/hyteg_amd/host/p1operator.hpp
@@ -27,7 +27,13 @@
          sorTables_[l] = buildSorTables( perCell );
          if ( l >= HYTEG_HIP_MIN_LEVEL )
             hipCheck( hyteg_hip_prepare_level( (int) l ), "P1ConstantOperator: prepare_level" );
-      }
+         uploadShellSlots( l );
+      }
+   }
+   ~P1ConstantOperator()
+   {
+      for ( auto& t : shellSlots_ )
+         hyteg_hip_free( t.second );
    }
 
    std::shared_ptr< PrimitiveStorage > getStorage() const { return storage_; }
@@ -77,31 +83,40 @@
                                                             level >= HYTEG_HIP_MIN_LEVEL );
       PrimitiveStorage::ShareSend send;
       const bool bySharesKernel = shellDst.beginSumSharedCopiesByShares( level, flag, send );
-      storage_->forLocalCells( [&]( uint_t c, const MacroCell& cell ) {
-         const auto& S = getCellStencils( cell.id, level );
-         if ( bySharesKernel )
-         {
-            hipCheck( hyteg_hip_p1_apply_cell_boundary_p2p( shellDst.getCellPointer( c, level ), src.getCellPointer( c, level ), (int) level,
-                                                            &S.slots[0][0], storage_->maskFor( cell, flag ), shellUpdate, send.first, send.list,
-                                                            send.a.peers, send.a.npeers, send.a.seq, send.a.counter, storage_->stream() ),
-                      "apply: boundary + send" );
-            return;
-         }
-         hipCheck( hyteg_hip_p1_apply_cell_boundary( shellDst.getCellPointer( c, level ), src.getCellPointer( c, level ), (int) level,
-                                                     &S.slots[0][0], storage_->maskFor( cell, flag ), shellUpdate, storage_->stream() ),
-                   "apply: boundary" );
-      } );
+      const uint_t nLocal   = storage_->getNumberOfLocalCells();
+      const bool   useCells = storage_->applyCells() && nLocal > 1 && !bySharesKernel && shellSlots_.count( level ) > 0;
+      storage_->resetCellsLaunches();
+      if ( useCells )
+         applyShellCells( src, shellDst, level, flag, shellUpdate );
+      else
+         storage_->forLocalCells( [&]( uint_t c, const MacroCell& cell ) {
+            const auto& S = getCellStencils( cell.id, level );
+            if ( bySharesKernel )
+            {
+               hipCheck( hyteg_hip_p1_apply_cell_boundary_p2p( shellDst.getCellPointer( c, level ), src.getCellPointer( c, level ), (int) level,
+                                                               &S.slots[0][0], storage_->maskFor( cell, flag ), shellUpdate, send.first, send.list,
+                                                               send.a.peers, send.a.npeers, send.a.seq, send.a.counter, storage_->stream() ),
+                         "apply: boundary + send" );
+               return;
+            }
+            hipCheck( hyteg_hip_p1_apply_cell_boundary( shellDst.getCellPointer( c, level ), src.getCellPointer( c, level ), (int) level,
+                                                        &S.slots[0][0], storage_->maskFor( cell, flag ), shellUpdate, storage_->stream() ),
+                      "apply: boundary" );
+         } );
       if ( !bySharesKernel )
          shellDst.beginSumSharedCopies( level, flag );
       chain.toMain();
-      storage_->forLocalCells( [&]( uint_t c, const MacroCell& cell ) {
-         const unsigned mask = storage_->maskFor( cell, flag );
-         if ( ( mask & HYTEG_HIP_MASK_INNER ) && level >= HYTEG_HIP_MIN_LEVEL )
-            hipCheck( hyteg_hip_p1_apply_cell( dst.getCellPointer( c, level ), src.getCellPointer( c, level ), (int) level,
-                                               getCellStencils( cell.id, level ).inner, hipUpdate( updateType ),
-                                               cellLanes.active() ? storage_->laneStream( (int) c + 1 ) : storage_->stream() ),
-                      "apply: cell" );
-      } );
+      if ( useCells && level >= HYTEG_HIP_MIN_LEVEL && level <= 8 )
+         applyInnerCells( src, dst, level, flag, updateType, cellLanes );
+      else
+         storage_->forLocalCells( [&]( uint_t c, const MacroCell& cell ) {
+            const unsigned mask = storage_->maskFor( cell, flag );
+            if ( ( mask & HYTEG_HIP_MASK_INNER ) && level >= HYTEG_HIP_MIN_LEVEL )
+               hipCheck( hyteg_hip_p1_apply_cell( dst.getCellPointer( c, level ), src.getCellPointer( c, level ), (int) level,
+                                                  getCellStencils( cell.id, level ).inner, hipUpdate( updateType ),
+                                                  cellLanes.active() ? storage_->laneStream( (int) c + 1 ) : storage_->stream() ),
+                         "apply: cell" );
+         } );
       cellLanes.join();
       chain.toSide();
       shellDst.endSumSharedCopies( level, flag );
@@ -614,6 +629,90 @@
    }
 
  private:
+   void uploadShellSlots( uint_t level )
+   {
+      if ( storage_->getNumberOfLocalCells() < 2 )
+         return;
+      std::vector< double > h;
+      for ( int id : storage_->getLocalCellIDs() )
+      {
+         const auto& S = getCellStencils( id, level );
+         h.insert( h.end(), &S.slots[0][0], &S.slots[0][0] + 14 * 15 );
+      }
+      void*&             dev = shellSlots_[level];
+      hyteg_hip_stream_t s   = storage_->stream();
+      hipCheck( hyteg_hip_malloc( &dev, h.size() * sizeof( double ) ), "P1ConstantOperator: shell slots: malloc" );
+      hipCheck( hyteg_hip_upload( dev, h.data(), h.size() * sizeof( double ), s ), "P1ConstantOperator: shell slots: upload" );
+      hipCheck( hyteg_hip_stream_synchronize( s ), "P1ConstantOperator: shell slots: sync" );
+   }
+   template < typename F >
+   static void forEvenGroups( int n, int minGroups, F&& fn )
+   {
+      if ( n <= 0 )
+         return;
+      const int groups = std::min( n, std::max( minGroups, ( n + 15 ) / 16 ) );
+      for ( int g = 0, first = 0; g < groups; ++g )
+      {
+         const int count = n / groups + ( g < n % groups ? 1 : 0 );
+         fn( g, first, count );
+         first += count;
+      }
+   }
+   void applyShellCells( const P1Function< double >& src, const P1Function< double >& shellDst, uint_t level, DoFType flag, int shellUpdate ) const
+   {
+      const int                    n = (int) storage_->getNumberOfLocalCells();
+      std::vector< double* >       d( (size_t) n );
+      std::vector< const double* > u( (size_t) n );
+      std::vector< unsigned >      m( (size_t) n );
+      storage_->forLocalCells( [&]( uint_t c, const MacroCell& cell ) {
+         d[c] = shellDst.getCellPointer( c, level );
+         u[c] = src.getCellPointer( c, level );
+         m[c] = storage_->maskFor( cell, flag );
+      } );
+      const double*      slots = static_cast< const double* >( shellSlots_.at( level ) );
+      hyteg_hip_stream_t s     = storage_->stream();
+      forEvenGroups( n, 1, [&]( int, int first, int count ) {
+         bool any = false;
+         for ( int i = first; i < first + count; ++i )
+            any = any || ( m[(size_t) i] & HYTEG_HIP_MASK_SHELL );
+         if ( !any )
+            return;
+         hipCheck( hyteg_hip_p1_apply_cells_boundary( d.data() + first, u.data() + first, slots + (size_t) first * 14 * 15, m.data() + first, count,
+                                                      (int) level, shellUpdate, s ),
+                   "apply: cells boundary" );
+         storage_->countCellsLaunch();
+      } );
+   }
+   void applyInnerCells( const P1Function< double >& src, const P1Function< double >& dst, uint_t level, DoFType flag, UpdateType updateType,
+                         const PrimitiveStorage::LaneScope& cellLanes ) const
+   {
+      std::vector< void* >       d;
+      std::vector< const void* > u;
+      std::vector< double >      w;
+      storage_->forLocalCells( [&]( uint_t c, const MacroCell& cell ) {
+         if ( !( storage_->maskFor( cell, flag ) & HYTEG_HIP_MASK_INNER ) )
+            return;
+         d.push_back( dst.getCellPointer( c, level ) );
+         u.push_back( src.getCellPointer( c, level ) );
+         const double* inner = getCellStencils( cell.id, level ).inner;
+         w.insert( w.end(), inner, inner + 15 );
+      } );
+      forEvenGroups( (int) d.size(), cellLanes.active() ? cellLanes.lanes() : 1, [&]( int g, int first, int count ) {
+         hyteg_hip_stream_t s  = cellLanes.active() ? storage_->laneStream( g + 1 ) : storage_->stream();
+         int                rc = hyteg_hip_p1_apply_cells_inner( d.data() + first, u.data() + first, w.data() + (size_t) first * 15, count, (int) level,
+                                                                 hipUpdate( updateType ), s );
+         if ( rc == HYTEG_HIP_OK )
+            storage_->countCellsLaunch();
+         if ( rc == HYTEG_HIP_ENOTSUP )
+         {
+            rc = HYTEG_HIP_OK;
+            for ( int i = first; i < first + count && rc == HYTEG_HIP_OK; ++i )
+               rc = hyteg_hip_p1_apply_cell( static_cast< double* >( d[(size_t) i] ), static_cast< const double* >( u[(size_t) i] ), (int) level,
+                                             w.data() + (size_t) i * 15, hipUpdate( updateType ), s );
+         }
+         hipCheck( rc, "apply: cells inner" );
+      } );
+   }
    template < typename T, typename Build >
    const T* deviceTable( std::map< std::pair< uint_t, uint_t >, const T* >& cache, uint_t level, uint_t nf, Build&& hostTable ) const
    {
@@ -759,6 +858,7 @@
    mutable std::map< std::pair< uint_t, uint_t >, const double* >                         stencilTables_, restTables_;
    mutable std::map< std::pair< uint_t, uint_t >, const hyteg_hip_sor_shell_tables* >     shellTables_;
    std::shared_ptr< P1Function< double > >                    inverseDiagonalValues_;
+   std::map< uint_t, void* >                                  shellSlots_;
 };
 
 using P1ConstantLaplaceOperator = P1ConstantOperator< forms::P1LaplaceForm >;
diff --git a/hyteg_amd/host/storage.hpp b/hyteg_amd/host/storage.hpp
--- a/hyteg_amd/host/storage.hpp
+++ b/hyteg_amd/host/storage.hpp
@@ -339,6 +339,27 @@
    unsigned stepsLaunchesSeen() const { return stepsLaunches_; }
    void     resetStepsLaunches() const { stepsLaunches_ = 0; }
    void     countStepsLaunch() const { ++stepsLaunches_; }
+   void setApplyCells( int on )
+   {
+      if ( on != 0 && on != 1 )
+         throw std::runtime_error( "setApplyCells: 0 (per-cell launches) or 1 (cells launches)" );
+      applyCells_ = on;
+   }
+   bool applyCells() const
+   {
+      if ( applyCells_ < 0 )
+      {
+         static const int fromEnv = [] {
+            const char* e = std::getenv( "HYTEG_AMD_APPLY_CELLS" );
+            return e ? ( std::atoi( e ) != 0 ? 1 : 0 ) : 1;
+         }();
+         applyCells_ = fromEnv;
+      }
+      return applyCells_ != 0;
+   }
+   unsigned cellsLaunchesSeen() const { return cellsLaunches_; }
+   void     resetCellsLaunches() const { cellsLaunches_ = 0; }
+   void     countCellsLaunch() const { ++cellsLaunches_; }
    bool applyStepsUsable() const
    {
       if ( nranks_ != 1 || mainStream_ || timingTree_ )
@@ -1054,7 +1075,8 @@
    mutable hyteg_hip_event_t                               laneEvents_[LanePlanner::kMaxLanes]  = {}, laneFork_ = nullptr;
    mutable int                                             laneCount_ = -1, laneDepth_ = 0, applySteps_ = -1;
    mutable int                                             cellLanesMin_ = -1;
-   mutable unsigned                                        laneUsed_  = 0, lanesSeen_ = 0, stepsLaunches_ = 0;
+   mutable int                                             applyCells_ = -1;
+   mutable unsigned                                        laneUsed_  = 0, lanesSeen_ = 0, stepsLaunches_ = 0, cellsLaunches_ = 0;
    mutable bool                                            lanesOn_ = false, laneManual_ = false;
    std::shared_ptr< Transport >                            transport_;
    std::shared_ptr< TimingTree >                           timingTree_;
diff --git a/include/hyteg_hip.h b/include/hyteg_hip.h
--- a/include/hyteg_hip.h
+++ b/include/hyteg_hip.h
@@ -84,6 +84,13 @@
                                                  const double*      w ,
                                                  int                update,
                                                  hyteg_hip_stream_t stream );
+HYTEG_HIP_API int hyteg_hip_p1_apply_cells_inner( void* const*       dsts ,
+                                                  const void* const* srcs ,
+                                                  const double*      stencils ,
+                                                  int                ncells,
+                                                  int                level,
+                                                  int                update,
+                                                  hyteg_hip_stream_t stream );
 
 HYTEG_HIP_API int hyteg_hip_p1_apply_cell_f32( float* dst, const float* src, int level, const double* w , int update, hyteg_hip_stream_t stream );
 HYTEG_HIP_API int hyteg_hip_p1_jacobi_cell_f32( float*             dst,
@@ -212,6 +219,14 @@
                                                     unsigned           mask,
                                                     int                update,
                                                     hyteg_hip_stream_t stream );
+HYTEG_HIP_API int hyteg_hip_p1_apply_cells_boundary( double* const*       dsts ,
+                                                     const double* const* srcs ,
+                                                     const double*        w_slots_dev ,
+                                                     const unsigned*      masks ,
+                                                     int                  ncells,
+                                                     int                  level,
+                                                     int                  update,
+                                                     hyteg_hip_stream_t   stream );
 
 HYTEG_HIP_API int hyteg_hip_p1_vector_cell_masked( int                  op,
                                                    double*              dst,
diff --git a/include/hyteg_host.h b/include/hyteg_host.h
--- a/include/hyteg_host.h
+++ b/include/hyteg_host.h
@@ -40,6 +40,8 @@
                                          const unsigned long long* write_ids, int* lane_out, unsigned* waits_out );
 HYTEG_HOST_API int hyteg_host_storage_set_apply_steps( hh_storage_t s, int steps );
 HYTEG_HOST_API int hyteg_host_storage_steps_launches( hh_storage_t s, unsigned* count );
+HYTEG_HOST_API int hyteg_host_storage_set_apply_cells( hh_storage_t s, int on );
+HYTEG_HOST_API int hyteg_host_storage_cells_launches( hh_storage_t s, unsigned* count );
 HYTEG_HOST_API int hyteg_host_apply_steps_plan( int npairs, const unsigned long long* src_ids, const unsigned long long* dst_ids, int first, int steps,
                                                 int max_group, int lanes, int* sizes_out, int* ngroups_out );
 HYTEG_HOST_API int hyteg_host_storage_enable_timing( hh_storage_t s, int on, int synchronize );
```

New measurement: 257.2 billion, median of 2. About the same (+0.0%).
